# ZihanLiao/pytorch-kaldi-resnet

Hardware: AMD Instinct MI355X
Metric: utterances/sec (300-frame x 80 fbank, bs256/GPU), ResNet-34 + AAM-softmax training step (higher is better)
Workload: dtype f32 (operands as 2 fp16 terms of value x 2^k, 3 cross products, f32 accumulate); 1 GPU; BASELINE configs[1]: ResNet-34 + AAM-softmax (m 0.2, s 30), 1211 speakers, 300-frame x 80 fbank, per-GPU batch 256, fwd+CE+bwd+SGD(0.9, wd 5e-4); global_batch=256, frames=300, feat_dim=80, parallelism=dp1, launch=hipGraph replay (1 graph), mfma=f16x3

## Files before the change

### include/spkhip.h

```cpp
#ifndef SPKHIP_H
#define SPKHIP_H
#include <stddef.h>
#ifdef __cplusplus
extern "C" {
#endif

int spk_version(void);
const char* spk_last_error(void);
int spk_build_flags(void);

#define SPK_IN_AFFINE_RELU 1
#define SPK_EPI_AFFINE 2
#define SPK_EPI_ADD 4
#define SPK_EPI_RELU 8
#define SPK_EPI_STATS 16
#define SPK_IN_BNBWD 64
#define SPK_EPI_BNBWD 32

#define SPK_CONV_WS 128
#define SPK_CONV_PIPE 1024

#define SPK_CONV_M16 (1 << 17)

#define SPK_WGRAD_GROUPS 2048

#define SPK_WGRAD_NOSHIFT (1 << 18)
#define SPK_WGRAD_M16 (1 << 19)
#define SPK_IN_PRESPLIT (1 << 14)
#define SPK_SIDE_PRESPLIT (1 << 15)
#define SPK_DY_PRESPLIT (1 << 16)
#define SPK_CONV_CK32 (1 << 23)
#define SPK_EPI_WMASK (1 << 24)


int spk_pack_conv_weight(const float* w, float* wpk, int Cout, int Cin, int KH, int KW, int transpose, void* stream);
int spk_pack_conv_weight_split(const float* w, void* wpk, int Cout, int Cin, int KH, int KW, int transpose, int split,
                               void* stream);
int spk_pack_job_bytes(void);
int spk_pack_conv_weights_batched(const void* jobs, int njobs, int total_blocks, int has_f16 , void* stream);

int spk_conv_mfma(const float* in, const float* wpk, float* out, const float* in_scale, const float* in_shift,
                  const float* epi_scale, const float* epi_shift, const float* epi_add, const float* in_raw,
                  const float* in_act, const float* in_bn4, const float* in_coef, const unsigned* in_mask , const unsigned* bn_mask , const unsigned* add_mask ,
                  float* side_draw, float* side_dz,
                  const float* bn_raw, const float* bn_act, const float* bn4, float* stats, int B, int IH,
                  int IW, int Cin, int OH, int OW, int OHf, int OWf, int Cout, int IS, int OS, int ooy, int oox,
                  int ntaps, const int* tap_dy , const int* tap_dx , const int* tap_w , int TH,
                  int TW, int MT, int NT, int kc, int ips, int flags, int split, const unsigned* in_amax, unsigned* out_amax,
                  unsigned* side_amax, void* stream);
int spk_conv_mfma_len(const float* in, const float* wpk, float* out, const float* in_scale, const float* in_shift,
                      const float* epi_scale, const float* epi_shift, const float* epi_add, const float* in_raw,
                      const float* in_act, const float* in_bn4, const float* in_coef, const unsigned* in_mask,
                      const unsigned* bn_mask, const unsigned* add_mask, float* side_draw, float* side_dz,
                      const float* bn_raw, const float* bn_act, const float* bn4, float* stats, int B, int IH,
                      int IW, int Cin, int OH, int OW, int OHf, int OWf, int Cout, int IS, int OS, int ooy, int oox,
                      int ntaps, const int* tap_dy , const int* tap_dx , const int* tap_w , int TH,
                      int TW, int MT, int NT, int kc, int ips, int flags, int split, const unsigned* in_amax, unsigned* out_amax,
                      unsigned* side_amax, const int* wlen , void* stream);

int spk_conv_wgrad_limits(int WN, int* max_halo_pix , int* max_tile_pix );
size_t spk_conv_wgrad_workspace(int nsplit, int ksize, int Cin, int Cout);
int spk_conv3x3_c32_stream(const float* in, const float* wpk, float* out, const float* in_scale, const float* in_shift, float* stats,
                           int B, int H, int W, int flags, const unsigned* in_amax, unsigned* out_amax, int nblocks, void* stream);
int spk_conv1x1_stream(const float* in, const float* wpk, float* out, const float* in_scale, const float* in_shift,
                       const float* epi_add, const unsigned* add_mask, const float* bn_raw, const unsigned* bn_mask,
                       const float* bn4, float* stats, long long P, int C, int flags, const unsigned* in_amax, unsigned* out_amax,
                       int nblocks, void* stream);
int spk_conv1x1_stream_rows(int nblocks, int C);
int spk_wgrad_reduce(const float* partial, float* dw, int nslab, int ksize, int Cin, int Cout, int accumulate, void* stream);
int spk_conv_wgrad(const float* x, const float* dy, float* dw, float* partial, const float* in_scale,
                   const float* in_shift, int B, int IH, int IW, int Cin, int OH, int OW, int Cout, int ksize, int stride,
                   int TH, int TW, int WN, int nsplit, int flags, int accumulate, int split , const unsigned* dy_amax , const unsigned* x_amax , void* stream);

#define SPK_PTR_ADD_MASK 1
#define SPK_PTR_BN_MASK 2
#define SPK_PTR_IN_MASK 4
#define SPK_PTR_IN_ACT 8
#define SPK_PTR_BN_ACT 16
#define SPK_PTR_SIDE_DZ 32
int spk_conv_variant_of(int MT, int NT, int split, int flags, int ptrs);
int spk_wgrad_variant_of(int ksize, int stride, int TH, int TW, int WN, int split, int flags);

int spk_stem_fwd_blocks(int B, int F, int T);
int spk_stem_conv_fwd(const float* x, const float* w, float* out, float* stats, const float* epi_scale,
                      const float* epi_shift, int B, int F, int T, int flags,
                      unsigned* amax_out , void* stream);
int spk_stem_conv_fwd_len(const float* x, const float* w, float* out, float* stats, const float* epi_scale,
                          const float* epi_shift, int B, int F, int T, int flags, unsigned* amax_out, const int* len ,
                          void* stream);
int spk_stem_wgrad_blocks(int B, int F, int T);
int spk_stem_conv_wgrad(const float* x, const float* draw, float* dw, float* partial, int B, int F, int T,
                        int accumulate, void* stream);
int spk_stem_stats(const float* x, const float* w, float* stats, int B, int F, int T, void* stream);
int spk_stem_fwd_apply(const float* x, const float* w, const float* scale, const float* shift, float* raw_out, float* act_out,
                       unsigned* mask_out, unsigned* amax_out, int B, int F, int T, void* stream);
int spk_stem_bwd_wgrad(const float* x, const float* d, const float* raw, const float* mean, const float* invstd,
                       const float* scale, const float* shift, const float* coef, float* dw, float* partial, int B, int F, int T,
                       int accumulate, void* stream);

int spk_bn_stats_blocks(long long N, int C);
int spk_bn_stats_partial(const float* x, float* partial , long long N, int C, void* stream);
size_t spk_bn_finalize_workspace(int nblk, int C);
int spk_bn_finalize(const float* partial, int nblk, int C, double count, const float* gamma, const float* beta,
                    float* running_mean, float* running_var, long long* num_batches_tracked, float* mean, float* invstd,
                    float* scale, float* shift, float momentum, float eps, double* ws,
                    const unsigned* amax_in, unsigned* est_out ,
                    void* stream);
int spk_bn_eval_coeffs(const float* gamma, const float* beta, const float* running_mean, const float* running_var,
                       float* scale, float* shift, int C, float eps, void* stream);
int spk_bn_apply(const float* raw, const float* scale, const float* shift, const float* res, const float* res_scale,
                 const float* res_shift, float* out, unsigned* mask_out, long long N, int C, int relu,
                 unsigned* amax_out , void* stream);
int spk_bn_bwd_reduce(const float* dy, const float* raw, const float* act, const float* mean, const float* invstd,
                      const float* scale, const float* shift, float* partial, long long N, int C, int mask_mode,
                      unsigned* chan_amax , void* stream);
int spk_bn_bwd_finalize(const float* partial, int nblk, int C, double count, const float* gamma, const float* invstd,
                        float* dgamma, float* dbeta, float* coef , int accumulate, double* ws,
                        const unsigned* amax_in, const unsigned* raw_amax, const float* mean, unsigned* est_out ,
                        const unsigned* chan_amax ,
                        void* stream);
int spk_bn_bwd_apply(const float* dy, const float* raw, const float* act, const float* mean, const float* invstd,
                     const float* scale, const float* shift, const float* coef, float* draw, float* dz_out, long long N,
                     int C, int mask_mode, unsigned* amax_out ,
                     const unsigned* pair_scale , void* stream);
int spk_absmax(const float* x, unsigned* slot, long long n, void* stream);
int spk_bnbwd_estimate(const float* coef, const float* mean, const float* invstd, int C, const unsigned* amax_in,
                       const unsigned* raw_amax, unsigned* est, void* stream);
int spk_f16_window_count(const float* x, const float* scale, const float* shift, long long n, int C, const unsigned* slot,
                         int pairs, unsigned long long* counts , void* stream);
int spk_affine_estimate(const float* scale, const float* shift, int C, const unsigned* amax_in, unsigned* est, void* stream);

int spk_se_chunks(long long HW);
int spk_se_squeeze(const float* x, float* partial, double* sums , int B, int H, int W, int C, const int* wlen,
                   void* stream);
int spk_se_excite(const double* sums, const float* scale, const float* shift, const float* W1, const float* W2, float* q,
                  float* u, float* g, int B, int C, int Cr, int H, int W, const int* wlen, void* stream);
int spk_se_apply(const float* raw, const float* scale, const float* shift, const float* gate, const float* res,
                 const float* res_scale, const float* res_shift, float* out, unsigned* mask_out, int B, int H, int W, int C,
                 int relu, unsigned* amax_out, const int* wlen, void* stream);
int spk_se_bwd_reduce(const float* dout, const float* raw, const float* act, float* partial, double* S , int B,
                      long long HW, int C, int mask_mode, unsigned* chan_amax, void* stream);
int spk_se_bwd_gate(const double* S, const double* sums, const float* q, const float* u, const float* g, const float* W1,
                    const float* W2, const float* mean, const float* invstd, const float* scale, const float* shift,
                    const float* gamma, float* da, float* du, float* dq, float* dW1, float* dW2, float* dgamma, float* dbeta,
                    float* coef, int accumulate, int B, int C, int Cr, long long HW, const unsigned* amax_in,
                    const unsigned* raw_amax, const unsigned* chan_amax, unsigned* est_out, void* stream);
int spk_se_bwd_apply(const float* dout, const float* raw, const float* act, const float* gate, const float* dqs ,
                     const float* mean, const float* invstd, const float* coef, float* draw, float* e_out, int B, long long HW,
                     int C, int mask_mode, unsigned* amax_out, const unsigned* pair_scale, void* stream);

int spk_stats_pool_fwd(const float* x , float* out , int B, int H, int W, int C,
                       int mode, void* stream);
int spk_stats_pool_fwd_len(const float* x, float* out, const int* wlen, int B, int H, int W, int C, int mode, void* stream);
int spk_stats_pool_bwd(const float* x, const float* gout, float* dx, int B, int H, int W, int C, int mode,
                       unsigned* amax_out , void* stream);
int spk_stats_pool_row_form(int on);
int spk_stats_pool_row_cap(void);

int spk_gemm_splitk(int M, int N, int K);
size_t spk_gemm_workspace(int M, int N, int K);
int spk_gemm_f32(const float* A, const float* B, float* C, const float* bias, int M, int N, int K, long long sam,
                 long long sak, long long sbk, long long sbn, long long ldc, float alpha, int accumulate, float* workspace,
                 void* stream);
int spk_colsum(const float* dy, float* db, int M, int N, int accumulate, void* stream);

int spk_l2norm_fwd(const float* x, float* y, float* inv_norm, int R, int D, float eps, void* stream);
int spk_l2norm_bwd(const float* y, const float* inv_norm, const float* dy, float* dx, int R, int D, float eps,
                   int accumulate, void* stream);
int spk_aam_margin_fwd(const float* cosv, const long long* label, float* logits, int B, int S, float m, float s,
                       void* stream);
int spk_aam_margin_bwd(const float* cosv, const long long* label, const float* dlogits, float* dcos, int B, int S,
                       float m, float s, void* stream);
int spk_softmax_ce(const float* logits, const long long* label, float* loss_row, float* dlogits, int* rank, int B, int S,
                   float grad_scale, void* stream);
int spk_mean(const float* v, float* out, int n, void* stream);
int spk_relu_bwd(const float* y, const float* dy, float* dx, long long n, void* stream);

int spk_sgd_step(float* p, const float* g, float* buf, long long n, float lr, float momentum, float weight_decay,
                 float grad_scale, int first_step, void* stream);

int spk_center_normalize(const float* emb , const float* mean , float* out, int N, int D, float eps,
                         void* stream);
int spk_trial_cosine(const float* en , const float* te , const int* ia, const int* ib, float* out,
                     int T, int D, int n_en, int n_te, void* stream);
int spk_topk_mean_std(const float* scores, float* mean_out, float* std_out, int N, int M, int k, long long ld, void* stream);

int spk_eval_tile(int which);
int spk_segment_mean(const double* emb , const int* rows , const int* seg_off , float* out ,
                     int N, int S, int D, void* stream);
int spk_trial_snorm(const void* score, int score_f64, const int* ia, const int* ib, const double* e_mean, const double* e_std,
                    const double* t_mean, const double* t_std, double* out, int T, void* stream);
size_t spk_sort_trials_workspace(int T);
int spk_sort_trials(const double* score, unsigned* order, void* ws, int T, void* stream);
size_t spk_error_sweep_workspace(int T, int P);
int spk_error_sweep(const double* score, const unsigned char* label, const unsigned* order, const double* costs, int P,
                    double* out_d , long long* out_i , void* ws, int T, void* stream);

int spk_fbank_tile_frames(int L, int S, int P, int F);
int spk_fbank_fwd(const float* wave, const int* nsamp, const long long* utt_ids, int B, long long Nmax, const float* window,
                  const float* twiddle, const float* mel_w, const int* mel_lo, const int* mel_off, int L, int S, int P, int F,
                  int snip_edges, float dither, float preemph, int remove_dc, float energy_floor, unsigned long long seed,
                  float* feats, float* log_energy, int* T_out, int Tcap, void* stream);
int spk_mfcc_tile_frames(int L, int S, int P, int F, int C);
int spk_mfcc_fwd(const float* wave, const int* nsamp, const long long* utt_ids, int B, long long Nmax, const float* window,
                 const float* twiddle, const float* mel_w, const int* mel_lo, const int* mel_off, const float* dct,
                 const float* lifter, int L, int S, int P, int F, int C, int snip_edges, float dither, float preemph, int remove_dc,
                 float energy_floor, int use_energy, int htk_compat, unsigned long long seed, float* feats, float* log_energy,
                 int* T_out, int Tcap, void* stream);
int spk_fbank_span_fwd(const float* wave, const int* nsamp, const long long* first, const long long* total, const int* frame0,
                       const int* nframes, const long long* utt_ids, int B, long long Nmax, const float* window, const float* twiddle,
                       const float* mel_w, const int* mel_lo, const int* mel_off, int L, int S, int P, int F, int snip_edges,
                       float dither, float preemph, int remove_dc, float energy_floor, unsigned long long seed, float* feats,
                       float* log_energy, int* T_out, int Tcap, void* stream);
int spk_mfcc_span_fwd(const float* wave, const int* nsamp, const long long* first, const long long* total, const int* frame0,
                      const int* nframes, const long long* utt_ids, int B, long long Nmax, const float* window, const float* twiddle,
                      const float* mel_w, const int* mel_lo, const int* mel_off, const float* dct, const float* lifter, int L, int S,
                      int P, int F, int C, int snip_edges, float dither, float preemph, int remove_dc, float energy_floor,
                      int use_energy, int htk_compat, unsigned long long seed, float* feats, float* log_energy, int* T_out, int Tcap,
                      void* stream);
int spk_pcm16_to_f32(const short* pcm , const int* count , int B, long long Nmax, float* out ,
                     void* stream);
int spk_fbank_dither_noise(float* out , long long utt_id, unsigned long long seed, int frame0, int nframes, int L,
                           void* stream);
int spk_vad_count(const float* log_energy, const int* T, int B, int Tcap, double energy_threshold, double mean_scale,
                  int frames_context, double proportion, int* vad , int* idx , int* count ,
                  void* stream);
int spk_cmn_select(const float* x, const int* T, const int* idx, const int* count, double* prefix, float* out, int B, int F,
                   int Tcap, int Tout, int cmn_window, void* stream);

int spk_resample_tile(int iu, int ou, int K);
int spk_resample_fwd(const float* wave_in, const int* nsamp_in, int B, long long Nmax_in, const int* first, const float* wq,
                     int fi, int fo, int K, float* wave_out, int* nsamp_out, long long Nmax_out, void* stream);

int spk_augment_max_rir(void);
int spk_augment_max_early(void);
int spk_augment_workspace(int B, long long Nmax, int Rmax, int Emax, long long Fmax, int nd, long long* sizes );
int spk_augment_fwd(const float* wave, const int* nsamp, int B, long long Nmax, const float* rir_pool, long long rir_pool_len,
                    const long long* rir_off, const int* rir_row, int Rmax, int Emax, const float* noise_pool,
                    long long noise_pool_len, const int* desc_ptr, const long long* desc_off, const int* desc_len,
                    const double* desc_snr, int nd, long long Fmax, const float* twiddle, float* spectra, float* y, double* work,
                    int quantize, float* out, unsigned long long* clipped, void* stream);

int spk_cm_decode(const unsigned char* codes, const float* colhdr, const int* lengths, int B, int F, int T, float* out, void* stream);
int spk_cm_compress(const float* x, const int* T, int B, int F, int Tcap, float* ws, float* minrange, int* hdr, unsigned char* codes,
                    void* stream);

int spk_scatter_slab_rows(long long N);
size_t spk_scatter_f64_workspace(long long N, int D);
int spk_scatter_f64(const void* X, int x_f64, long long ld, const double* mu, const double* w, double* C, void* ws, long long N, int D,
                    void* stream);
int spk_segment_sum_f64(const void* X, int x_f64, long long ld, const int* rows, const int* seg_off , double* out ,
                        int* count , int mean, int K, int D, void* stream);
int spk_affine_lennorm(const void* X, int x_f64, long long ldx, const double* A, const double* b, const double* q, int scale, void* Y,
                       int y_f64, long long N, int Di, int Do, void* stream);
int spk_plda_posterior_rows(const double* mt , const int* count, const double* psi, double* w_out, double* r_out, int K,
                            int D, void* stream);
int spk_plda_llr(const double* en , const double* te , const int* ia, const int* ib, const double* psi,
                 const int* count , const int* tab_count , const double* tab_log , int U, float* out,
                 int T, int D, int n_en, int n_te, void* stream);

#ifdef __cplusplus
}
#endif
#endif
```

### pytorch-kaldi-resnet_amd/csrc/bn.hip

```cpp
#include "spk_common.h"

enum { MASK_NONE = 0, MASK_ACT = 1, MASK_RAW = 2, MASK_BITS = 3 };

__global__ __launch_bounds__(256) void bn_stats_partial_kernel(const float* __restrict__ x, float* __restrict__ partial,
                                                               long long N, int C, int rows_per_block) {
    __shared__ float red[256][8];
    const int tid = threadIdx.x;
    const int qpr = C >> 2;
    const int quad = tid % qpr, prow = tid / qpr, rstep = 256 / qpr;
    const long long r0 = (long long)blockIdx.x * rows_per_block;
    long long r1 = r0 + rows_per_block;
    if (r1 > N) r1 = N;
    f32x4 s = {0.f, 0.f, 0.f, 0.f}, ss = {0.f, 0.f, 0.f, 0.f};
    for (long long r = r0 + prow; r < r1; r += rstep) {
        const f32x4 v = *(const f32x4*)(x + r * C + quad * 4);
        s += v;
        ss += v * v;
    }
#pragma unroll
    for (int k = 0; k < 4; ++k) {
        red[tid][k] = s[k];
        red[tid][4 + k] = ss[k];
    }
    __syncthreads();
    if (tid < qpr) {
        float a[8];
#pragma unroll
        for (int k = 0; k < 8; ++k) a[k] = 0.f;
        for (int p = 0; p < rstep; ++p)
#pragma unroll
            for (int k = 0; k < 8; ++k) a[k] += red[p * qpr + tid][k];
        float* dst = partial + ((size_t)blockIdx.x * C + tid * 4) * 2;
#pragma unroll
        for (int k = 0; k < 4; ++k) {
            dst[k * 2 + 0] = a[k];
            dst[k * 2 + 1] = a[4 + k];
        }
    }
}

static bool bn_c_ok(int C) { return C >= 4 && C <= 1024 && (C & (C - 1)) == 0; }

#ifndef BN_STATS_BLOCKS
#define BN_STATS_BLOCKS 4096
#endif
extern "C" int spk_bn_stats_blocks(long long N, int C) {
    (void)C;
    long long nb = (N + 255) / 256;
    if (nb > BN_STATS_BLOCKS) nb = BN_STATS_BLOCKS;
    return (int)(nb < 1 ? 1 : nb);
}

extern "C" int spk_bn_stats_partial(const float* x, float* partial, long long N, int C, void* stream) {
    SPK_REQUIRE(x && partial, "spk_bn_stats_partial: null pointer");
    SPK_REQUIRE(N > 0 && bn_c_ok(C), "spk_bn_stats_partial: N=%lld C=%d (C must be a power of two in [4,1024])", N, C);
    const int nb = spk_bn_stats_blocks(N, C);
    const int rpb = (int)((N + nb - 1) / nb);
    hipLaunchKernelGGL(bn_stats_partial_kernel, dim3(nb), dim3(256), 0, (hipStream_t)stream, x, partial, N, C, rpb);
    SPK_LAUNCH_CHECK("spk_bn_stats_partial");
    return 0;
}

#define BN_STAGE_ROWS 256
__global__ __launch_bounds__(256) void bn_fold_partials_kernel(const float* __restrict__ partial, double* __restrict__ ws,
                                                               int nblk, int C) {
    __shared__ double red[8][32][2];
    const int tid = threadIdx.x, c = tid & 31, row = tid >> 5;
    const int ch = blockIdx.x * 32 + c;
    const int per = (nblk + BN_STAGE_ROWS - 1) / BN_STAGE_ROWS;
    const int k0 = blockIdx.y * per;
    int k1 = k0 + per;
    if (k1 > nblk) k1 = nblk;
    double s = 0.0, ss = 0.0;
    if (ch < C) {
        const size_t pitch = (size_t)8 * C * 2;
        const float* q = partial + ((size_t)(k0 + row) * C + ch) * 2;
        int k = k0 + row;
        for (; k + 24 < k1; k += 32, q += 4 * pitch) {
            const float2 a = *(const float2*)q, b = *(const float2*)(q + pitch);
            const float2 c2 = *(const float2*)(q + 2 * pitch), d = *(const float2*)(q + 3 * pitch);
            s += (double)a.x; ss += (double)a.y;
            s += (double)b.x; ss += (double)b.y;
            s += (double)c2.x; ss += (double)c2.y;
            s += (double)d.x; ss += (double)d.y;
        }
        for (; k < k1; k += 8, q += pitch) {
            const float2 p = *(const float2*)q;
            s += (double)p.x;
            ss += (double)p.y;
        }
    }
    red[row][c][0] = s;
    red[row][c][1] = ss;
    __syncthreads();
    if (row == 0 && ch < C) {
        for (int k = 1; k < 8; ++k) {
            s += red[k][c][0];
            ss += red[k][c][1];
        }
        ws[((size_t)blockIdx.y * C + ch) * 2 + 0] = s;
        ws[((size_t)blockIdx.y * C + ch) * 2 + 1] = ss;
    }
}

template <typename T>
__device__ inline void bn_sum_rows(const T* __restrict__ partial, int nrows, int C, int ch, int row, double& s, double& ss) {
    const size_t pitch = (size_t)8 * C * 2;
    const T* p = partial + ((size_t)row * C + ch) * 2;
    int k = row;
    for (; k + 24 < nrows; k += 32, p += 4 * pitch) {
        const T a0 = p[0], a1 = p[1], b0 = p[pitch], b1 = p[pitch + 1];
        const T c0 = p[2 * pitch], c1 = p[2 * pitch + 1], d0 = p[3 * pitch], d1 = p[3 * pitch + 1];
        s += (double)a0; ss += (double)a1;
        s += (double)b0; ss += (double)b1;
        s += (double)c0; ss += (double)c1;
        s += (double)d0; ss += (double)d1;
    }
    for (; k < nrows; k += 8, p += pitch) {
        s += (double)p[0];
        ss += (double)p[1];
    }
}

template <typename T>
__global__ __launch_bounds__(256) void bn_finalize_kernel(const T* __restrict__ partial, int nblk, int C, double count,
                                                          const float* __restrict__ gamma, const float* __restrict__ beta,
                                                          float* __restrict__ running_mean, float* __restrict__ running_var,
                                                          long long* __restrict__ nbt, float* __restrict__ mean_out,
                                                          float* __restrict__ invstd_out, float* __restrict__ scale,
                                                          float* __restrict__ shift, float momentum, float eps,
                                                          const unsigned* __restrict__ amax_in, unsigned* __restrict__ est_out) {
    __shared__ double red[8][32][2];
    const int tid = threadIdx.x, c = tid & 31, row = tid >> 5;
    const int ch = blockIdx.x * 32 + c;
    double s = 0.0, ss = 0.0;
    if (ch < C) bn_sum_rows<T>(partial, nblk, C, ch, row, s, ss);
    red[row][c][0] = s;
    red[row][c][1] = ss;
    __syncthreads();
    if (row == 0 && ch < C) {
        for (int k = 1; k < 8; ++k) {
            s += red[k][c][0];
            ss += red[k][c][1];
        }
        const double mean = s / count;
        double var = ss / count - mean * mean;
        if (var < 0.0 || count <= 1.0) var = 0.0;
        const float invstd = (float)(1.0 / sqrt(var + (double)eps));
        const float g = gamma[ch], b = beta[ch];
        const float sc = g * invstd;
        mean_out[ch] = (float)mean;
        invstd_out[ch] = invstd;
        const float shv = b - (float)mean * sc;
        scale[ch] = sc;
        shift[ch] = shv;
        if (est_out) {
            const float e = fabsf(sc) * __uint_as_float(*amax_in) + fabsf(shv);
            const unsigned bits = __float_as_uint(e);
            if (bits > __hip_atomic_load(est_out, __ATOMIC_RELAXED, __HIP_MEMORY_SCOPE_AGENT)) atomicMax(est_out, bits);
        }
        if (running_mean) {
            const double unbiased = count > 1.0 ? var * (count / (count - 1.0)) : var;
            running_mean[ch] = (1.f - momentum) * running_mean[ch] + momentum * (float)mean;
            running_var[ch] = (1.f - momentum) * running_var[ch] + momentum * (float)unbiased;
        }
    }
    if (nbt && blockIdx.x == 0 && tid == 0) *nbt += 1;
}

extern "C" size_t spk_bn_finalize_workspace(int nblk, int C) {
    return nblk > BN_STAGE_ROWS ? (size_t)BN_STAGE_ROWS * C * 2 * sizeof(double) : 0;
}

extern "C" int spk_bn_finalize(const float* partial, int nblk, int C, double count, const float* gamma, const float* beta,
                               float* running_mean, float* running_var, long long* num_batches_tracked, float* mean,
                               float* invstd, float* scale, float* shift, float momentum, float eps, double* ws,
                               const unsigned* amax_in, unsigned* est_out, void* stream) {
    SPK_REQUIRE(partial && gamma && beta && mean && invstd && scale && shift, "spk_bn_finalize: null pointer");
    SPK_REQUIRE(nblk > 0 && C > 0 && count > 0, "spk_bn_finalize: bad sizes");
    SPK_REQUIRE((running_mean == nullptr) == (running_var == nullptr), "spk_bn_finalize: running stats must come in pairs");
    SPK_REQUIRE(!est_out || amax_in, "spk_bn_finalize: est_out needs amax_in");
    hipStream_t st = (hipStream_t)stream;
    if (spk_bn_finalize_workspace(nblk, C)) {
        SPK_REQUIRE(ws, "spk_bn_finalize: %d partial rows need the fp64 workspace", nblk);
        hipLaunchKernelGGL(bn_fold_partials_kernel, dim3(spk_ceil_div(C, 32), BN_STAGE_ROWS), dim3(256), 0, st, partial, ws, nblk, C);
        SPK_LAUNCH_CHECK("spk_bn_finalize(fold)");
        hipLaunchKernelGGL(bn_finalize_kernel<double>, dim3(spk_ceil_div(C, 32)), dim3(256), 0, st, ws, BN_STAGE_ROWS, C, count,
                           gamma, beta, running_mean, running_var, num_batches_tracked, mean, invstd, scale, shift, momentum, eps,
                           amax_in, est_out);
    } else {
        hipLaunchKernelGGL(bn_finalize_kernel<float>, dim3(spk_ceil_div(C, 32)), dim3(256), 0, st, partial, nblk, C, count, gamma,
                           beta, running_mean, running_var, num_batches_tracked, mean, invstd, scale, shift, momentum, eps, amax_in,
                           est_out);
    }
    SPK_LAUNCH_CHECK("spk_bn_finalize");
    return 0;
}

__global__ void bn_eval_coeffs_kernel(const float* gamma, const float* beta, const float* rm, const float* rv,
                                      float* scale, float* shift, int C, float eps) {
    const int c = blockIdx.x * blockDim.x + threadIdx.x;
    if (c >= C) return;
    const float invstd = 1.f / sqrtf(rv[c] + eps);
    const float sc = gamma[c] * invstd;
    scale[c] = sc;
    shift[c] = beta[c] - rm[c] * sc;
}

extern "C" int spk_bn_eval_coeffs(const float* gamma, const float* beta, const float* running_mean,
                                  const float* running_var, float* scale, float* shift, int C, float eps, void* stream) {
    SPK_REQUIRE(gamma && beta && running_mean && running_var && scale && shift, "spk_bn_eval_coeffs: null pointer");
    hipLaunchKernelGGL(bn_eval_coeffs_kernel, dim3(spk_ceil_div(C, 256)), dim3(256), 0, (hipStream_t)stream, gamma, beta,
                       running_mean, running_var, scale, shift, C, eps);
    SPK_LAUNCH_CHECK("spk_bn_eval_coeffs");
    return 0;
}

#ifndef BN_APPLY_U
#define BN_APPLY_U 4
#endif
#ifndef BN_APPLY_CAP
#define BN_APPLY_CAP 0
#endif
#ifndef BN_BWD_APPLY_U
#define BN_BWD_APPLY_U 1
#endif
#ifndef BN_BWD_APPLY_CAP
#define BN_BWD_APPLY_CAP 2048
#endif
static int stream_grid(long long nquads, int per_thread = 1, int cap = 8192) {
    long long nb = (nquads + 256LL * per_thread - 1) / (256LL * per_thread);
    if (cap > 0 && nb > cap) nb = cap;
    if (nb > 2147483647LL) nb = 2147483647LL;
    return (int)(nb < 1 ? 1 : nb);
}
#ifndef BN_NT
#define BN_NT 1
#endif
static __device__ __forceinline__ f32x4 ld_stream(const float* p) {
#if BN_NT
    return __builtin_nontemporal_load((const f32x4*)p);
#else
    return *(const f32x4*)p;
#endif
}
static __device__ __forceinline__ void st_stream(float* p, f32x4 v) {
#if BN_NT
    __builtin_nontemporal_store(v, (f32x4*)p);
#else
    *(f32x4*)p = v;
#endif
}
__global__ __launch_bounds__(256) void bn_apply_kernel(const float* __restrict__ raw, const float* __restrict__ scale,
                                                       const float* __restrict__ shift, const float* __restrict__ res,
                                                       const float* __restrict__ rscale, const float* __restrict__ rshift,
                                                       float* __restrict__ out, unsigned* __restrict__ mask_out, long long nquads,
                                                       int C, int relu, unsigned* __restrict__ amax_out) {
    const int cmask = C - 1;
    float mx = 0.f;
    constexpr int U = BN_APPLY_U;
    const long long stride = (long long)gridDim.x * 256;
    const bool fixed_c = C <= 1024;
    const int c0 = (threadIdx.x * 4) & cmask;
    f32x4 psc = *(const f32x4*)(scale + c0), psh = *(const f32x4*)(shift + c0), prs = psc, prh = psh;
    if (rscale) {
        prs = *(const f32x4*)(rscale + c0);
        prh = *(const f32x4*)(rshift + c0);
    }
    for (long long i0 = (long long)blockIdx.x * 256 + threadIdx.x; i0 < nquads; i0 += stride * U) {
        f32x4 rv[U], sv[U];
        long long idx[U];
#pragma unroll
        for (int u = 0; u < U; ++u) {
            const long long i = i0 + stride * u;
            idx[u] = i < nquads ? i : i0;
            rv[u] = ld_stream(raw + idx[u] * 4);
            if (res) sv[u] = ld_stream(res + idx[u] * 4);
        }
#pragma unroll
        for (int u = 0; u < U; ++u) {
            const long long i = i0 + stride * u;
            if (i >= nquads) continue;
            if (!fixed_c) {
                const int c = (int)((i * 4) & cmask);
                psc = *(const f32x4*)(scale + c);
                psh = *(const f32x4*)(shift + c);
                if (rscale) {
                    prs = *(const f32x4*)(rscale + c);
                    prh = *(const f32x4*)(rshift + c);
                }
            }
            f32x4 v = rv[u] * psc + psh;
            if (res) {
                f32x4 r = sv[u];
                if (rscale) r = r * prs + prh;
                v += r;
            }
            if (relu) {
                v[0] = fmaxf(v[0], 0.f);
                v[1] = fmaxf(v[1], 0.f);
                v[2] = fmaxf(v[2], 0.f);
                v[3] = fmaxf(v[3], 0.f);
            }
            st_stream(out + i * 4, v);
            mx = fmaxf(fmaxf(mx, fmaxf(fabsf(v[0]), fabsf(v[1]))), fmaxf(fabsf(v[2]), fabsf(v[3])));
            if (mask_out) {
                unsigned bits = (v[0] > 0.f ? 1u : 0u) | (v[1] > 0.f ? 2u : 0u) | (v[2] > 0.f ? 4u : 0u) | (v[3] > 0.f ? 8u : 0u);
                bits <<= 4 * (threadIdx.x & 7);
                bits |= __shfl_xor(bits, 1, 64);
                bits |= __shfl_xor(bits, 2, 64);
                bits |= __shfl_xor(bits, 4, 64);
                if ((threadIdx.x & 7) == 0) mask_out[i >> 3] = bits;
            }
        }
    }
    if (amax_out) spk_wave_amax_commit(mx, amax_out);
}

extern "C" int spk_bn_apply(const float* raw, const float* scale, const float* shift, const float* res,
                            const float* res_scale, const float* res_shift, float* out, unsigned* mask_out, long long N, int C,
                            int relu, unsigned* amax_out, void* stream) {
    SPK_REQUIRE(raw && scale && shift && out, "spk_bn_apply: null pointer");
    SPK_REQUIRE(N > 0 && bn_c_ok(C), "spk_bn_apply: N=%lld C=%d", N, C);
    SPK_REQUIRE((res_scale == nullptr) == (res_shift == nullptr), "spk_bn_apply: residual affine must come in pairs");
    SPK_REQUIRE(!res_scale || res, "spk_bn_apply: residual affine without residual");
    SPK_REQUIRE(!mask_out || C % 32 == 0, "spk_bn_apply: the sign mask needs C %% 32 == 0 (C=%d)", C);
    const long long nquads = N * C / 4;
    hipLaunchKernelGGL(bn_apply_kernel, dim3(stream_grid(nquads, BN_APPLY_U, BN_APPLY_CAP)), dim3(256), 0, (hipStream_t)stream, raw, scale, shift, res,
                       res_scale, res_shift, out, mask_out, nquads, C, relu, amax_out);
    SPK_LAUNCH_CHECK("spk_bn_apply");
    return 0;
}

__device__ inline f32x4 bn_mask(f32x4 dy, int mode, const float* act, const float* raw_p, f32x4 rawv, f32x4 sc, f32x4 sh,
                                long long off, int C = 0) {
    if (mode == MASK_BITS) {
        const int lg = 31 - __builtin_clz((unsigned)C);
        const long long pix = off >> lg;
        const int c = (int)(off & (C - 1));
        const unsigned bits = ((const unsigned*)act)[pix * (C >> 5) + (c >> 5)] >> (c & 31);
#pragma unroll
        for (int k = 0; k < 4; ++k) dy[k] = ((bits >> k) & 1u) ? dy[k] : 0.f;
    } else if (mode == MASK_ACT) {
        const f32x4 a = *(const f32x4*)(act + off);
#pragma unroll
        for (int k = 0; k < 4; ++k) dy[k] = a[k] > 0.f ? dy[k] : 0.f;
    } else if (mode == MASK_RAW) {
        const f32x4 z = rawv * sc + sh;
#pragma unroll
        for (int k = 0; k < 4; ++k) dy[k] = z[k] > 0.f ? dy[k] : 0.f;
    }
    (void)raw_p;
    return dy;
}

__global__ __launch_bounds__(256) void bn_bwd_reduce_kernel(const float* __restrict__ dy, const float* __restrict__ raw,
                                                            const float* __restrict__ act, const float* __restrict__ mean,
                                                            const float* __restrict__ invstd, const float* __restrict__ scale,
                                                            const float* __restrict__ shift, float* __restrict__ partial,
                                                            long long N, int C, int rows_per_block, int mode,
                                                            unsigned* __restrict__ chan_amax) {
    __shared__ float red[256][8];
    const int tid = threadIdx.x;
    const int qpr = C >> 2;
    const int quad = tid % qpr, prow = tid / qpr, rstep = 256 / qpr;
    const long long r0 = (long long)blockIdx.x * rows_per_block;
    long long r1 = r0 + rows_per_block;
    if (r1 > N) r1 = N;
    const f32x4 mu = *(const f32x4*)(mean + quad * 4), is = *(const f32x4*)(invstd + quad * 4);
    const f32x4 sc = *(const f32x4*)(scale + quad * 4), sh = *(const f32x4*)(shift + quad * 4);
    f32x4 s = {0.f, 0.f, 0.f, 0.f}, ss = {0.f, 0.f, 0.f, 0.f}, mx = {0.f, 0.f, 0.f, 0.f};
    for (long long r = r0 + prow; r < r1; r += rstep) {
        const long long off = r * C + quad * 4;
        const f32x4 rv = ld_stream(raw + off);
        f32x4 d = ld_stream(dy + off);
        d = bn_mask(d, mode, act, raw, rv, sc, sh, off, C);
        const f32x4 xh = (rv - mu) * is;
        s += d;
        ss += d * xh;
#pragma unroll
        for (int k = 0; k < 4; ++k) mx[k] = fmaxf(mx[k], spk_finite_abs(d[k]));
    }
#pragma unroll
    for (int k = 0; k < 4; ++k) {
        red[tid][k] = s[k];
        red[tid][4 + k] = ss[k];
    }
    __syncthreads();
    if (tid < qpr) {
        float a[8];
#pragma unroll
        for (int k = 0; k < 8; ++k) a[k] = 0.f;
        for (int p = 0; p < rstep; ++p)
#pragma unroll
            for (int k = 0; k < 8; ++k) a[k] += red[p * qpr + tid][k];
        float* dst = partial + ((size_t)blockIdx.x * C + tid * 4) * 2;
#pragma unroll
        for (int k = 0; k < 4; ++k) {
            dst[k * 2 + 0] = a[k];
            dst[k * 2 + 1] = a[4 + k];
        }
    }
    if (chan_amax) {
        __syncthreads();
#pragma unroll
        for (int k = 0; k < 4; ++k) red[tid][k] = mx[k];
        __syncthreads();
        if (tid < qpr) {
#pragma unroll
            for (int k = 0; k < 4; ++k) {
                float m = 0.f;
                for (int p = 0; p < rstep; ++p) m = fmaxf(m, red[p * qpr + tid][k]);
                const unsigned bits = __float_as_uint(m);
                unsigned* slot = chan_amax + tid * 4 + k;
                if (bits > __hip_atomic_load(slot, __ATOMIC_RELAXED, __HIP_MEMORY_SCOPE_AGENT)) atomicMax(slot, bits);
            }
        }
    }
}

extern "C" int spk_bn_bwd_reduce(const float* dy, const float* raw, const float* act, const float* mean, const float* invstd,
                                 const float* scale, const float* shift, float* partial, long long N, int C, int mask_mode,
                                 unsigned* chan_amax, void* stream) {
    SPK_REQUIRE(dy && raw && mean && invstd && scale && shift && partial, "spk_bn_bwd_reduce: null pointer");
    SPK_REQUIRE(N > 0 && bn_c_ok(C), "spk_bn_bwd_reduce: N=%lld C=%d", N, C);
    SPK_REQUIRE(mask_mode >= 0 && mask_mode <= 3, "spk_bn_bwd_reduce: mask_mode=%d", mask_mode);
    SPK_REQUIRE((mask_mode != MASK_ACT && mask_mode != MASK_BITS) || act, "spk_bn_bwd_reduce: MASK_ACT / MASK_BITS need the activated tensor / its sign bits");
    const int nb = spk_bn_stats_blocks(N, C);
    const int rpb = (int)((N + nb - 1) / nb);
    hipLaunchKernelGGL(bn_bwd_reduce_kernel, dim3(nb), dim3(256), 0, (hipStream_t)stream, dy, raw, act, mean, invstd, scale,
                       shift, partial, N, C, rpb, mask_mode, chan_amax);
    SPK_LAUNCH_CHECK("spk_bn_bwd_reduce");
    return 0;
}

__device__ inline float bnbwd_bound(float k1, float m1, float m2, float mean, float invstd, float A, float R) {
    const float xh = (R + fabsf(mean)) * fabsf(invstd);
    return fabsf(k1) * (A + fabsf(m1) + xh * fabsf(m2)) * (1.f + 1.52587890625e-05f);
}

template <typename T>
__global__ __launch_bounds__(256) void bn_bwd_finalize_kernel(const T* __restrict__ partial, int nblk, int C, double count,
                                                              const float* __restrict__ gamma, const float* __restrict__ invstd,
                                                              float* __restrict__ dgamma, float* __restrict__ dbeta,
                                                              float* __restrict__ coef, int accumulate,
                                                              const unsigned* __restrict__ amax_in, const unsigned* __restrict__ raw_amax,
                                                              const float* __restrict__ mean, unsigned* __restrict__ est_out,
                                                              const unsigned* __restrict__ chan_amax) {
    __shared__ double red[8][32][2];
    const int tid = threadIdx.x, c = tid & 31, row = tid >> 5;
    const int ch = blockIdx.x * 32 + c;
    double s = 0.0, ss = 0.0;
    if (ch < C) bn_sum_rows<T>(partial, nblk, C, ch, row, s, ss);
    red[row][c][0] = s;
    red[row][c][1] = ss;
    __syncthreads();
    if (row == 0 && ch < C) {
        for (int k = 1; k < 8; ++k) {
            s += red[k][c][0];
            ss += red[k][c][1];
        }
        dbeta[ch] = accumulate ? dbeta[ch] + (float)s : (float)s;
        dgamma[ch] = accumulate ? dgamma[ch] + (float)ss : (float)ss;
        const float k1 = gamma[ch] * invstd[ch], m1 = (float)(s / count), m2 = (float)(ss / count);
        coef[ch] = k1;
        coef[C + ch] = m1;
        coef[2 * C + ch] = m2;
        if (est_out) {
            const float A = chan_amax ? __uint_as_float(chan_amax[ch]) : __uint_as_float(*amax_in);
            const float e = bnbwd_bound(k1, m1, m2, mean[ch], invstd[ch], A, __uint_as_float(*raw_amax));
            const unsigned bits = __float_as_uint(e);
            if (bits > __hip_atomic_load(est_out, __ATOMIC_RELAXED, __HIP_MEMORY_SCOPE_AGENT)) atomicMax(est_out, bits);
        }
    }
}

extern "C" int spk_bn_bwd_finalize(const float* partial, int nblk, int C, double count, const float* gamma,
                                   const float* invstd, float* dgamma, float* dbeta, float* coef, int accumulate,
                                   double* ws, const unsigned* amax_in, const unsigned* raw_amax, const float* mean,
                                   unsigned* est_out, const unsigned* chan_amax, void* stream) {
    SPK_REQUIRE(partial && gamma && invstd && dgamma && dbeta && coef, "spk_bn_bwd_finalize: null pointer");
    SPK_REQUIRE(nblk > 0 && C > 0 && count > 0, "spk_bn_bwd_finalize: bad sizes");
    SPK_REQUIRE(!est_out || ((amax_in || chan_amax) && raw_amax && mean),
                "spk_bn_bwd_finalize: est_out needs amax_in (or chan_amax), raw_amax and mean");
    hipStream_t st = (hipStream_t)stream;
    if (spk_bn_finalize_workspace(nblk, C)) {
        SPK_REQUIRE(ws, "spk_bn_bwd_finalize: %d partial rows need the fp64 workspace", nblk);
        hipLaunchKernelGGL(bn_fold_partials_kernel, dim3(spk_ceil_div(C, 32), BN_STAGE_ROWS), dim3(256), 0, st, partial, ws, nblk, C);
        SPK_LAUNCH_CHECK("spk_bn_bwd_finalize(fold)");
        hipLaunchKernelGGL(bn_bwd_finalize_kernel<double>, dim3(spk_ceil_div(C, 32)), dim3(256), 0, st, ws, BN_STAGE_ROWS, C, count,
                           gamma, invstd, dgamma, dbeta, coef, accumulate, amax_in, raw_amax, mean, est_out, chan_amax);
    } else {
        hipLaunchKernelGGL(bn_bwd_finalize_kernel<float>, dim3(spk_ceil_div(C, 32)), dim3(256), 0, st, partial, nblk, C, count, gamma,
                           invstd, dgamma, dbeta, coef, accumulate, amax_in, raw_amax, mean, est_out, chan_amax);
    }
    SPK_LAUNCH_CHECK("spk_bn_bwd_finalize");
    return 0;
}

__global__ __launch_bounds__(256) void bn_bwd_apply_kernel(const float* __restrict__ dy, const float* __restrict__ raw,
                                                           const float* __restrict__ act, const float* __restrict__ mean,
                                                           const float* __restrict__ invstd, const float* __restrict__ scale,
                                                           const float* __restrict__ shift, const float* __restrict__ coef,
                                                           float* __restrict__ draw, float* __restrict__ dz_out,
                                                           unsigned nquads, int C, int mode, unsigned* __restrict__ amax_out,
                                                           const unsigned* __restrict__ pair_scale) {
    const int cmask = C - 1;
    float mx = 0.f;
    const float sig = pair_scale ? spk_sigma_from_amax_bits(*pair_scale) : 1.f;
    constexpr int U = BN_BWD_APPLY_U;
    const unsigned stride = gridDim.x * 256u;
    const int lgq = 29 - __builtin_clz((unsigned)C);
    const unsigned cw = (unsigned)C >> 5;
    const bool fixed_c = C <= 1024;
    const int c0 = (threadIdx.x * 4) & cmask;
    f32x4 pmu = *(const f32x4*)(mean + c0), pis = *(const f32x4*)(invstd + c0), pk1 = *(const f32x4*)(coef + c0);
    f32x4 pm1 = *(const f32x4*)(coef + C + c0), pm2 = *(const f32x4*)(coef + 2 * C + c0), psc = pmu, psh = pmu;
    if (mode == MASK_RAW) {
        psc = *(const f32x4*)(scale + c0);
        psh = *(const f32x4*)(shift + c0);
    }
    for (unsigned i0 = blockIdx.x * 256u + threadIdx.x; i0 < nquads; i0 += stride * U) {
        f32x4 rvv[U], dv[U], av[U];
        unsigned mw[U];
#pragma unroll
        for (int u = 0; u < U; ++u) {
            const unsigned i = i0 + stride * u;
            const unsigned ii = i < nquads && i >= i0 ? i : i0;
            const size_t off = (size_t)ii * 4;
            rvv[u] = ld_stream(raw + off);
            dv[u] = ld_stream(dy + off);
            if (mode == MASK_BITS) mw[u] = ((const unsigned*)act)[(size_t)(ii >> lgq) * cw + (((ii * 4u) & (unsigned)cmask) >> 5)];
            else if (mode == MASK_ACT) av[u] = *(const f32x4*)(act + off);
        }
#pragma unroll
        for (int u = 0; u < U; ++u) {
            const unsigned i = i0 + stride * u;
            if (i >= nquads || i < i0) continue;
            const int c = fixed_c ? c0 : (int)((i * 4u) & (unsigned)cmask);
            if (!fixed_c) {
                pmu = *(const f32x4*)(mean + c);
                pis = *(const f32x4*)(invstd + c);
                pk1 = *(const f32x4*)(coef + c);
                pm1 = *(const f32x4*)(coef + C + c);
                pm2 = *(const f32x4*)(coef + 2 * C + c);
                if (mode == MASK_RAW) {
                    psc = *(const f32x4*)(scale + c);
                    psh = *(const f32x4*)(shift + c);
                }
            }
            const size_t off = (size_t)i * 4;
            const f32x4 rv = rvv[u];
            f32x4 d = dv[u];
            if (mode == MASK_BITS) {
                const unsigned bits = mw[u] >> (c & 31);
#pragma unroll
                for (int k = 0; k < 4; ++k) d[k] = ((bits >> k) & 1u) ? d[k] : 0.f;
            } else if (mode == MASK_ACT) {
#pragma unroll
                for (int k = 0; k < 4; ++k) d[k] = av[u][k] > 0.f ? d[k] : 0.f;
            } else if (mode == MASK_RAW) {
                const f32x4 z = rv * psc + psh;
#pragma unroll
                for (int k = 0; k < 4; ++k) d[k] = z[k] > 0.f ? d[k] : 0.f;
            }
            const f32x4 xh = (rv - pmu) * pis;
            const f32x4 o = pk1 * (d - pm1 - xh * pm2);
            if (dz_out) st_stream(dz_out + off, d);
            if (pair_scale) {
                uint2 t0, t1;
                split2h(o, sig, t0, t1);
                st_stream(draw + off, spk_pair_pack(t0, t1));
            } else
                st_stream(draw + off, o);
            mx = fmaxf(fmaxf(mx, fmaxf(fabsf(o[0]), fabsf(o[1]))), fmaxf(fabsf(o[2]), fabsf(o[3])));
        }
    }
    if (amax_out) spk_wave_amax_commit(mx, amax_out);
}

extern "C" int spk_bn_bwd_apply(const float* dy, const float* raw, const float* act, const float* mean, const float* invstd,
                                const float* scale, const float* shift, const float* coef, float* draw, float* dz_out,
                                long long N, int C, int mask_mode, unsigned* amax_out, const unsigned* pair_scale, void* stream) {
    SPK_REQUIRE(dy && raw && mean && invstd && scale && shift && coef && draw, "spk_bn_bwd_apply: null pointer");
    SPK_REQUIRE(N > 0 && bn_c_ok(C), "spk_bn_bwd_apply: N=%lld C=%d", N, C);
    SPK_REQUIRE(mask_mode >= 0 && mask_mode <= 3, "spk_bn_bwd_apply: mask_mode=%d", mask_mode);
    SPK_REQUIRE((mask_mode != MASK_ACT && mask_mode != MASK_BITS) || act, "spk_bn_bwd_apply: MASK_ACT / MASK_BITS need the activated tensor / its sign bits");
    const long long nquads = N * C / 4;
    SPK_REQUIRE(nquads < 2147483647LL / 8, "spk_bn_bwd_apply: %lld values exceed the 32-bit group index of the kernel", N * C);
    hipLaunchKernelGGL(bn_bwd_apply_kernel, dim3(stream_grid(nquads, BN_BWD_APPLY_U, BN_BWD_APPLY_CAP)), dim3(256), 0, (hipStream_t)stream, dy, raw, act, mean,
                       invstd, scale, shift, coef, draw, dz_out, (unsigned)nquads, C, mask_mode, amax_out, pair_scale);
    SPK_LAUNCH_CHECK("spk_bn_bwd_apply");
    return 0;
}

__global__ __launch_bounds__(256) void absmax_kernel(const float* __restrict__ x, long long n, unsigned* __restrict__ slot) {
    float mx = 0.f;
    const long long nq = n >> 2;
    for (long long i = (long long)blockIdx.x * 256 + threadIdx.x; i < nq; i += (long long)gridDim.x * 256) {
        const f32x4 v = *(const f32x4*)(x + i * 4);
        mx = fmaxf(fmaxf(mx, fmaxf(spk_finite_abs(v[0]), spk_finite_abs(v[1]))), fmaxf(spk_finite_abs(v[2]), spk_finite_abs(v[3])));
    }
    if (blockIdx.x == 0 && threadIdx.x < (n & 3)) mx = fmaxf(mx, spk_finite_abs(x[nq * 4 + threadIdx.x]));
    spk_wave_amax_commit(mx, slot);
}

extern "C" int spk_absmax(const float* x, unsigned* slot, long long n, void* stream) {
    SPK_REQUIRE(x && slot && n > 0, "spk_absmax: bad arguments");
    SPK_REQUIRE((((size_t)x) & 15) == 0, "spk_absmax: x must be 16-byte aligned");
    hipLaunchKernelGGL(absmax_kernel, dim3(stream_grid(n / 4 + 1)), dim3(256), 0, (hipStream_t)stream, x, n, slot);
    SPK_LAUNCH_CHECK("spk_absmax");
    return 0;
}

__global__ __launch_bounds__(256) void bnbwd_estimate_kernel(const float* __restrict__ coef, const float* __restrict__ mean,
                                                             const float* __restrict__ invstd, int C,
                                                             const unsigned* __restrict__ amax_in, const unsigned* __restrict__ raw_amax,
                                                             unsigned* __restrict__ est) {
    __shared__ float red[4];
    const float A = __uint_as_float(*amax_in), R = __uint_as_float(*raw_amax);
    float mx = 0.f;
    for (int c = threadIdx.x; c < C; c += 256)
        mx = fmaxf(mx, bnbwd_bound(coef[c], coef[C + c], coef[2 * C + c], mean[c], invstd[c], A, R));
#pragma unroll
    for (int off = 32; off >= 1; off >>= 1) mx = fmaxf(mx, __shfl_xor(mx, off, 64));
    if ((threadIdx.x & 63) == 0) red[threadIdx.x >> 6] = mx;
    __syncthreads();
    if (threadIdx.x == 0) *est = __float_as_uint(fmaxf(fmaxf(red[0], red[1]), fmaxf(red[2], red[3])));
}

__global__ __launch_bounds__(256) void affine_estimate_kernel(const float* __restrict__ scale, const float* __restrict__ shift, int C,
                                                              const unsigned* __restrict__ amax_in, unsigned* __restrict__ est) {
    __shared__ float red[2][4];
    float ms = 0.f, mh = 0.f;
    for (int c = threadIdx.x; c < C; c += 256) {
        ms = fmaxf(ms, fabsf(scale[c]));
        mh = fmaxf(mh, fabsf(shift[c]));
    }
#pragma unroll
    for (int off = 32; off >= 1; off >>= 1) {
        ms = fmaxf(ms, __shfl_xor(ms, off, 64));
        mh = fmaxf(mh, __shfl_xor(mh, off, 64));
    }
    if ((threadIdx.x & 63) == 0) {
        red[0][threadIdx.x >> 6] = ms;
        red[1][threadIdx.x >> 6] = mh;
    }
    __syncthreads();
    if (threadIdx.x == 0) {
        ms = fmaxf(fmaxf(red[0][0], red[0][1]), fmaxf(red[0][2], red[0][3]));
        mh = fmaxf(fmaxf(red[1][0], red[1][1]), fmaxf(red[1][2], red[1][3]));
        *est = __float_as_uint(ms * __uint_as_float(*amax_in) + mh);
    }
}

extern "C" int spk_affine_estimate(const float* scale, const float* shift, int C, const unsigned* amax_in, unsigned* est,
                                   void* stream) {
    SPK_REQUIRE(scale && shift && amax_in && est && C > 0, "spk_affine_estimate: bad arguments");
    hipLaunchKernelGGL(affine_estimate_kernel, dim3(1), dim3(256), 0, (hipStream_t)stream, scale, shift, C, amax_in, est);
    SPK_LAUNCH_CHECK("spk_affine_estimate");
    return 0;
}

extern "C" int spk_bnbwd_estimate(const float* coef, const float* mean, const float* invstd, int C, const unsigned* amax_in,
                                  const unsigned* raw_amax, unsigned* est, void* stream) {
    SPK_REQUIRE(coef && mean && invstd && amax_in && raw_amax && est && C > 0, "spk_bnbwd_estimate: bad arguments");
    hipLaunchKernelGGL(bnbwd_estimate_kernel, dim3(1), dim3(256), 0, (hipStream_t)stream, coef, mean, invstd, C, amax_in, raw_amax, est);
    SPK_LAUNCH_CHECK("spk_bnbwd_estimate");
    return 0;
}

__global__ __launch_bounds__(256) void f16_window_count_kernel(const float* __restrict__ x, const float* __restrict__ scale,
                                                               const float* __restrict__ shift, long long nquads, int C,
                                                               const unsigned* __restrict__ slot, int pairs,
                                                               unsigned long long* __restrict__ counts) {
    const float sig = spk_sigma_from_amax_bits(*slot);
    const int cmask = C - 1;
    unsigned n = 0, sat = 0, lo_lost = 0, hi_sub = 0;
    for (long long i = (long long)blockIdx.x * 256 + threadIdx.x; i < nquads; i += (long long)gridDim.x * 256) {
        f32x4 v = *(const f32x4*)(x + i * 4);
        float hi[4], lo[4];
        if (pairs) {
            const uint4 u = __builtin_bit_cast(uint4, v);
            const f16x4 a = __builtin_bit_cast(f16x4, (uint2){u.x, u.y}), b = __builtin_bit_cast(f16x4, (uint2){u.z, u.w});
#pragma unroll
            for (int k = 0; k < 4; ++k) {
                hi[k] = (float)a[k];
                lo[k] = (float)b[k];
                sat += fabsf(hi[k]) >= 65504.f;
            }
        } else {
            if (scale) {
                const int c = (int)((i * 4) & cmask);
                v = v * *(const f32x4*)(scale + c) + *(const f32x4*)(shift + c);
#pragma unroll
                for (int k = 0; k < 4; ++k) v[k] = fmaxf(v[k], 0.f);
            }
#pragma unroll
            for (int k = 0; k < 4; ++k) {
                const float u = v[k] * sig;
                sat += fabsf(u) > 65504.f;
                const float uc = __builtin_amdgcn_fmed3f(u, -65504.f, 65504.f);
                const _Float16 a = (_Float16)uc;
                hi[k] = (float)a;
                lo[k] = (float)(_Float16)(uc - (float)a);
            }
        }
#pragma unroll
        for (int k = 0; k < 4; ++k) {
            n += 1;
            lo_lost += lo[k] != 0.f && fabsf(lo[k]) < 6.103515625e-05f;
            hi_sub += hi[k] != 0.f && fabsf(hi[k]) < 6.103515625e-05f;
        }
    }
    unsigned vals[4] = {n, sat, lo_lost, hi_sub};
#pragma unroll
    for (int j = 0; j < 4; ++j) {
        unsigned v = vals[j];
#pragma unroll
        for (int off = 32; off >= 1; off >>= 1) v += __shfl_xor(v, off, 64);
        if ((threadIdx.x & 63) == 0 && v) atomicAdd(counts + j, (unsigned long long)v);
    }
}

extern "C" int spk_f16_window_count(const float* x, const float* scale, const float* shift, long long n, int C,
                                    const unsigned* slot, int pairs, unsigned long long* counts, void* stream) {
    SPK_REQUIRE(x && slot && counts && n > 0 && n % 4 == 0, "spk_f16_window_count: bad arguments (n must be a multiple of 4)");
    SPK_REQUIRE((scale == nullptr) == (shift == nullptr), "spk_f16_window_count: scale / shift come in pairs");
    SPK_REQUIRE(!scale || (bn_c_ok(C) && !pairs), "spk_f16_window_count: the affine form needs a power-of-two C and an fp32 tensor");
    hipLaunchKernelGGL(f16_window_count_kernel, dim3(stream_grid(n / 4)), dim3(256), 0, (hipStream_t)stream, x, scale, shift, n / 4,
                       scale ? C : 4, slot, pairs, counts);
    SPK_LAUNCH_CHECK("spk_f16_window_count");
    return 0;
}
```

### pytorch-kaldi-resnet_amd/engine.py

```python
import torch

from . import ops
from .hip import MASK_ACT, MASK_BITS, MASK_NONE, MASK_RAW


class _Conv:
    def __init__(self, holder):
        self.h = holder
        self.cin, self.cout, self.k, self.stride = holder.cin, holder.cout, holder.k, holder.stride
        self.wpk = None
        self.wpk_t = None

    def repack(self, need_t):
        w = self.h.weight.data
        if self.cin == 1:
            return
        self.wpk = ops.pack_conv_weight(w, False, self.wpk)
        if need_t:
            self.wpk_t = ops.pack_conv_weight(w, True, self.wpk_t)

    def pack_jobs(self, need_t):
        w = self.h.weight.data
        if self.cin == 1:
            return []
        n = ops.packed_numel(w)
        if self.wpk is None or self.wpk.numel() != n:
            self.wpk = torch.empty(n, device=w.device, dtype=torch.float32)
        jobs = [(w, self.wpk, False)]
        if need_t:
            nt = ops.packed_numel(w, bwd=True)
            if self.wpk_t is None or self.wpk_t.numel() != nt:
                self.wpk_t = torch.empty(nt, device=w.device, dtype=torch.float32)
            jobs.append((w, self.wpk_t, True))
        return jobs


class _BN:
    def __init__(self, holder):
        self.h = holder
        self.c = holder.c
        self.t4 = None
        self.s4 = None
        self.e2 = None

    def finalize(self, partial, count, amax_in=None, est_out=None, keep=True):
        name = "t4" if keep else "s4"
        if getattr(self, name) is None:
            setattr(self, name, torch.empty(4, self.c, device=partial.device, dtype=torch.float32))
        t4 = getattr(self, name)
        h = self.h
        ops.bn_finalize(partial, count, h.weight.data, h.bias.data, h.running_mean, h.running_var, h.num_batches_tracked,
                        t4, amax_in=amax_in, est_out=est_out)
        return t4

    def eval_coeffs(self):
        h = self.h
        if self.e2 is None:
            self.e2 = torch.empty(2, self.c, device=h.weight.device, dtype=torch.float32)
        ops.bn_eval_coeffs(h.weight.data, h.bias.data, h.running_mean, h.running_var, self.e2)
        return self.e2


class _Block:
    def __init__(self, bp):
        self.kind = bp.kind
        self.convs = [_Conv(bp.conv1), _Conv(bp.conv2)] + ([_Conv(bp.conv3)] if bp.kind == "bottleneck" else [])
        self.bns = [_BN(bp.bn1), _BN(bp.bn2)] + ([_BN(bp.bn3)] if bp.kind == "bottleneck" else [])
        self.ds = None
        if bp.downsample is not None:
            self.ds = (_Conv(bp.downsample[0]), _BN(bp.downsample[1]))
        self.se = bp.se if bp.kind == "se_basic" else None


class _LogitsFn(torch.autograd.Function):

    @staticmethod
    def forward(ctx, eng, x, y, anchor):
        logits, saved = eng.forward_train(x, y)
        ctx.eng = eng
        ctx.saved = saved
        return logits

    @staticmethod
    def backward(ctx, dlogits):
        ctx.eng.backward(ctx.saved, dlogits.contiguous())
        ctx.saved = None
        return None, None, None, None


class Engine:
    def __init__(self, model):
        self.m = model
        r = model.res
        self.stem_conv = _Conv(r.conv1)
        self.stem_bn = _BN(r.bn1)
        self.blocks = []
        for li in range(1, 5):
            for bp in getattr(r, "layer%d" % li):
                self.blocks.append(_Block(bp))
        self.head_bn = _BN(model.bn1) if hasattr(model, "bn1") else None
        self.pool_mode = 1 if model.pooling == "mean+std" else 0
        self.dirty = True
        self._packed_for_bwd = False
        self._pack_tables = {}
        self._amax_pool = None
        self._amax_fwd = None
        self._amax_eval = None
        self._fwd_gen = 0
        self.wgrad_stream = None
        self.use_side_stream = True
        self.fuse_bn_reduce = True
        self.fuse_bn_apply = True
        import os
        self.use_sign_masks = os.environ.get("SPK_SIGN_MASKS", "1") == "1"
        self.fuse_apply_min_c = int(os.environ.get("SPK_FUSE_APPLY_MINC", "0"))
        self._fuse_apply_max_c = int(os.environ["SPK_FUSE_APPLY_MAXC"]) if "SPK_FUSE_APPLY_MAXC" in os.environ else None
        self.fuse_apply_1x1 = os.environ.get("SPK_FUSE_APPLY_1X1", "0") == "1"
        self.pair_draw = os.environ.get("SPK_PAIR_DRAW", "1") == "1"
        stem_fused = os.environ.get("SPK_STEM_FUSED", "1")
        self.stem_fused_fwd = stem_fused in ("1", "fwd")
        self.stem_fused_bwd = stem_fused in ("1", "bwd")
        self.chan_amax = os.environ.get("SPK_CHAN_AMAX", "1") == "1"
        self.window_counts = None
        self.bound_log = None

    @property
    def fuse_apply_max_c(self):
        if self._fuse_apply_max_c is not None:
            return self._fuse_apply_max_c
        return 32 if (self.pair_draw and ops.split_for(3, True) == 3) else 1000000

    @fuse_apply_max_c.setter
    def fuse_apply_max_c(self, v):
        self._fuse_apply_max_c = v

    def _all_convs(self):
        for b in self.blocks:
            for c in b.convs:
                yield c
            if b.ds is not None:
                yield b.ds[0]

    def _repack(self, need_t):
        if not self.dirty and (self._packed_for_bwd or not need_t):
            return
        jobs = [j for c in self._all_convs() for j in c.pack_jobs(need_t)]
        key = [(w.data_ptr(), p.data_ptr(), t, ops.split_for(w.shape[2], t)) for w, p, t in jobs]
        tab = self._pack_tables.get(need_t)
        if tab is None or tab.key != key:
            assert not torch.cuda.is_current_stream_capturing() or tab is None, "pack table changed during graph capture"
            tab = self._pack_tables[need_t] = ops.PackTable(jobs, jobs[0][0].device)
        tab.run()
        self.dirty = False
        self._packed_for_bwd = need_t

    def _check_input(self, x):
        if not x.is_cuda:
            raise RuntimeError("pytorch_kaldi_resnet_amd runs on MI355X only: input must be a device tensor "
                               "(there is no CPU fallback)")
        if x.dim() != 3 or x.size(1) != self.m.feat_dim:
            raise RuntimeError("expected input [B, %d, T], got %s" % (self.m.feat_dim, tuple(x.shape)))
        if x.dtype != torch.float32:
            raise RuntimeError("expected float32 input")
        return x.contiguous()

    def _fwd_pool(self, device, train=False):
        if ops.split_for(3) != 3 and ops.split_for(3, True) != 3:
            return None
        name = "_amax_fwd" if train else "_amax_eval"
        if getattr(self, name) is None:
            setattr(self, name, ops.AmaxPool(device))
        pool = getattr(self, name)
        pool.reset()
        return pool

    def _count(self, x, slot, affine=None, pairs=False):
        if self.window_counts is not None and slot is not None:
            ops.f16_window_count(x, slot, self.window_counts, affine=affine, pairs=pairs)

    def trunk_eval(self, x, wl=None):
        self._repack(False)
        pool = self._fwd_pool(x.device)
        take = (lambda: pool.take()) if pool is not None else (lambda: None)
        f16 = ops.split_for(3) == 3
        e = self.stem_bn.eval_coeffs()
        a_amax = take()
        a, _ = ops.stem_fwd(x, self.stem_conv.h.weight.data, epi_affine=(e[0], e[1]), relu=True, amax_out=a_amax,
                            wlen=None if wl is None else wl[0])
        stage = 0
        for b in self.blocks:
            evs = [bn.eval_coeffs() for bn in b.bns]
            if b.ds is not None:
                ed = b.ds[1].eval_coeffs()
                res, _ = ops.conv_fwd(a, b.ds[0].wpk, b.ds[0].cout, 1, b.ds[0].stride, epi_affine=(ed[0], ed[1]),
                                      in_amax=a_amax if ops.split_for(1) == 3 else None)
            else:
                res = a
            h, h_amax = a, a_amax
            n = len(b.convs)
            for i, (c, ev) in enumerate(zip(b.convs, evs)):
                last = i == n - 1
                o_amax = take()
                if c.stride == 2:
                    stage += 1
                if last and b.se is not None:
                    wls = None if wl is None else wl[stage]
                    z, _ = ops.conv_fwd(h, c.wpk, c.cout, c.k, c.stride, epi_affine=(ev[0], ev[1]),
                                        in_amax=h_amax if ops.split_for(c.k) == 3 else None)
                    _, gate = self._se_gate(b, z, None, wls)
                    h = ops.se_apply(z, None, gate, res=res, relu=True, amax_out=o_amax, wlen=wls)
                    h_amax = o_amax
                    continue
                h, _ = ops.conv_fwd(h, c.wpk, c.cout, c.k, c.stride, epi_affine=(ev[0], ev[1]),
                                    epi_add=res if last else None, relu=True,
                                    in_amax=h_amax if ops.split_for(c.k) == 3 else None, out_amax=o_amax,
                                    wlen=None if wl is None else wl[stage])
                h_amax = o_amax
            a, a_amax = h, h_amax
        return a

    @staticmethod
    def _se_gate(b, t, affine, wlen=None):
        sums = ops.se_squeeze(t, wlen)
        q, u, g = ops.se_excite(sums, affine, b.se.w1.data, b.se.w2.data, t.shape[1], t.shape[2], wlen)
        return (sums, q, u, g), g

    def embed_eval(self, x, wl=None):
        feat = self.trunk_eval(x, wl)
        pooled = ops.stats_pool_fwd(feat, self.pool_mode, wlen=None if wl is None else wl[3])
        return ops.linear_fwd(pooled, self.m.fc1.weight.data, self.m.fc1.bias.data)

    @staticmethod
    def stage_widths(lengths, B, T, device):
        if isinstance(lengths, torch.Tensor):
            if lengths.dtype.is_floating_point or lengths.dtype.is_complex or lengths.dtype == torch.bool:
                raise TypeError("lengths must be integers, got a %s tensor" % lengths.dtype)
            L = lengths.detach().to("cpu", torch.int64).reshape(-1)
            if lengths.dim() != 1:
                raise ValueError("lengths must be one-dimensional [B], got shape %s" % (tuple(lengths.shape),))
        else:
            vals = list(lengths)
            if not all(isinstance(v, int) or (hasattr(v, "__index__") and not isinstance(v, (bool, float))) for v in vals) \
                    or any(isinstance(v, bool) for v in vals):
                raise TypeError("lengths must be integers")
            L = torch.tensor([int(v) for v in vals], dtype=torch.int64)
        if L.numel() != B:
            raise ValueError("lengths has %d entries for a batch of %d utterances" % (L.numel(), B))
        if B and (int(L.min()) < 1 or int(L.max()) > T):
            raise ValueError("lengths must lie in [1, T=%d], got min %d max %d" % (T, int(L.min()), int(L.max())))
        w = [L]
        for _ in range(3):
            w.append((w[-1] + 1) // 2)
        return torch.stack(w).to(torch.int32).to(device)

    def predict(self, x, lengths=None):
        x = self._check_input(x)
        with torch.no_grad():
            if lengths is not None:
                if self.m.training:
                    raise RuntimeError("predict(lengths=...) needs eval mode: with BatchNorm batch statistics a padded batch has "
                                       "no per-utterance meaning (call model.eval() first)")
                return self.embed_eval(x, self.stage_widths(lengths, x.shape[0], x.shape[2], x.device))
            if self.m.training:
                emb, _ = self._embed_train(x, save=False)
                return emb
            return self.embed_eval(x)

    def _head_fwd(self, emb, y, train, save):
        m = self.m
        sv = {}
        h = emb
        if m.loss in ("softmax", "AAM-v1"):
            bn = self.head_bn
            if train:
                part = ops.bn_stats_partial(emb)
                t4 = bn.finalize(part, emb.shape[0], keep=save)
                h = ops.bn_apply(emb, t4[2], t4[3], relu=True)
            else:
                e2 = bn.eval_coeffs()
                h = ops.bn_apply(emb, e2[0], e2[1], relu=True)
            sv["h"] = h
        if m.loss == "softmax":
            logits = ops.linear_fwd(h, m.last.weight.data, m.last.bias.data)
        else:
            if y is None:
                raise RuntimeError("AAM heads need labels (scripts/model.py:483: label=None fails in the reference too)")
            y = y.contiguous()
            hn, hinv = ops.l2norm_fwd(h)
            wn, winv = ops.l2norm_fwd(m.last.weight.data)
            B, S, D = h.shape[0], wn.shape[0], wn.shape[1]
            cosv = ops.gemm(hn, wn, B, S, D, D, 1, 1, D)
            logits = ops.aam_margin_fwd(cosv, y, m.m, m.s)
            if save:
                sv.update(hn=hn, hinv=hinv, wn=wn, winv=winv, cosv=cosv, y=y)
        return logits, sv

    def _head_bwd(self, emb, sv, dlogits, acc):
        m = self.m
        if m.loss == "softmax":
            dh = ops.linear_bwd(sv["h"], m.last.weight.data, dlogits, m.last.weight.grad, m.last.bias.grad, accumulate=acc)
        else:
            dcos = ops.aam_margin_bwd(sv["cosv"], sv["y"], dlogits, m.m, m.s)
            B, S = dcos.shape
            D = sv["wn"].shape[1]
            dhn = ops.gemm(dcos, sv["wn"], B, D, S, S, 1, D, 1)
            dwn = ops.gemm(dcos, sv["hn"], S, D, B, 1, S, D, 1)
            dh = ops.l2norm_bwd(sv["hn"], sv["hinv"], dhn)
            ops.l2norm_bwd(sv["wn"], sv["winv"], dwn, out=m.last.weight.grad, accumulate=acc)
        if m.loss in ("softmax", "AAM-v1"):
            bn = self.head_bn
            dh = ops.bn_backward(dh, emb, sv["h"], bn.t4, bn.h.weight.data, bn.h.weight.grad, bn.h.bias.grad, MASK_ACT,
                                 accumulate=acc)
        return dh

    def _trunk_train(self, x, save):
        saved = {"x": x, "blocks": []}
        pool = self._fwd_pool(x.device, train=save)
        if save:
            self._fwd_gen += 1
        saved["gen"] = self._fwd_gen
        take = (lambda: pool.take()) if pool is not None else (lambda: None)
        f16 = ops.split_for(3) == 3
        B, F, T = x.shape
        use_masks = save and self.use_sign_masks
        w0 = self.stem_conv.h.weight.data
        if self.stem_fused_fwd:
            t4 = self.stem_bn.finalize(ops.stem_stats(x, w0), B * F * T, keep=save)
            a_amax = take()
            raw0, a, amask = ops.stem_fwd_apply(x, w0, t4[2], t4[3], mask=use_masks, amax_out=a_amax)
        else:
            raw0, st = ops.stem_fwd(x, w0, stats=True)
            t4 = self.stem_bn.finalize(st, B * F * T, keep=save)
            a_amax = take()
            a = ops.bn_apply(raw0, t4[2], t4[3], relu=True, mask=use_masks, amax_out=a_amax)
            a, amask = a if use_masks else (a, None)
        saved["raw0"] = raw0
        for b in self.blocks:
            rec = {"x": a, "xmask": amask, "in_amax": [], "raw_amax": []}
            raws = []
            h, aff, h_amax = a, None, a_amax
            for c, bn in zip(b.convs, b.bns):
                rec["in_amax"].append(h_amax)
                raw_amax = take()
                rec["raw_amax"].append(raw_amax)
                if ops.split_for(c.k) == 3:
                    self._count(h, h_amax, affine=aff)
                raw, st = ops.conv_fwd(h, c.wpk, c.cout, c.k, c.stride, in_affine=aff, stats=True,
                                       in_amax=h_amax if ops.split_for(c.k) == 3 else None, out_amax=raw_amax)
                est = take()
                t4 = bn.finalize(st, raw.shape[0] * raw.shape[1] * raw.shape[2], amax_in=raw_amax, est_out=est, keep=save)
                raws.append(raw)
                h, aff, h_amax = raw, (t4[2], t4[3]), est
            out_amax = take()
            gate = None
            if b.se is not None:
                rec["se"], gate = self._se_gate(b, h, aff)
            if b.ds is not None:
                rawd, st = ops.conv_fwd(a, b.ds[0].wpk, b.ds[0].cout, 1, b.ds[0].stride, stats=True,
                                        in_amax=a_amax if ops.split_for(1) == 3 else None)
                td = b.ds[1].finalize(st, rawd.shape[0] * rawd.shape[1] * rawd.shape[2], keep=save)
                if gate is not None:
                    out = ops.se_apply(h, aff, gate, res=rawd, res_affine=(td[2], td[3]), relu=True, mask=use_masks,
                                       amax_out=out_amax)
                else:
                    out = ops.bn_apply(h, aff[0], aff[1], res=rawd, res_affine=(td[2], td[3]), relu=True, mask=use_masks,
                                       amax_out=out_amax)
                rec["rawd"] = rawd
            elif gate is not None:
                out = ops.se_apply(h, aff, gate, res=a, relu=True, mask=use_masks, amax_out=out_amax)
            else:
                out = ops.bn_apply(h, aff[0], aff[1], res=a, relu=True, mask=use_masks, amax_out=out_amax)
            out, amask = out if use_masks else (out, None)
            rec["raws"] = raws
            rec["out"] = out
            rec["mask"] = amask
            if save:
                saved["blocks"].append(rec)
            a, a_amax = out, out_amax
        return a, saved

    def _embed_train(self, x, save):
        self._repack(save)
        feat, saved = self._trunk_train(x, save)
        pooled = ops.stats_pool_fwd(feat, self.pool_mode)
        emb = ops.linear_fwd(pooled, self.m.fc1.weight.data, self.m.fc1.bias.data)
        saved["feat"], saved["pooled"], saved["emb"] = feat, pooled, emb
        return emb, saved

    def forward_train(self, x, y):
        emb, saved = self._embed_train(x, True)
        logits, sv = self._head_fwd(emb, y, True, True)
        saved["head"] = sv
        return logits, saved

    def forward_logits(self, x, y=None):
        x = self._check_input(x)
        m = self.m
        if m.training and torch.is_grad_enabled():
            anchor = m.fc1.bias
            return _LogitsFn.apply(self, x, y, anchor)
        with torch.no_grad():
            if m.training:
                emb, _ = self._embed_train(x, save=False)
                logits, _ = self._head_fwd(emb, y, True, False)
            else:
                emb = self.embed_eval(x)
                logits, _ = self._head_fwd(emb, y, False, False)
            return logits

    def _wgrad(self, x, dy, dw, k, stride, in_affine=None, accumulate=False, dy_amax=None, x_amax=None, dy_presplit=False):
        if not self.use_side_stream:
            return ops.conv_wgrad(x, dy, dw, k, stride, in_affine=in_affine, accumulate=accumulate, dy_amax=dy_amax,
                                  x_amax=x_amax, dy_presplit=dy_presplit)
        if self.wgrad_stream is None:
            self.wgrad_stream = torch.cuda.Stream()
        main = torch.cuda.current_stream()
        side = self.wgrad_stream
        side.wait_stream(main)
        for t in (x, dy):
            t.record_stream(side)
        with torch.cuda.stream(side):
            ops.conv_wgrad(x, dy, dw, k, stride, in_affine=in_affine, accumulate=accumulate, dy_amax=dy_amax, x_amax=x_amax,
                           dy_presplit=dy_presplit)

    def _join_wgrad(self):
        if self.use_side_stream and self.wgrad_stream is not None:
            torch.cuda.current_stream().wait_stream(self.wgrad_stream)

    def backward(self, saved, dlogits, on_stage_done=None):
        m = self.m
        acc = not m.attach_grads()
        if saved.get("gen") != self._fwd_gen:
            raise RuntimeError("backward of a training forward whose BatchNorm statistics rows and operand-scale slots were reused "
                               "by a later training forward (the engine keeps one set per model: run backward before the next "
                               "forward that requires grad)")
        with torch.no_grad():
            demb = self._head_bwd(saved["emb"], saved["head"], dlogits, acc)
            dpooled = ops.linear_bwd(saved["pooled"], m.fc1.weight.data, demb, m.fc1.weight.grad, m.fc1.bias.grad,
                                     accumulate=acc)
            amx = None
            if ops.split_for(3, True) == 3:
                if self._amax_pool is None:
                    self._amax_pool = ops.AmaxPool(dpooled.device)
                amx = self._amax_pool
                amx.reset()
            d_amax = amx.take() if amx else None
            d = ops.stats_pool_bwd(saved["feat"], dpooled, self.pool_mode, amax_out=d_amax)
            if on_stage_done:
                on_stage_done("head")
            nblk = len(self.blocks)
            stage_of = []
            for li in range(1, 5):
                stage_of += [li] * len(getattr(m.res, "layer%d" % li))
            part = None
            last_stage = stage_of[-1]
            for bi in range(nblk - 1, -1, -1):
                if bi > 0:
                    prev = (saved["blocks"][bi - 1]["raws"][-1], self.blocks[bi - 1].bns[-1].t4)
                else:
                    prev = (saved["raw0"], self.stem_bn.t4)
                chan = self.chan_amax and amx is not None and stage_of[bi] == last_stage
                if chan and bi > 0 and stage_of[bi - 1] == last_stage:
                    prev = None
                if bi > 0 and self.blocks[bi - 1].se is not None:
                    prev = None
                d, part, d_amax = self._block_bwd(self.blocks[bi], saved["blocks"][bi], d, acc, part, prev, d_amax, amx, chan)
                saved["blocks"][bi] = None
                if on_stage_done and (bi == 0 or stage_of[bi - 1] != stage_of[bi]):
                    self._join_wgrad()
                    on_stage_done("layer%d" % stage_of[bi])
            bn = self.stem_bn
            if self.stem_fused_bwd:
                raw0 = saved["raw0"]
                if part is None:
                    part = ops.bn_bwd_partial(d, raw0, None, bn.t4, MASK_RAW)
                coef = ops.bn_bwd_coef(part, raw0.numel() // raw0.shape[-1], bn.h.weight.data, bn.t4, bn.h.weight.grad,
                                       bn.h.bias.grad, accumulate=acc)
                ops.stem_bwd_wgrad(saved["x"], d, raw0, bn.t4, coef, self.stem_conv.h.weight.grad, accumulate=acc)
            else:
                draw0 = ops.bn_backward(d, saved["raw0"], None, bn.t4, bn.h.weight.data, bn.h.weight.grad, bn.h.bias.grad,
                                        MASK_RAW, draw_out=d, accumulate=acc, partial=part)
                ops.stem_wgrad(saved["x"], draw0, self.stem_conv.h.weight.grad, accumulate=acc)
            self._join_wgrad()
            if on_stage_done:
                on_stage_done("stem")

    def _block_bwd(self, b, rec, dout, acc, dout_partial=None, prev=None, dout_amax=None, amx=None, chan=False):
        x, raws, out = rec["x"], rec["raws"], rec["out"]
        n = len(b.convs)
        g, g_part, g_amax, dz = dout, dout_partial, dout_amax, None
        take = (lambda: amx.take()) if amx is not None else (lambda: None)
        for i in range(n - 1, -1, -1):
            c, bn, raw = b.convs[i], b.bns[i], raws[i]
            last = i == n - 1
            inp = x if i == 0 else raws[i - 1]
            in_aff = None if i == 0 else (b.bns[i - 1].t4[2], b.bns[i - 1].t4[3])
            hw = (inp.shape[1], inp.shape[2])
            act = out if last else None
            f16 = amx is not None and ops.split_for(c.k, True) == 3
            add_dz, bnb = False, None
            if i > 0:
                if c.stride == 1 and self.fuse_bn_reduce:
                    bnb = (raws[i - 1], None, b.bns[i - 1].t4)
            elif b.ds is None:
                add_dz = True
                if c.stride == 1 and self.fuse_bn_reduce and prev is not None:
                    bnb = (prev[0], x, prev[1])
                    if rec.get("xmask") is not None:
                        bnb = bnb + (rec["xmask"],)
            res_amax, draw_amax = take(), take()
            pairs = f16 and self.pair_draw
            raw_amax = rec["raw_amax"][i] if f16 else None
            se_last = last and b.se is not None
            if not se_last and self.fuse_bn_apply and c.stride == 1 and (self.fuse_apply_min_c <= c.cout <= self.fuse_apply_max_c
                                                                         or (c.k == 1 and self.fuse_apply_1x1)):
                ca = None
                if g_part is None:
                    ca = amx.take_n(c.cout) if (chan and last and f16) else None
                    g_part = ops.bn_bwd_partial(g, raw, act, bn.t4, MASK_ACT if last else MASK_RAW, chan_amax=ca)
                est = take() if f16 else None
                coef = ops.bn_bwd_coef(g_part, raw.numel() // raw.shape[-1], bn.h.weight.data, bn.t4, bn.h.weight.grad,
                                       bn.h.bias.grad, acc, amax_in=g_amax, raw_amax=raw_amax, est_out=est, chan_amax=ca)
                draw = torch.empty_like(raw)
                lazy_dz = b.ds is None and rec.get("mask") is not None and n > 1
                dzb = torch.empty_like(raw) if (last and not lazy_dz) else None
                inb = (raw, act, bn.t4, coef)
                if last and rec.get("mask") is not None:
                    inb = inb + (rec["mask"],)
                if add_dz and lazy_dz:
                    res = ops.conv_dgrad(g, c.wpk_t, c.cin, c.k, 1, hw, add=dout, add_mask=rec["mask"], bn_bwd=bnb,
                                         in_bnbwd=inb, side=(draw, dzb), in_amax=est, out_amax=res_amax, side_amax=draw_amax,
                                         side_presplit=pairs)
                else:
                    res = ops.conv_dgrad(g, c.wpk_t, c.cin, c.k, 1, hw, add=dz if add_dz else None, bn_bwd=bnb,
                                         in_bnbwd=inb, side=(draw, dzb), in_amax=est, out_amax=res_amax, side_amax=draw_amax,
                                         side_presplit=pairs)
                if last:
                    dz = dzb
                draw_slot = est if pairs else draw_amax
                self._count(draw, draw_slot, pairs=pairs)
                if self.bound_log is not None and est is not None:
                    self.bound_log.append((c.cout, c.k, est, draw_amax))
            else:
                lazy_dz = False
                est = take() if pairs else None
                pair = (g_amax, raw_amax, est) if pairs else None
                if se_last:
                    bits = rec.get("mask")
                    lazy_dz = b.ds is None and bits is not None and n > 1
                    ca = amx.take_n(c.cout) if (chan and pairs) else None
                    mode, actm = (MASK_BITS, bits) if bits is not None else (MASK_ACT, out)
                    sums, q, u, gate = rec["se"]
                    S = ops.se_bwd_reduce(g, raw, actm, mode, chan_amax=ca)
                    w1, w2 = b.se.w1, b.se.w2
                    coef, dq, _, _ = ops.se_bwd_gate(S, sums, q, u, gate, w1.data, w2.data, bn.t4, bn.h.weight.data, w1.grad,
                                                     w2.grad, bn.h.weight.grad, bn.h.bias.grad, raw.shape[1] * raw.shape[2],
                                                     accumulate=acc, pair=pair, chan_amax=ca)
                    draw = ops.se_bwd_apply(g, raw, actm, mode, gate, dq[1], bn.t4, coef, e_out=None if lazy_dz else g,
                                            amax_out=draw_amax, pair_scale=est)
                    dz = None if lazy_dz else g
                elif last:
                    bits = rec.get("mask")
                    lazy_dz = b.ds is None and bits is not None and n > 1
                    ca = amx.take_n(c.cout) if (chan and pairs and g_part is None) else None
                    draw = ops.bn_backward(g, raw, bits if bits is not None else out, bn.t4, bn.h.weight.data, bn.h.weight.grad,
                                           bn.h.bias.grad, MASK_BITS if bits is not None else MASK_ACT,
                                           dz_out=None if lazy_dz else g, accumulate=acc, partial=g_part, amax_out=draw_amax,
                                           pair=pair, chan_amax=ca)
                    dz = None if lazy_dz else g
                else:
                    draw = ops.bn_backward(g, raw, None, bn.t4, bn.h.weight.data, bn.h.weight.grad, bn.h.bias.grad, MASK_RAW,
                                           draw_out=g, accumulate=acc, partial=g_part, amax_out=draw_amax, pair=pair)
                draw_slot = est if pairs else draw_amax
                self._count(draw, draw_slot, pairs=pairs)
                if self.bound_log is not None and est is not None:
                    self.bound_log.append((c.cout, c.k, est, draw_amax))
                if add_dz and dz is None and rec.get("mask") is not None:
                    res = ops.conv_dgrad(draw, c.wpk_t, c.cin, c.k, c.stride, hw, add=dout, add_mask=rec["mask"], bn_bwd=bnb,
                                         in_amax=draw_slot if f16 else None, out_amax=res_amax, in_presplit=pairs)
                else:
                    res = ops.conv_dgrad(draw, c.wpk_t, c.cin, c.k, c.stride, hw, add=dz if add_dz else None, bn_bwd=bnb,
                                         in_amax=draw_slot if f16 else None, out_amax=res_amax, in_presplit=pairs)
            g, g_part = res if bnb is not None else (res, None)
            g_amax = res_amax
            self._wgrad(inp, draw, c.h.weight.grad, c.k, c.stride, in_affine=in_aff, accumulate=acc,
                        dy_amax=draw_slot if f16 else None, x_amax=rec["in_amax"][i] if f16 else None, dy_presplit=pairs)
        dx, part, dx_amax = g, g_part, g_amax
        if b.ds is not None:
            cd, bnd = b.ds
            f16d = amx is not None and ops.split_for(1, True) == 3
            drawd_amax = take() if f16d else None
            drawd = ops.bn_backward(dz, rec["rawd"], None, bnd.t4, bnd.h.weight.data, bnd.h.weight.grad, bnd.h.bias.grad,
                                    MASK_NONE, draw_out=dz, accumulate=acc, amax_out=drawd_amax)
            self._count(drawd, drawd_amax)
            self._wgrad(x, drawd, cd.h.weight.grad, 1, cd.stride, accumulate=acc, dy_amax=drawd_amax,
                        x_amax=rec["in_amax"][0] if f16d else None)
            ops.conv_dgrad(drawd, cd.wpk_t, cd.cin, 1, cd.stride, (x.shape[1], x.shape[2]), out=dx, accumulate=True,
                           in_amax=drawd_amax, out_amax=dx_amax)
            part = None
        return dx, part, dx_amax

    def loss_and_grad(self, x, y, on_stage_done=None):
        x = self._check_input(x)
        y = y.contiguous()
        with torch.no_grad():
            logits, saved = self.forward_train(x, y)
            loss_row, dl, rank = ops.softmax_ce(logits, y, grad_scale=1.0 / logits.shape[0])
            loss = ops.mean(loss_row)
        self.backward(saved, dl, on_stage_done)
        return loss, logits, rank


STAGE_ORDER = ["head", "layer4", "layer3", "layer2", "layer1", "stem"]


class GraphedTrainStep:

    def __init__(self, engine, batch, frames, warmup=2, side_stream=None, segmented=False, pool=None):
        import os
        if side_stream is None:
            side_stream = os.environ.get("SPK_GRAPH_SIDE", "0") == "1"
        m = engine.m
        dev = m.flat_parameters().device
        self.eng = engine
        side, engine.use_side_stream = engine.use_side_stream, bool(side_stream)
        self.x = torch.zeros(batch, m.feat_dim, frames, device=dev)
        self.y = torch.zeros(batch, dtype=torch.long, device=dev)
        self.shape = (batch, m.feat_dim, frames)
        saved_buffers = [b.clone() for b in m.buffers()]
        s = torch.cuda.Stream()
        s.wait_stream(torch.cuda.current_stream())
        with torch.cuda.stream(s):
            for _ in range(warmup):
                for p in m.parameters():
                    p.grad = None
                engine.loss_and_grad(self.x, self.y)
        torch.cuda.current_stream().wait_stream(s)
        torch.cuda.synchronize()
        for b, sb in zip(m.buffers(), saved_buffers):
            b.copy_(sb)
        for p in m.parameters():
            p.grad = None
        engine.dirty = True
        self.segments = []
        cap = {"g": None, "ctx": None}

        def begin():
            g = torch.cuda.CUDAGraph()
            kw = {"pool": self.segments[0][0].pool()} if self.segments else ({"pool": pool} if pool is not None else {})
            ctx = torch.cuda.graph(g, capture_error_mode="thread_local", **kw)
            ctx.__enter__()
            cap["g"], cap["ctx"] = g, ctx

        def end(name):
            cap["ctx"].__exit__(None, None, None)
            self.segments.append((cap["g"], name))
            cap["g"] = cap["ctx"] = None

        def cut(name):
            end(name)
            if name != STAGE_ORDER[-1]:
                begin()

        begin()
        try:
            self.loss, self.logits, self.rank = engine.loss_and_grad(self.x, self.y, cut if segmented else None)
            if cap["ctx"] is not None:
                end(None)
        except BaseException:
            if cap["ctx"] is not None:
                cap["ctx"].__exit__(None, None, None)
            raise
        self.graph = self.segments[0][0]
        assert [n for _, n in self.segments] == (STAGE_ORDER if segmented else [None])
        self.pack_table = engine._pack_tables.get(True)
        assert self.pack_table is not None and self.pack_table.launches_captured >= 1, \
            "the captured training step does not contain the conv-weight re-pack"
        engine.dirty = True
        engine.use_side_stream = side

    def matches(self, x):
        return tuple(x.shape) == self.shape

    def pool(self):
        return self.segments[0][0].pool()

    def __call__(self, x, y, on_stage_done=None):
        self.x.copy_(x, non_blocking=True)
        self.y.copy_(y, non_blocking=True)
        for g, name in self.segments:
            g.replay()
            if name is not None and on_stage_done is not None:
                on_stage_done(name)
        self.eng.dirty, self.eng._packed_for_bwd = False, True
        self.eng.m.attach_grads()
        return self.loss, self.logits, self.rank


class GraphedStepCache:

    def __init__(self, engine, segmented=False, max_graphs=64, warmup=2):
        self.eng, self.segmented, self.max_graphs, self.warmup = engine, segmented, max_graphs, warmup
        self.steps = {}
        self._pool_owner = None
        self.captures = 0

    def get(self, batch, frames):
        key = (int(batch), int(frames))
        st = self.steps.pop(key, None)
        if st is None:
            pool = self._pool_owner.pool() if self._pool_owner is not None else None
            st = GraphedTrainStep(self.eng, key[0], key[1], warmup=self.warmup, segmented=self.segmented, pool=pool)
            if self._pool_owner is None:
                self._pool_owner = st
            self.captures += 1
            while len(self.steps) >= self.max_graphs:
                old = next(iter(self.steps))
                if self.steps[old] is self._pool_owner:
                    self.steps[old] = self.steps.pop(old)
                    if len(self.steps) == 1:
                        break
                    continue
                del self.steps[old]
        self.steps[key] = st
        return st

    def __call__(self, x, y, on_stage_done=None):
        return self.get(x.shape[0], x.shape[2])(x, y, on_stage_done)

    def __len__(self):
        return len(self.steps)
```

### pytorch-kaldi-resnet_amd/hip.py

```python
import ctypes
import os

import torch

_HERE = os.path.dirname(os.path.abspath(__file__))
LIB_PATH = os.environ.get("SPK_LIB", os.path.join(_HERE, "libspkhip.so"))

IN_AFFINE_RELU, EPI_AFFINE, EPI_ADD, EPI_RELU, EPI_STATS, EPI_BNBWD, IN_BNBWD, CONV_WS = 1, 2, 4, 8, 16, 32, 64, 128
CONV_PIPE = 1024
WGRAD_GROUPS = 2048
IN_PRESPLIT, SIDE_PRESPLIT, DY_PRESPLIT = 1 << 14, 1 << 15, 1 << 16
CONV_M16 = 1 << 17
CONV_CK32 = 1 << 23
WGRAD_NOSHIFT = 1 << 18
WGRAD_M16 = 1 << 19
EPI_WMASK = 1 << 24
PTR_ADD_MASK, PTR_BN_MASK, PTR_IN_MASK, PTR_IN_ACT, PTR_BN_ACT, PTR_SIDE_DZ = 1, 2, 4, 8, 16, 32
MASK_NONE, MASK_ACT, MASK_RAW, MASK_BITS = 0, 1, 2, 3

_P = ctypes.c_void_p
_I = ctypes.c_int
_L = ctypes.c_longlong
_F = ctypes.c_float
_D = ctypes.c_double
_IP = ctypes.POINTER(ctypes.c_int)

_SIGS = {
    "spk_pack_conv_weight": [_P, _P, _I, _I, _I, _I, _I, _P],
    "spk_pack_conv_weight_split": [_P, _P, _I, _I, _I, _I, _I, _I, _P],
    "spk_pack_job_bytes": [],
    "spk_build_flags": [],
    "spk_pack_conv_weights_batched": [_P, _I, _I, _I, _P],
    "spk_conv_mfma": [_P] * 21 + [_I] * 14 + [_IP, _IP, _IP] + [_I] * 8 + [_P, _P, _P, _P],
    "spk_conv_mfma_len": [_P] * 21 + [_I] * 14 + [_IP, _IP, _IP] + [_I] * 8 + [_P, _P, _P, _P, _P],
    "spk_conv3x3_c32_stream": [_P] * 6 + [_I] * 4 + [_P, _P, _I, _P],
    "spk_conv1x1_stream": [_P] * 11 + [_L, _I, _I, _P, _P, _I, _P],
    "spk_conv1x1_stream_rows": [_I, _I],
    "spk_conv_wgrad": [_P] * 6 + [_I] * 16 + [_P, _P, _P],
    "spk_conv_wgrad_limits": [_I, _IP, _IP],
    "spk_wgrad_reduce": [_P, _P, _I, _I, _I, _I, _I, _P],
    "spk_conv_variant_of": [_I, _I, _I, _I, _I],
    "spk_wgrad_variant_of": [_I, _I, _I, _I, _I, _I, _I],
    "spk_stem_fwd_blocks": [_I, _I, _I],
    "spk_stem_conv_fwd": [_P] * 6 + [_I] * 4 + [_P, _P],
    "spk_stem_conv_fwd_len": [_P] * 6 + [_I] * 4 + [_P, _P, _P],
    "spk_stem_wgrad_blocks": [_I, _I, _I],
    "spk_stem_conv_wgrad": [_P] * 4 + [_I] * 4 + [_P],
    "spk_stem_stats": [_P] * 3 + [_I] * 3 + [_P],
    "spk_stem_fwd_apply": [_P] * 8 + [_I] * 3 + [_P],
    "spk_stem_bwd_wgrad": [_P] * 10 + [_I] * 4 + [_P],
    "spk_bn_stats_blocks": [_L, _I],
    "spk_bn_stats_partial": [_P, _P, _L, _I, _P],
    "spk_bn_finalize": [_P, _I, _I, _D] + [_P] * 9 + [_F, _F, _P, _P, _P, _P],
    "spk_bn_eval_coeffs": [_P] * 6 + [_I, _F, _P],
    "spk_bn_apply": [_P] * 8 + [_L, _I, _I, _P, _P],
    "spk_bn_bwd_reduce": [_P] * 8 + [_L, _I, _I, _P, _P],
    "spk_bn_bwd_finalize": [_P, _I, _I, _D] + [_P] * 5 + [_I, _P, _P, _P, _P, _P, _P, _P],
    "spk_bn_bwd_apply": [_P] * 10 + [_L, _I, _I, _P, _P, _P],
    "spk_absmax": [_P, _P, _L, _P],
    "spk_bnbwd_estimate": [_P, _P, _P, _I, _P, _P, _P, _P],
    "spk_f16_window_count": [_P, _P, _P, _L, _I, _P, _I, _P, _P],
    "spk_affine_estimate": [_P, _P, _I, _P, _P, _P],
    "spk_se_chunks": [_L],
    "spk_se_squeeze": [_P, _P, _P, _I, _I, _I, _I, _P, _P],
    "spk_se_excite": [_P] * 8 + [_I] * 5 + [_P, _P],
    "spk_se_apply": [_P] * 9 + [_I] * 5 + [_P, _P, _P],
    "spk_se_bwd_reduce": [_P] * 5 + [_I, _L, _I, _I, _P, _P],
    "spk_se_bwd_gate": [_P] * 20 + [_I] * 4 + [_L] + [_P] * 5,
    "spk_se_bwd_apply": [_P] * 10 + [_I, _L, _I, _I, _P, _P, _P],
    "spk_stats_pool_fwd": [_P, _P, _I, _I, _I, _I, _I, _P],
    "spk_stats_pool_fwd_len": [_P, _P, _P, _I, _I, _I, _I, _I, _P],
    "spk_stats_pool_bwd": [_P, _P, _P, _I, _I, _I, _I, _I, _P, _P],
    "spk_stats_pool_row_form": [_I],
    "spk_stats_pool_row_cap": [],
    "spk_gemm_f32": [_P] * 4 + [_I] * 3 + [_L] * 5 + [_F, _I, _P, _P],
    "spk_gemm_splitk": [_I, _I, _I],
    "spk_colsum": [_P, _P, _I, _I, _I, _P],
    "spk_l2norm_fwd": [_P, _P, _P, _I, _I, _F, _P],
    "spk_l2norm_bwd": [_P, _P, _P, _P, _I, _I, _F, _I, _P],
    "spk_aam_margin_fwd": [_P, _P, _P, _I, _I, _F, _F, _P],
    "spk_aam_margin_bwd": [_P, _P, _P, _P, _I, _I, _F, _F, _P],
    "spk_softmax_ce": [_P] * 5 + [_I, _I, _F, _P],
    "spk_mean": [_P, _P, _I, _P],
    "spk_relu_bwd": [_P, _P, _P, _L, _P],
    "spk_sgd_step": [_P, _P, _P, _L, _F, _F, _F, _F, _I, _P],
    "spk_center_normalize": [_P, _P, _P, _I, _I, _F, _P],
    "spk_trial_cosine": [_P, _P, _P, _P, _P, _I, _I, _I, _I, _P],
    "spk_topk_mean_std": [_P, _P, _P, _I, _I, _I, _L, _P],
    "spk_fbank_tile_frames": [_I, _I, _I, _I],
    "spk_fbank_fwd": [_P, _P, _P, _I, _L] + [_P] * 5 + [_I] * 5 + [_F, _F, _I, _F, ctypes.c_ulonglong, _P, _P, _P, _I, _P],
    "spk_mfcc_tile_frames": [_I, _I, _I, _I, _I],
    "spk_mfcc_fwd": [_P, _P, _P, _I, _L] + [_P] * 7 + [_I] * 6 + [_F, _F, _I, _F, _I, _I, ctypes.c_ulonglong, _P, _P, _P, _I, _P],
    "spk_fbank_span_fwd": [_P] * 7 + [_I, _L] + [_P] * 5 + [_I] * 5 + [_F, _F, _I, _F, ctypes.c_ulonglong, _P, _P, _P, _I, _P],
    "spk_mfcc_span_fwd": [_P] * 7 + [_I, _L] + [_P] * 7 + [_I] * 6 + [_F, _F, _I, _F, _I, _I, ctypes.c_ulonglong, _P, _P, _P, _I, _P],
    "spk_pcm16_to_f32": [_P, _P, _I, _L, _P, _P],
    "spk_fbank_dither_noise":[_P, _L, ctypes.c_ulonglong, _I, _I, _I, _P],
    "spk_vad_count": [_P, _P, _I, _I, _D, _D, _I, _D, _P, _P, _P, _P],
    "spk_cmn_select": [_P] * 6 + [_I] * 5 + [_P],
    "spk_resample_tile": [_I, _I, _I],
    "spk_resample_fwd": [_P, _P, _I, _L, _P, _P, _I, _I, _I, _P, _P, _L, _P],
    "spk_augment_max_rir": [],
    "spk_augment_max_early": [],
    "spk_augment_workspace": [_I, _L, _I, _I, _L, _I, ctypes.POINTER(_L)],
    "spk_cm_decode": [_P, _P, _P, _I, _I, _I, _P, _P],
    "spk_cm_compress": [_P, _P, _I, _I, _I, _P, _P, _P, _P, _P],
    "spk_eval_tile": [_I],
    "spk_segment_mean": [_P, _P, _P, _P, _I, _I, _I, _P],
    "spk_trial_snorm": [_P, _I] + [_P] * 7 + [_I, _P],
    "spk_sort_trials": [_P, _P, _P, _I, _P],
    "spk_error_sweep": [_P, _P, _P, _P, _I, _P, _P, _P, _I, _P],
    "spk_scatter_slab_rows": [_L],
    "spk_scatter_f64": [_P, _I, _L, _P, _P, _P, _P, _L, _I, _P],
    "spk_segment_sum_f64": [_P, _I, _L, _P, _P, _P, _P, _I, _I, _I, _P],
    "spk_affine_lennorm": [_P, _I, _L, _P, _P, _P, _I, _P, _I, _L, _I, _I, _P],
    "spk_plda_posterior_rows": [_P] * 5 + [_I, _I, _P],
    "spk_plda_llr": [_P] * 8 + [_I, _P, _I, _I, _I, _I, _P],
    "spk_augment_fwd": [_P, _P, _I, _L, _P, _L, _P, _P, _I, _I, _P, _L, _P, _P, _P, _P, _I, _L, _P, _P, _P, _P, _I, _P, _P, _P],
}

_lib = None


def lib():
    global _lib
    if _lib is None:
        if not os.path.exists(LIB_PATH) and "SPK_LIB" not in os.environ:
            try:
                import importlib.util
                spec = importlib.util.spec_from_file_location("spk_build", os.path.join(_HERE, "build.py"))
                mod = importlib.util.module_from_spec(spec)
                spec.loader.exec_module(mod)
                mod.build(force=True, verbose=False)
            except Exception as e:
                raise RuntimeError("libspkhip.so is missing at %s and building it failed (%s). Run `python "
                                   "__graft_entry__.py build` (hipcc --offload-arch=gfx950). There is no fallback path."
                                   % (LIB_PATH, e))
        if not os.path.exists(LIB_PATH):
            raise RuntimeError(
                "libspkhip.so is missing at %s: run `python __graft_entry__.py build` "
                "(hipcc --offload-arch=gfx950). There is no fallback path." % LIB_PATH)
        l = ctypes.CDLL(LIB_PATH)
        l.spk_last_error.restype = ctypes.c_char_p
        l.spk_version.restype = ctypes.c_int
        l.spk_conv_wgrad_workspace.restype = ctypes.c_size_t
        l.spk_conv_wgrad_workspace.argtypes = [_I, _I, _I, _I]
        l.spk_bn_finalize_workspace.restype = ctypes.c_size_t
        l.spk_bn_finalize_workspace.argtypes = [_I, _I]
        l.spk_gemm_workspace.restype = ctypes.c_size_t
        l.spk_gemm_workspace.argtypes = [_I, _I, _I]
        l.spk_sort_trials_workspace.restype = ctypes.c_size_t
        l.spk_sort_trials_workspace.argtypes = [_I]
        l.spk_error_sweep_workspace.restype = ctypes.c_size_t
        l.spk_error_sweep_workspace.argtypes = [_I, _I]
        l.spk_scatter_f64_workspace.restype = ctypes.c_size_t
        l.spk_scatter_f64_workspace.argtypes = [_L, _I]
        for name, sig in _SIGS.items():
            fn = getattr(l, name)
            fn.argtypes = sig
            fn.restype = ctypes.c_int
        if os.environ.get("SPK_POOL_ROWS", "1") == "0":
            l.spk_stats_pool_row_form(0)
        _lib = l
    return _lib


def has_experimental():
    return bool(lib().spk_build_flags() & 1)


def exported_symbols():
    return ["spk_version", "spk_last_error", "spk_conv_wgrad_workspace", "spk_bn_finalize_workspace", "spk_gemm_workspace",
            "spk_sort_trials_workspace", "spk_error_sweep_workspace", "spk_scatter_f64_workspace"] + list(_SIGS)


def ptr(t):
    if t is None:
        return None
    assert t.is_cuda, "libspkhip takes device tensors only"
    assert t.is_contiguous(), "libspkhip takes contiguous tensors only"
    return t.data_ptr()


def stream():
    return torch.cuda.current_stream().cuda_stream


def check(rc, name):
    if rc != 0:
        msg = lib().spk_last_error().decode()
        raise RuntimeError("%s failed (rc=%d): %s" % (name, rc, msg))


def call(name, *args):
    rc = getattr(lib(), name)(*args)
    check(rc, name)
```

### pytorch-kaldi-resnet_amd/ops.py

```python
import collections
import ctypes
import os

import torch

from . import hip, tiling
from .hip import (CONV_CK32, CONV_M16, CONV_PIPE, CONV_WS, DY_PRESPLIT, IN_PRESPLIT, SIDE_PRESPLIT, WGRAD_GROUPS, EPI_ADD, EPI_AFFINE, EPI_BNBWD, EPI_RELU,
                  EPI_STATS, EPI_WMASK, IN_AFFINE_RELU, IN_BNBWD, MASK_ACT, MASK_NONE, MASK_RAW,
                  call, ptr, stream)

BN_EPS = 1e-5
BN_MOMENTUM = 0.1

PROFILE = None
_raw_call = call


def call(name, *args, label=None, flops=0.0, nbytes=0.0):
    if PROFILE is None:
        return _raw_call(name, *args)
    e0 = torch.cuda.Event(enable_timing=True)
    e1 = torch.cuda.Event(enable_timing=True)
    e0.record()
    _raw_call(name, *args)
    e1.record()
    PROFILE.append((label or name, flops, e0, e1, nbytes))


def _iarr(v):
    return (ctypes.c_int * len(v))(*v)


class AmaxPool:

    def __init__(self, device, n=4096):
        self.table = torch.zeros(n, device=device, dtype=torch.int32)
        self.next = 0

    def take_n(self, n):
        i = self.next
        assert i + n <= self.table.numel(), "AmaxPool exhausted"
        self.next = i + n
        return self.table[i:i + n]

    def reset(self):
        self.table.zero_()
        self.next = 0

    def take(self):
        i = self.next
        assert i < self.table.numel(), "AmaxPool exhausted"
        self.next = i + 1
        return self.table[i:i + 1]


def absmax_into(t, slot):
    call("spk_absmax", ptr(t), ptr(slot), t.numel(), stream())
    return slot


def affine_estimate(scale, shift, amax_in, est):
    call("spk_affine_estimate", ptr(scale), ptr(shift), scale.numel(), ptr(amax_in), ptr(est), stream())
    return est


def _amax_fwd_fallback(x, in_affine):
    slot = absmax_into(x, torch.zeros(1, device=x.device, dtype=torch.int32))
    if in_affine is None:
        return slot
    return affine_estimate(in_affine[0], in_affine[1], slot, torch.zeros(1, device=x.device, dtype=torch.int32))


def bnbwd_estimate(coef, bn4, amax_in, raw_amax, est=None):
    if est is None:
        est = torch.zeros(1, device=coef.device, dtype=torch.int32)
    call("spk_bnbwd_estimate", ptr(coef), ptr(bn4[0]), ptr(bn4[1]), coef.shape[1], ptr(amax_in), ptr(raw_amax), ptr(est), stream())
    return est


def _amax_fallback(dy, in_bnbwd):
    slot = torch.zeros(1, device=dy.device, dtype=torch.int32)
    absmax_into(dy, slot)
    if in_bnbwd is None:
        return slot
    raw_slot = absmax_into(in_bnbwd[0], torch.zeros(1, device=dy.device, dtype=torch.int32))
    return bnbwd_estimate(in_bnbwd[3], in_bnbwd[2], slot, raw_slot)


def f16_window_count(x, slot, counts, affine=None, pairs=False):
    C = x.shape[-1]
    call("spk_f16_window_count", ptr(x), ptr(affine[0]) if affine else None, ptr(affine[1]) if affine else None, x.numel(), C,
         ptr(slot), 1 if pairs else 0, ptr(counts), stream())
    return counts


def conv_out_hw(h, w, ksize, stride):
    pad = 1 if ksize == 3 else 0
    return (h + 2 * pad - ksize) // stride + 1, (w + 2 * pad - ksize) // stride + 1


MFMA_MODES = {"f32": 0, "bf16x6": 6, "bf16x9": 9, "f16x3": 3}
SPLIT = MFMA_MODES[os.environ.get("SPK_MFMA", "f16x3")]
SPLIT_BWD = MFMA_MODES[os.environ["SPK_MFMA_BWD"]] if os.environ.get("SPK_MFMA_BWD") else None


WS_CONV = os.environ.get("SPK_CONV_WS", "auto")
assert WS_CONV in ("0", "1", "auto"), "SPK_CONV_WS must be 0, 1 or auto"
WS_AUTO_MIN_COUT = 128
PIPE_CONV = os.environ.get("SPK_CONV_PIPE", "1") == "1"
PIPE_M16 = os.environ.get("SPK_PIPE_M16", "1") == "1"
PIPE_WGRAD = os.environ.get("SPK_WGRAD_PIPE", "0") == "1"
PIPE_BNBWD = os.environ.get("SPK_PIPE_BNBWD", "0") == "1"
GROUPED_1X1 = os.environ.get("SPK_WGRAD_1X1_GROUPS", "1") == "1"
WM16 = os.environ.get("SPK_WM16", "1") == "1"
C32M16 = os.environ.get("SPK_C32M16", "1") == "1"
WM_SHIFT = os.environ.get("SPK_WM_SHIFT", "1") == "1"
GROUPED_3X3 = os.environ.get("SPK_WGRAD_3X3_GROUPS", "1") == "1"
GROUPED_1X1_BLOCKS = int(os.environ.get("SPK_WGRAD_1X1_BLOCKS", "512"))
C32_PLANE = int(os.environ.get("SPK_C32_PLANE", "32"))
assert C32_PLANE in (16, 32), "SPK_C32_PLANE: 16 or 32"
C32_PLANE_TILES = ((2, 1), (1, 1))
PIPE_MIN_CIN = int(os.environ.get("SPK_PIPE_MIN_CIN", "64"))
PIPE_MAX_LDS = int(os.environ.get("SPK_PIPE_MAX_LDS", str(80 * 1024)))
PIPE_TILES = ((2, 1), (3, 1), (1, 2), (2, 2), (3, 2), (1, 4))
WS_WGRAD = os.environ.get("SPK_WGRAD_WS", "0") == "1"
WS_WGRAD_BLOCKS = int(os.environ.get("SPK_WGRAD_WS_BLOCKS", "256"))
WS_MIN_TAPS = int(os.environ.get("SPK_WS_MIN_TAPS", "9"))
LABEL_SHAPES = os.environ.get("SPK_LABEL_SHAPES", "0") == "1"
WS_FORCE = None


def _experimental():
    return hip.has_experimental()


SPLIT_1X1 = os.environ.get("SPK_SPLIT_1X1", "1") == "1"
KC_CANDIDATES = tuple(int(v) for v in os.environ.get("SPK_KC", "4,2").split(","))


def split_for(ksize, bwd=False):
    mode = SPLIT_BWD if (bwd and SPLIT_BWD is not None) else SPLIT
    if ksize == 3:
        return mode
    return 3 if (mode == 3 and SPLIT_1X1 and ksize == 1) else 0


def pack_conv_weight(w, transpose=False, out=None):
    Cout, Cin, KH, KW = w.shape
    split = split_for(KH, bwd=transpose)
    n = packed_numel(w, bwd=transpose)
    if out is None or out.numel() != n:
        out = torch.empty(n, device=w.device, dtype=torch.float32)
    if split:
        call("spk_pack_conv_weight_split", ptr(w), ptr(out), Cout, Cin, KH, KW, 1 if transpose else 0, split, stream(),
             label="spk_pack_conv_weight")
    else:
        call("spk_pack_conv_weight", ptr(w), ptr(out), Cout, Cin, KH, KW, 1 if transpose else 0, stream(),
             label="spk_pack_conv_weight")
    return out


def packed_numel(w, bwd=False):
    sp = split_for(w.shape[2], bwd)
    return w.numel() * 3 // 2 if sp in (6, 9) else (w.numel() + 4 if sp == 3 else w.numel())


class PackTable:

    def __init__(self, jobs, device):
        import struct
        assert hip.lib().spk_pack_job_bytes() == 48
        blob, block0 = b"", 0
        self.key = []
        for w, wpk, transpose in jobs:
            Cout, Cin, KH, KW = w.shape
            split = split_for(KH, bwd=transpose)
            assert wpk.numel() == packed_numel(w, bwd=transpose) and w.is_contiguous()
            blob += struct.pack("<QQ8i", w.data_ptr(), wpk.data_ptr(), Cout, Cin, KH * KW, 1 if transpose else 0, split,
                                w.numel(), block0, 0)
            block0 += (w.numel() + 255) // 256
            self.key.append((w.data_ptr(), wpk.data_ptr(), transpose, split))
        self.njobs, self.blocks = len(jobs), block0
        self.has_f16 = any(k[3] == 3 for k in self.key)
        self.table = torch.frombuffer(bytearray(blob), dtype=torch.uint8).to(device)
        self.launches = 0
        self.launches_captured = 0

    def run(self):
        self.launches += 1
        if torch.cuda.is_current_stream_capturing():
            self.launches_captured += 1
        call("spk_pack_conv_weights_batched", ptr(self.table), self.njobs, self.blocks, 1 if self.has_f16 else 0, stream(),
             label="spk_pack_conv_weight")


STREAM_1X1 = os.environ.get("SPK_STREAM_1X1", "1") == "1"
STREAM_1X1_BLOCKS = int(os.environ.get("SPK_STREAM_1X1_BLOCKS", "512"))
STREAM_C32 = os.environ.get("SPK_STREAM_C32", "1") == "1"
STREAM_C32_BLOCKS = int(os.environ.get("SPK_STREAM_C32_BLOCKS", "512"))
FWD_TAPS = tuple((kh - 1, kw - 1, kh * 3 + kw) for kh in range(3) for kw in range(3))

ConvPlan = collections.namedtuple("ConvPlan", "entry flags label nblocks stats_rows key TH TW MT NT WC kc ips IS",
                                  defaults=(None,) * 9 + (1, 1))
WgradPlan = collections.namedtuple("WgradPlan", "TH TW WN family cg nsplit flags label")


def _mask_form(t, n):
    return None if t is None else "sign" if len(t) > n else "raw" if t[1] is None else "act"


def _plan_conv(B, IH, IW, Cin, OH, OW, OHf, OWf, Cout, taps, IS, OS, ooy, oox, split, experimental, in_affine=False,
               epi_affine=False, epi_add=False, relu=False, want_stats=False, bn_bwd=None, in_bnbwd=None, side=False,
               add_mask=False, in_presplit=False, side_presplit=False, wlen=False, out_is_x=False):
    ntaps = len(taps)
    dys, dxs = [t[0] for t in taps], [t[1] for t in taps]
    want_stats = want_stats or bn_bwd is not None
    flags = ((IN_AFFINE_RELU if in_affine else 0) | (IN_PRESPLIT if in_presplit else 0) | (SIDE_PRESPLIT if side_presplit else 0)
             | (EPI_AFFINE if epi_affine else 0) | (EPI_ADD if epi_add else 0) | (EPI_RELU if relu else 0)
             | (IN_BNBWD if in_bnbwd is not None else 0) | (EPI_BNBWD if bn_bwd is not None else 0) | (EPI_WMASK if wlen else 0)
             | (EPI_STATS if want_stats else 0))
    shape = " C%d %dx%d" % (Cout, OH, OW) if LABEL_SHAPES else ""
    same_map = (not wlen and split == 3 and IS == 1 and OS == 1 and ooy == 0 and oox == 0 and (IH, IW) == (OH, OW) == (OHf, OWf)
                and in_bnbwd is None and not side and not epi_affine and not relu and not side_presplit)
    stream_c32 = (STREAM_C32 and same_map and Cin == 32 and Cout == 32 and want_stats and bn_bwd is None and not epi_add
                  and not in_presplit and not add_mask and tuple(taps) == FWD_TAPS and B * OH * OW * 32 < 2 ** 31 - 65536)
    if stream_c32:
        nblocks = max(1, min(STREAM_C32_BLOCKS, B * (-(-IH // 8)) * (-(-IW // 16))))
        return ConvPlan("spk_conv3x3_c32_stream", flags, "conv3x3_c32_stream_kernel" + shape, nblocks, 4 * nblocks)
    stream_1x1 = (STREAM_1X1 and same_map and ntaps == 1 and dys[0] == 0 and dxs[0] == 0 and Cin == Cout and Cin in (32, 64, 128)
                  and not out_is_x and bn_bwd != "act" and B * OH * OW * Cin < 2 ** 31)
    if stream_1x1:
        tp = 64 * (1 if Cin >= 128 else (2 if Cin == 64 else 4))
        nblocks = max(1, min(STREAM_1X1_BLOCKS, -(-(B * IH * IW) // tp)))
        return ConvPlan("spk_conv1x1_stream", flags, "conv1x1_stream_kernel<%d>" % Cin + shape, nblocks)
    ips = 1
    if ntaps == 1 and IS > 1 and dys[0] == 0 and dxs[0] == 0:
        ips, IS = IS, 1
    key = (OH, OW, IS, max(dys) - min(dys) + 1, max(dxs) - min(dxs) + 1, ntaps, Cout)
    c32 = C32_PLANE == 32 and split == 3 and Cin == 32 and in_bnbwd is not None and ntaps == 9
    TH, TW, MT, NT = tiling.conv_tile(*key, mode=(2 if c32 else 1) if in_bnbwd is not None else 0, split=split)
    pipe_fused = (PIPE_CONV and PIPE_BNBWD and split == 3 and in_bnbwd == "sign" and MT * NT <= 4 and Cout <= 128
                  and WS_FORCE is None and WS_CONV != "1" and not side_presplit)
    ws_on = (WS_CONV == "1" or WS_FORCE is not None or (
        WS_CONV == "auto" and experimental and split == 3 and in_bnbwd is not None and Cout >= WS_AUTO_MIN_COUT and not pipe_fused))
    ws, WC = None, 1
    if split and ws_on and not side_presplit and not in_presplit and ntaps >= WS_MIN_TAPS and ips == 1:
        ws = WS_FORCE or tiling.ws_tile(*key)
    if ws is not None:
        TH, TW, MT, NT, WC = ws
        flags |= CONV_WS | ({1: 0, 2: 1, 4: 2}[WC] << 8)
    kc = 1
    if ntaps == 1:
        halo = ((TH - 1) * IS + 1) * ((TW - 1) * IS + 1)
        kc = next((c for c in KC_CANDIDATES if Cin % (32 * c) == 0 and c * halo * tiling.LDS_PIX_BYTES <= tiling.LDS_HARD), 1)
    halo9 = ((TH - 1) * IS + key[3]) * ((TW - 1) * IS + key[4])
    pipe = (PIPE_CONV and ws is None and split == 3 and ntaps == 9 and kc == 1 and (in_bnbwd is None or pipe_fused) and halo9 <= 576
            and (2 * halo9 + 1) * 80 <= PIPE_MAX_LDS and Cin >= PIPE_MIN_CIN and (MT, NT) in PIPE_TILES)
    m16 = pipe and PIPE_M16 and in_bnbwd is None and (MT, NT) == (3, 2) and halo9 <= 512 and IS == 1
    c32 = c32 and ws is None and not pipe and kc == 1 and (MT, NT) in C32_PLANE_TILES
    flags |= (CONV_PIPE if pipe else 0) | (CONV_M16 if m16 else 0) | (CONV_CK32 if c32 else 0)
    fused = "true" if in_bnbwd is not None else "false"
    if ws is not None:
        label = "conv_ws_kernel<%d,%d,%d,%s,%d>" % (MT, NT, WC, fused, split)
    elif pipe and in_bnbwd is not None:
        label = "conv_pipe_kernel<%d,%d,true,true>" % (MT, NT)
    elif pipe:
        pair = ",true" if in_presplit else (",false" if m16 else "")
        label = "conv_pipe_kernel<%d,%d,false,false%s%s>" % (MT, NT, pair, ",true" if m16 else "")
    else:
        label = "conv_mfma_kernel<%d,%d,%s,%d>" % (MT, NT, fused, split)
    if LABEL_SHAPES and c32:
        shape += " plane32"
    rows = (4 // WC) * B * (-(-OH // TH)) * (-(-OW // TW))
    return ConvPlan("spk_conv_mfma_len" if wlen else "spk_conv_mfma", flags, label + shape, None, rows, key,
                    TH, TW, MT, NT, WC, kc, ips, IS)


def _conv_launch(x, wpk, out, Cout, taps, IS, OS, ooy, oox, OH, OW, in_affine, epi_affine, epi_add, relu, want_stats,
                 bn_bwd=None, in_bnbwd=None, side=None, split=0, add_mask=None, in_amax=None, out_amax=None, side_amax=None,
                 in_presplit=False, side_presplit=False, wlen=None):
    B, IH, IW, Cin = x.shape
    OHf, OWf = out.shape[1], out.shape[2]
    pa = (B, IH, IW, Cin, OH, OW, OHf, OWf, Cout, taps, IS, OS, ooy, oox, split, _experimental(), in_affine is not None,
          epi_affine is not None, epi_add is not None, relu, want_stats, _mask_form(bn_bwd, 3), _mask_form(in_bnbwd, 4),
          side is not None, add_mask is not None, in_presplit, side_presplit, wlen is not None, out is x)
    if tiling.AUTOTUNE and PROFILE is None and not torch.cuda.is_current_stream_capturing():
        p = _plan_conv(*pa)
        if p.key is not None and p.key not in (tiling.FORCE_CONV_SPLIT if split else tiling.FORCE_CONV):
            _autotune_conv(p.key, x, wpk, out, Cout, taps, p.IS, OS, ooy, oox, OH, OW, in_affine, epi_affine, epi_add, relu, split,
                           in_amax=in_amax, in_presplit=in_presplit)
    p = _plan_conv(*pa)
    if wlen is not None:
        _check_wlen(wlen, B)
    assert not in_presplit or (split == 3 and in_affine is None and in_bnbwd is None), "f16 pair input: f16x3 mode, plain input"
    assert not side_presplit or (split == 3 and in_bnbwd is not None), "f16 pair side output: fused BatchNorm-backward data gradient in the f16x3 mode"
    assert epi_add is None or epi_add.shape == out.shape
    in_mask = in_bnbwd[4] if (in_bnbwd is not None and len(in_bnbwd) > 4) else None
    bn_mask = bn_bwd[3] if (bn_bwd is not None and len(bn_bwd) > 3) else None
    for mk, ref in ((in_mask, x), (bn_mask, out), (add_mask, out)):
        if mk is not None:
            assert mk.dtype == torch.int32 and mk.numel() == ref.numel() // 32, "sign mask shape"
    if in_bnbwd is not None:
        assert in_affine is None and side is not None and side[0].shape == x.shape
        assert in_bnbwd[0].shape == x.shape and (in_bnbwd[1] is None or in_bnbwd[1].shape == x.shape)
    if bn_bwd is not None:
        assert bn_bwd[0].shape == out.shape and (bn_bwd[1] is None or bn_bwd[1].shape == out.shape)
    stats = None
    if p.flags & EPI_STATS:
        rows = p.stats_rows if p.stats_rows is not None else hip.lib().spk_conv1x1_stream_rows(p.nblocks, Cin)
        stats = torch.empty(rows, Cout, 2, device=x.device, dtype=torch.float32)
    in_aff = (ptr(in_affine[0]), ptr(in_affine[1])) if in_affine else (None, None)
    bn_raw, bn4 = (ptr(bn_bwd[0]), ptr(bn_bwd[2])) if bn_bwd else (None, None)
    if p.entry == "spk_conv3x3_c32_stream":
        args = (*in_aff, ptr(stats), B, IH, IW, p.flags, ptr(in_amax), ptr(out_amax), p.nblocks)
    elif p.entry == "spk_conv1x1_stream":
        args = (*in_aff, ptr(epi_add), ptr(add_mask), bn_raw, ptr(bn_mask), bn4, ptr(stats), B * IH * IW, Cin, p.flags,
                ptr(in_amax), ptr(out_amax), p.nblocks)
    else:
        args = (*in_aff, ptr(epi_affine[0]) if epi_affine else None, ptr(epi_affine[1]) if epi_affine else None, ptr(epi_add),
                ptr(in_bnbwd[0]) if in_bnbwd else None, ptr(in_bnbwd[1]) if (in_bnbwd and in_mask is None) else None,
                ptr(in_bnbwd[2]) if in_bnbwd else None, ptr(in_bnbwd[3]) if in_bnbwd else None,
                ptr(in_mask), ptr(bn_mask), ptr(add_mask), ptr(side[0]) if side else None, ptr(side[1]) if side else None,
                bn_raw, ptr(bn_bwd[1]) if (bn_bwd and bn_mask is None) else None, bn4, ptr(stats),
                B, IH, IW, Cin, OH, OW, OHf, OWf, Cout, p.IS, OS, ooy, oox, len(taps),
                _iarr([t[0] for t in taps]), _iarr([t[1] for t in taps]), _iarr([t[2] for t in taps]),
                p.TH, p.TW, p.MT, p.NT, p.kc, p.ips, p.flags, split, ptr(in_amax), ptr(out_amax), ptr(side_amax),
                *(() if wlen is None else (ptr(wlen),)))
    ips, eff_is = p.ips, p.IS
    call(p.entry, ptr(x), ptr(wpk), ptr(out), *args, stream(), label=p.label,
         flops=2.0 * B * OH * OW * Cout * Cin * len(taps),
         nbytes=4.0 * (B * (IH // ips) * (IW // ips) * Cin * (min(1.0, len(taps) * OH * OW / max(1, (IH // ips) * (IW // ips))) if eff_is == 1 and OS > 1 else 1.0)
                       + B * OH * OW * Cout * (1 + (1 if epi_add is not None else 0) + (1 if bn_bwd is not None else 0))
                       + (2 * x.numel() if in_bnbwd is not None else 0)
                       + (x.numel() / 32 if in_mask is not None else 0) + (B * OH * OW * Cout / 32) * ((bn_mask is not None) + (add_mask is not None))
                       + wpk.numel()))
    return stats


def _check_wlen(wlen, B):
    if not (wlen.is_cuda and wlen.dtype == torch.int32 and wlen.dim() == 1 and wlen.numel() == B and wlen.is_contiguous()):
        raise RuntimeError("wlen must be a contiguous int32 device tensor [%d], got %s %s %s" % (B, wlen.dtype, tuple(wlen.shape), wlen.device))


def _time_launch(fn, reps=2):
    fn()
    e0, e1 = torch.cuda.Event(enable_timing=True), torch.cuda.Event(enable_timing=True)
    e0.record()
    for _ in range(reps):
        fn()
    e1.record()
    e1.synchronize()
    return e0.elapsed_time(e1) / reps


def _autotune_conv(key, x, wpk, out, Cout, taps, IS, OS, ooy, oox, OH, OW, in_affine, epi_affine, epi_add, relu, split=0,
                   in_amax=None, in_presplit=False):
    scratch = torch.empty_like(out)
    if split == 3 and in_amax is None:
        in_amax = _amax_fwd_fallback(x, in_affine)
    add = epi_add if (epi_add is None or epi_add.data_ptr() != out.data_ptr()) else scratch
    best = None
    table = tiling.FORCE_CONV_SPLIT if split else tiling.FORCE_CONV
    for cand in tiling.conv_candidates(*key, split=split):
        table[key] = cand
        try:
            ms = _time_launch(lambda: _conv_launch(x, wpk, scratch, Cout, taps, IS, OS, ooy, oox, OH, OW, in_affine,
                                                   epi_affine, add, relu, True, split=split, in_amax=in_amax,
                                                   in_presplit=in_presplit))
        except RuntimeError:
            continue
        if best is None or ms < best[0]:
            best = (ms, cand)
    if best is None:
        del table[key]
    else:
        table[key] = best[1]


def _autotune_wgrad(key, x, dy, ksize, stride, in_affine, dy_amax=None, x_amax=None, dy_presplit=False):
    scratch = torch.empty(dy.shape[3], x.shape[3], ksize, ksize, device=x.device, dtype=torch.float32)
    best = None
    for cand in tiling.wgrad_candidates(*key):
        tiling.FORCE_WGRAD[key] = cand
        try:
            ms = _time_launch(lambda: conv_wgrad(x, dy, scratch, ksize, stride, in_affine=in_affine, dy_amax=dy_amax,
                                                 x_amax=x_amax, dy_presplit=dy_presplit))
        except RuntimeError:
            continue
        if best is None or ms < best[0]:
            best = (ms, cand)
    if best is None:
        del tiling.FORCE_WGRAD[key]
    else:
        tiling.FORCE_WGRAD[key] = best[1]


def conv_fwd(x, wpk, Cout, ksize, stride, in_affine=None, epi_affine=None, epi_add=None, relu=False, stats=False,
             out=None, in_amax=None, out_amax=None, wlen=None):
    B, IH, IW, Cin = x.shape
    if split_for(ksize) == 3 and in_amax is None:
        in_amax = _amax_fwd_fallback(x, in_affine)
    OH, OW = conv_out_hw(IH, IW, ksize, stride)
    if out is None:
        out = torch.empty(B, OH, OW, Cout, device=x.device, dtype=torch.float32)
    taps = FWD_TAPS if ksize == 3 else [(0, 0, 0)]
    st = _conv_launch(x, wpk, out, Cout, taps, stride, 1, 0, 0, OH, OW, in_affine, epi_affine, epi_add, relu, stats,
                      split=split_for(ksize), in_amax=in_amax, out_amax=out_amax, wlen=wlen)
    return out, st


def conv_dgrad(dy, wpk_t, Cin, ksize, stride, in_hw, add=None, out=None, accumulate=False, bn_bwd=None, in_bnbwd=None,
               side=None, add_mask=None, in_amax=None, out_amax=None, side_amax=None, in_presplit=False, side_presplit=False):
    B, OH, OW, Cout = dy.shape
    assert not in_presplit or in_amax is not None, "an f16 pair tensor comes with its scale slot"
    if split_for(ksize, True) == 3 and in_amax is None:
        in_amax = _amax_fallback(dy, in_bnbwd)
    IH, IW = in_hw
    if out is None:
        assert not accumulate
        out = torch.empty(B, IH, IW, Cin, device=dy.device, dtype=torch.float32)
    if accumulate:
        assert add is None
        add = out
    if stride == 1:
        if ksize == 3:
            taps = [(1 - kh, 1 - kw, kh * 3 + kw) for kh in range(3) for kw in range(3)]
        else:
            taps = [(0, 0, 0)]
        st = _conv_launch(dy, wpk_t, out, Cin, taps, 1, 1, 0, 0, IH, IW, None, None, add, False, False, bn_bwd, in_bnbwd,
                          side, split=split_for(ksize, True), add_mask=add_mask, in_amax=in_amax, out_amax=out_amax,
                          side_amax=side_amax, in_presplit=in_presplit, side_presplit=side_presplit)
        return (out, st) if bn_bwd is not None else out
    assert stride == 2 and bn_bwd is None and in_bnbwd is None and add_mask is None
    if ksize == 1:
        if not accumulate:
            if add is not None:
                out.copy_(add)
            else:
                out.zero_()
        _conv_launch(dy, wpk_t, out, Cin, [(0, 0, 0)], 1, 2, 0, 0, (IH + 1) // 2, (IW + 1) // 2, None, None, out, False,
                     False, split=split_for(1, True), in_amax=in_amax, out_amax=out_amax, in_presplit=in_presplit)
        return out
    for cy in range(2):
        for cx in range(2):
            LH, LW = (IH - cy + 1) // 2, (IW - cx + 1) // 2
            if LH <= 0 or LW <= 0:
                continue
            taps = []
            for kh in range(3):
                if (cy + 1 - kh) % 2:
                    continue
                for kw in range(3):
                    if (cx + 1 - kw) % 2:
                        continue
                    taps.append(((cy + 1 - kh) // 2, (cx + 1 - kw) // 2, kh * 3 + kw))
            _conv_launch(dy, wpk_t, out, Cin, taps, 1, 2, cy, cx, LH, LW, None, None, add, False, False, split=split_for(3, True),
                         in_amax=in_amax, out_amax=out_amax, in_presplit=in_presplit)
    return out


_ws_cache = {}
_ws_retired = []


def _workspace(nbytes, device, name=None):
    key = (name, str(device), torch.cuda.current_stream().cuda_stream)
    w = _ws_cache.get(key)
    if w is None or w.numel() * 4 < nbytes:
        if w is not None:
            _ws_retired.append(w)
        w = torch.empty((nbytes + 3) // 4, device=device, dtype=torch.float32)
        _ws_cache[key] = w
    return w


def _plan_wgrad(B, Cin, OH, OW, Cout, ksize, stride, split, in_affine=False, dy_presplit=False):
    TH, TW, WN = tiling.wgrad_tile(OH, OW, Cin, Cout, ksize, stride, split=split)
    f16_3x3 = split == 3 and ksize == 3
    if C32M16 and f16_3x3 and WN == 1 and dy_presplit:
        TH, TW, WN = tiling.c32m16_tile(OH, OW, Cin, Cout, ksize, stride) or (TH, TW, WN)
    nreg = B * (-(-OH // TH)) * (-(-OW // TW))
    halo = ((TH - 1) * stride + ksize) * ((TW - 1) * stride + ksize)
    wv, hs = 4 // WN, 4 if halo <= 128 else 5
    nst = -(-(TH * TW) // 16)
    cg = 0
    if WS_WGRAD and f16_3x3 and not dy_presplit and 2 * (halo * 192 + nst * 16 * (WN * 192 + (64 if WN > 1 else 0))) <= 160 * 1024:
        family, label = "ws", "conv_wgrad_ws_kernel<%d,%d,%d,%d>" % (ksize * ksize, wv, WN, hs)
    elif (PIPE_WGRAD and f16_3x3 and not dy_presplit and nst % wv == 0 and nst // wv in (1, 2)
          and 2 * (2 * halo * 64 + 2 * WN * nst * 16 * 64) + 128 <= PIPE_MAX_LDS):
        family, label = "pipe", "conv_wgrad_pipe_kernel<%d,%d,%d,%d>" % (wv, WN, hs, nst // wv)
    elif (GROUPED_3X3 and f16_3x3 and WN == 2 and Cin % 64 == 0 and Cout % 64 == 0 and halo <= 112 and TH * TW <= 64
          and halo * 384 + nst * 16 * 448 <= 80 * 1024):
        m16 = WM16 and dy_presplit and halo * 416 + 2 * -(-(TH * TW) // 32) * 32 * 256 <= 80 * 1024
        family, label, cg = ("wm16", "conv_wgrad_wm16_kernel", 2) if m16 else ("wm", "conv_wgrad_wm_kernel", 2)
    elif (C32M16 and f16_3x3 and WN == 1 and dy_presplit and halo <= 192
          and halo * 192 + 2 * -(-(TH * TW) // 32) * 32 * 128 <= 80 * 1024):
        family, label = "c32m16", "conv_wgrad_c32m16_kernel"
    else:
        family = "split" if split else "f32"
        label = ("conv_wgrad_split_kernel<%d,%d,%d,%d,%d>" % (ksize * ksize, wv, WN, split, hs) if split
                 else "conv_wgrad_kernel<%d,%d,%d>" % (ksize * ksize, wv, WN))
    if GROUPED_1X1 and split == 3 and ksize == 1 and WN in (2, 4) and TH * TW <= 64:
        cg = 4 if Cin % 128 == 0 else (2 if Cin % 64 == 0 else 0)
        if cg and nst * 16 * (cg * 192 + WN * 192 + 64) > 80 * 1024:
            cg = 2 if cg == 4 else 0
        if cg:
            family, label = "1x1", "conv_wgrad_1x1_kernel<%d,%d,%d>" % (wv, WN, cg)
    nsplit = min(nreg, tiling.wgrad_nsplit(nreg, Cin, Cout, WN, WS_WGRAD_BLOCKS if family == "ws" else (GROUPED_1X1_BLOCKS if cg else None),
                                           cin_groups=cg or 1))
    flags = ((IN_AFFINE_RELU if in_affine else 0) | (CONV_WS if family == "ws" else 0) | (CONV_PIPE if family == "pipe" else 0)
             | (WGRAD_GROUPS | ({2: 1, 4: 2}[cg] << 12) if cg else 0) | (DY_PRESPLIT if dy_presplit else 0)
             | (hip.WGRAD_NOSHIFT if family in ("wm", "wm16") and not WM_SHIFT else 0)
             | (hip.WGRAD_M16 if family in ("wm16", "c32m16") else 0))
    return WgradPlan(TH, TW, WN, family, cg, nsplit, flags, label + (" C%d %dx%d" % (Cout, OH, OW) if LABEL_SHAPES else ""))


def conv_wgrad(x, dy, dw, ksize, stride, in_affine=None, accumulate=False, dy_amax=None, x_amax=None, dy_presplit=False):
    B, IH, IW, Cin = x.shape
    _, OH, OW, Cout = dy.shape
    split = split_for(ksize, True)
    assert not dy_presplit or (split == 3 and dy_amax is not None), "an f16 pair tensor comes with its scale slot (f16x3 mode)"
    if split == 3 and dy_amax is None:
        dy_amax = absmax_into(dy, torch.zeros(1, device=dy.device, dtype=torch.int32))
    if split == 3 and x_amax is None:
        x_amax = _amax_fwd_fallback(x, in_affine)
    wkey = (OH, OW, Cin, Cout, ksize, stride)
    if tiling.AUTOTUNE and wkey not in tiling.FORCE_WGRAD and PROFILE is None and not torch.cuda.is_current_stream_capturing():
        tiling.FORCE_WGRAD[wkey] = tiling._wgrad_tile(*wkey)
        _autotune_wgrad(wkey, x, dy, ksize, stride, in_affine, dy_amax, x_amax, dy_presplit)
    p = _plan_wgrad(B, Cin, OH, OW, Cout, ksize, stride, split, in_affine is not None, dy_presplit)
    nbytes = hip.lib().spk_conv_wgrad_workspace(p.nsplit, ksize, Cin, Cout)
    ws = _workspace(nbytes, x.device)
    call("spk_conv_wgrad", ptr(x), ptr(dy), ptr(dw), ptr(ws),
         ptr(in_affine[0]) if in_affine else None, ptr(in_affine[1]) if in_affine else None,
         B, IH, IW, Cin, OH, OW, Cout, ksize, stride, p.TH, p.TW, p.WN, p.nsplit, p.flags, 1 if accumulate else 0, split,
         ptr(dy_amax) if split == 3 else None, ptr(x_amax) if split == 3 else None, stream(), label=p.label,
         flops=2.0 * B * OH * OW * Cout * Cin * ksize * ksize, nbytes=4.0 * (x.numel() + dy.numel() + nbytes / 4))
    call("spk_wgrad_reduce", ptr(ws), ptr(dw), p.nsplit, ksize, Cin, Cout, 1 if accumulate else 0, stream())
    return dw


def stem_fwd(x, w, epi_affine=None, relu=False, stats=False, amax_out=None, wlen=None):
    B, F, T = x.shape
    out = torch.empty(B, F, T, 32, device=x.device, dtype=torch.float32)
    flags = (EPI_AFFINE if epi_affine is not None else 0) | (EPI_RELU if relu else 0) | (EPI_STATS if stats else 0)
    st = None
    if stats:
        st = torch.empty(hip.lib().spk_stem_fwd_blocks(B, F, T), 32, 2, device=x.device, dtype=torch.float32)
    args = (ptr(x), ptr(w), ptr(out), ptr(st), ptr(epi_affine[0]) if epi_affine else None,
            ptr(epi_affine[1]) if epi_affine else None, B, F, T)
    if wlen is None:
        call("spk_stem_conv_fwd", *args, flags, ptr(amax_out), stream())
    else:
        _check_wlen(wlen, B)
        call("spk_stem_conv_fwd_len", *args, flags | EPI_WMASK, ptr(amax_out), ptr(wlen), stream())
    return out, st


def stem_wgrad(x, draw, dw, accumulate=False):
    B, F, T = x.shape
    nblk = hip.lib().spk_stem_wgrad_blocks(B, F, T)
    ws = _workspace(nblk * 288 * 4, x.device)
    call("spk_stem_conv_wgrad", ptr(x), ptr(draw), ptr(dw), ptr(ws), B, F, T, 1 if accumulate else 0, stream())
    return dw


def stem_stats(x, w):
    B, F, T = x.shape
    st = torch.empty(hip.lib().spk_stem_fwd_blocks(B, F, T), 32, 2, device=x.device, dtype=torch.float32)
    call("spk_stem_stats", ptr(x), ptr(w), ptr(st), B, F, T, stream(), nbytes=4.0 * x.numel())
    return st


def stem_fwd_apply(x, w, scale, shift, mask=False, amax_out=None):
    B, F, T = x.shape
    raw = torch.empty(B, F, T, 32, device=x.device, dtype=torch.float32)
    act = torch.empty_like(raw)
    mk = torch.empty(B * F * T, device=x.device, dtype=torch.int32) if mask else None
    call("spk_stem_fwd_apply", ptr(x), ptr(w), ptr(scale), ptr(shift), ptr(raw), ptr(act), ptr(mk), ptr(amax_out), B, F, T,
         stream(), nbytes=4.0 * (x.numel() + 2 * raw.numel()) + (raw.numel() / 8 if mask else 0))
    return raw, act, mk


def stem_bwd_wgrad(x, d, raw, bn4, coef, dw, accumulate=False):
    B, F, T = x.shape
    nblk = hip.lib().spk_stem_wgrad_blocks(B, F, T)
    ws = _workspace(nblk * 288 * 4, x.device)
    call("spk_stem_bwd_wgrad", ptr(x), ptr(d), ptr(raw), ptr(bn4[0]), ptr(bn4[1]), ptr(bn4[2]), ptr(bn4[3]), ptr(coef), ptr(dw),
         ptr(ws), B, F, T, 1 if accumulate else 0, stream(), nbytes=4.0 * (x.numel() + 2 * raw.numel()))
    return dw


def bn_stats_partial(x2d):
    N, C = x2d.shape
    nblk = hip.lib().spk_bn_stats_blocks(N, C)
    part = torch.empty(nblk, C, 2, device=x2d.device, dtype=torch.float32)
    call("spk_bn_stats_partial", ptr(x2d), ptr(part), N, C, stream())
    return part


_ws64_cache = {}


def _ws64(device):
    w = _ws64_cache.get(str(device))
    if w is None:
        w = torch.zeros(256 * 2048 * 2 + 64, device=device, dtype=torch.float64)
        _ws64_cache[str(device)] = w
    return w


def bn_finalize(partial, count, gamma, beta, running_mean, running_var, nbt, out4, amax_in=None, est_out=None):
    C = gamma.numel()
    call("spk_bn_finalize", ptr(partial), partial.shape[0], C, float(count), ptr(gamma), ptr(beta), ptr(running_mean),
         ptr(running_var), ptr(nbt), ptr(out4[0]), ptr(out4[1]), ptr(out4[2]), ptr(out4[3]), BN_MOMENTUM, BN_EPS,
         ptr(_ws64(partial.device)), ptr(amax_in), ptr(est_out), stream())


def bn_eval_coeffs(gamma, beta, rm, rv, out2):
    C = gamma.numel()
    call("spk_bn_eval_coeffs", ptr(gamma), ptr(beta), ptr(rm), ptr(rv), ptr(out2[0]), ptr(out2[1]), C, BN_EPS, stream())


def bn_apply(raw, scale, shift, res=None, res_affine=None, relu=True, out=None, mask=False, amax_out=None):
    C = raw.shape[-1]
    N = raw.numel() // C
    if out is None:
        out = torch.empty_like(raw)
    mk = torch.empty(N * (C // 32), device=raw.device, dtype=torch.int32) if mask else None
    call("spk_bn_apply", ptr(raw), ptr(scale), ptr(shift), ptr(res),
         ptr(res_affine[0]) if res_affine else None, ptr(res_affine[1]) if res_affine else None, ptr(out), ptr(mk), N, C,
         1 if relu else 0, ptr(amax_out), stream(),
         nbytes=4.0 * raw.numel() * (2 + (1 if res is not None else 0)) + (raw.numel() / 8 if mask else 0))
    return (out, mk) if mask else out


def _bn_bwd_bytes(raw, mask_mode, passes):
    n = raw.numel()
    return 4.0 * n * passes + {MASK_NONE: 0.0, MASK_RAW: 0.0, MASK_ACT: 4.0 * n}.get(mask_mode, n / 8.0)


def bn_backward(dy, raw, act, bn4, gamma, dgamma, dbeta, mask_mode, draw_out=None, dz_out=None, accumulate=False,
                partial=None, amax_out=None, pair=None, chan_amax=None):
    C = raw.shape[-1]
    N = raw.numel() // C
    coef = torch.empty(3, C, device=raw.device, dtype=torch.float32)
    if partial is None:
        nblk = hip.lib().spk_bn_stats_blocks(N, C)
        part = torch.empty(nblk, C, 2, device=raw.device, dtype=torch.float32)
        call("spk_bn_bwd_reduce", ptr(dy), ptr(raw), ptr(act), ptr(bn4[0]), ptr(bn4[1]), ptr(bn4[2]), ptr(bn4[3]), ptr(part),
             N, C, mask_mode, ptr(chan_amax), stream(), nbytes=_bn_bwd_bytes(raw, mask_mode, 2))
    else:
        assert chan_amax is None, "chan_amax comes out of the reduction pass: partial must be None"
        part, nblk = partial, partial.shape[0]
    call("spk_bn_bwd_finalize", ptr(part), nblk, C, float(N), ptr(gamma), ptr(bn4[1]), ptr(dgamma), ptr(dbeta), ptr(coef),
         1 if accumulate else 0, ptr(_ws64(raw.device)), ptr(pair[0]) if pair else None, ptr(pair[1]) if pair else None,
         ptr(bn4[0]) if pair else None, ptr(pair[2]) if pair else None, ptr(chan_amax) if pair else None, stream())
    if draw_out is None:
        draw_out = torch.empty_like(raw)
    call("spk_bn_bwd_apply", ptr(dy), ptr(raw), ptr(act), ptr(bn4[0]), ptr(bn4[1]), ptr(bn4[2]), ptr(bn4[3]), ptr(coef),
         ptr(draw_out), ptr(dz_out), N, C, mask_mode, ptr(amax_out), ptr(pair[2]) if pair else None, stream(),
         nbytes=_bn_bwd_bytes(raw, mask_mode, 3 + (1 if dz_out is not None else 0)))
    return draw_out


def bn_bwd_coef(partial, count, gamma, bn4, dgamma, dbeta, accumulate=False, amax_in=None, raw_amax=None, est_out=None,
                chan_amax=None):
    C = gamma.numel()
    coef = torch.empty(3, C, device=gamma.device, dtype=torch.float32)
    assert est_out is None or (amax_in is not None and raw_amax is not None)
    call("spk_bn_bwd_finalize", ptr(partial), partial.shape[0], C, float(count), ptr(gamma), ptr(bn4[1]), ptr(dgamma),
         ptr(dbeta), ptr(coef), 1 if accumulate else 0, ptr(_ws64(gamma.device)), ptr(amax_in) if est_out is not None else None,
         ptr(raw_amax) if est_out is not None else None, ptr(bn4[0]) if est_out is not None else None, ptr(est_out),
         ptr(chan_amax) if est_out is not None else None, stream())
    return coef


def bn_bwd_partial(dy, raw, act, bn4, mask_mode, chan_amax=None):
    C = raw.shape[-1]
    N = raw.numel() // C
    nblk = hip.lib().spk_bn_stats_blocks(N, C)
    part = torch.empty(nblk, C, 2, device=raw.device, dtype=torch.float32)
    call("spk_bn_bwd_reduce", ptr(dy), ptr(raw), ptr(act), ptr(bn4[0]), ptr(bn4[1]), ptr(bn4[2]), ptr(bn4[3]), ptr(part),
         N, C, mask_mode, ptr(chan_amax), stream(), nbytes=_bn_bwd_bytes(raw, mask_mode, 2))
    return part


def se_squeeze(x, wlen=None):
    B, H, W, C = x.shape
    if wlen is not None:
        _check_wlen(wlen, B)
    part = torch.empty(B * hip.lib().spk_se_chunks(H * W) * C, device=x.device, dtype=torch.float32)
    sums = torch.empty(B, C, device=x.device, dtype=torch.float64)
    call("spk_se_squeeze", ptr(x), ptr(part), ptr(sums), B, H, W, C, ptr(wlen), stream(), nbytes=4.0 * x.numel())
    return sums


def se_excite(sums, affine, w1, w2, H, W, wlen=None):
    B, C = sums.shape
    Cr = w1.shape[0]
    assert tuple(w1.shape) == (Cr, C) and tuple(w2.shape) == (C, Cr)
    q = torch.empty(B, C, device=sums.device, dtype=torch.float32)
    u = torch.empty(B, Cr, device=sums.device, dtype=torch.float32)
    g = torch.empty(B, C, device=sums.device, dtype=torch.float32)
    call("spk_se_excite", ptr(sums), ptr(affine[0]) if affine else None, ptr(affine[1]) if affine else None, ptr(w1), ptr(w2),
         ptr(q), ptr(u), ptr(g), B, C, Cr, H, W, ptr(wlen), stream())
    return q, u, g


def se_apply(raw, affine, gate, res=None, res_affine=None, relu=True, mask=False, amax_out=None, wlen=None, out=None):
    B, H, W, C = raw.shape
    if wlen is not None:
        _check_wlen(wlen, B)
    if out is None:
        out = torch.empty_like(raw)
    mk = torch.empty(B * H * W * (C // 32), device=raw.device, dtype=torch.int32) if mask else None
    call("spk_se_apply", ptr(raw), ptr(affine[0]) if affine else None, ptr(affine[1]) if affine else None, ptr(gate), ptr(res),
         ptr(res_affine[0]) if res_affine else None, ptr(res_affine[1]) if res_affine else None, ptr(out), ptr(mk), B, H, W, C,
         1 if relu else 0, ptr(amax_out), ptr(wlen), stream(),
         nbytes=4.0 * raw.numel() * (2 + (1 if res is not None else 0)) + (raw.numel() / 8 if mask else 0))
    return (out, mk) if mask else out


def se_bwd_reduce(dout, raw, act, mask_mode, chan_amax=None):
    B, H, W, C = raw.shape
    part = torch.empty(B * hip.lib().spk_se_chunks(H * W) * 2 * C, device=raw.device, dtype=torch.float32)
    S = torch.empty(B, 2, C, device=raw.device, dtype=torch.float64)
    call("spk_se_bwd_reduce", ptr(dout), ptr(raw), ptr(act), ptr(part), ptr(S), B, H * W, C, mask_mode, ptr(chan_amax), stream(),
         nbytes=_bn_bwd_bytes(raw, mask_mode, 2))
    return S


def se_bwd_gate(S, sums, q, u, g, w1, w2, bn4, gamma, dw1, dw2, dgamma, dbeta, HW, accumulate=False, pair=None, chan_amax=None):
    B, C = q.shape
    Cr = u.shape[1]
    dev = q.device
    coef = torch.empty(3, C, device=dev, dtype=torch.float32)
    dq = torch.empty(2, B, C, device=dev, dtype=torch.float32)
    da = torch.empty(B, C, device=dev, dtype=torch.float32)
    du = torch.empty(B, Cr, device=dev, dtype=torch.float32)
    call("spk_se_bwd_gate", ptr(S), ptr(sums), ptr(q), ptr(u), ptr(g), ptr(w1), ptr(w2), ptr(bn4[0]), ptr(bn4[1]), ptr(bn4[2]),
         ptr(bn4[3]), ptr(gamma), ptr(da), ptr(du), ptr(dq), ptr(dw1), ptr(dw2), ptr(dgamma), ptr(dbeta), ptr(coef),
         1 if accumulate else 0, B, C, Cr, HW, ptr(pair[0]) if pair else None, ptr(pair[1]) if pair else None,
         ptr(chan_amax) if pair else None, ptr(pair[2]) if pair else None, stream())
    return coef, dq, da, du


def se_bwd_apply(dout, raw, act, mask_mode, g, dqs, bn4, coef, e_out=None, amax_out=None, pair_scale=None, draw_out=None):
    B, H, W, C = raw.shape
    if draw_out is None:
        draw_out = torch.empty_like(raw)
    call("spk_se_bwd_apply", ptr(dout), ptr(raw), ptr(act), ptr(g), ptr(dqs), ptr(bn4[0]), ptr(bn4[1]), ptr(coef), ptr(draw_out),
         ptr(e_out), B, H * W, C, mask_mode, ptr(amax_out), ptr(pair_scale), stream(),
         nbytes=_bn_bwd_bytes(raw, mask_mode, 3 + (1 if e_out is not None else 0)))
    return draw_out


def stats_pool_fwd(x, mode, wlen=None):
    B, H, W, C = x.shape
    out = torch.empty(B, C * H * (2 if mode else 1), device=x.device, dtype=torch.float32)
    if wlen is None:
        call("spk_stats_pool_fwd", ptr(x), ptr(out), B, H, W, C, mode, stream())
    else:
        _check_wlen(wlen, B)
        call("spk_stats_pool_fwd_len", ptr(x), ptr(out), ptr(wlen), B, H, W, C, mode, stream())
    return out


def stats_pool_bwd(x, gout, mode, amax_out=None):
    B, H, W, C = x.shape
    dx = torch.empty_like(x)
    call("spk_stats_pool_bwd", ptr(x), ptr(gout), ptr(dx), B, H, W, C, mode, ptr(amax_out), stream())
    return dx


def _ptr_rows(t):
    assert t.is_cuda and t.dim() == 2 and (t.stride(1) == 1 or t.shape[1] == 1) and t.stride(0) >= t.shape[1], \
        "libspkhip takes rows of unit stride only"
    return t.data_ptr()


def gemm(A, Bm, M, N, K, sam, sak, sbk, sbn, bias=None, out=None, alpha=1.0, accumulate=False):
    if out is None:
        out = torch.empty(M, N, device=A.device, dtype=torch.float32)
    ws = _workspace(hip.lib().spk_gemm_workspace(M, N, K), A.device, name="gemm")
    call("spk_gemm_f32", ptr(A), ptr(Bm), _ptr_rows(out), ptr(bias), M, N, K, sam, sak, sbk, sbn, out.stride(0), float(alpha),
         1 if accumulate else 0, ptr(ws), stream(), label="gemm_f32_kernel", flops=2.0 * M * N * K)
    return out


def linear_fwd(x, w, bias=None):
    M, K = x.shape
    N = w.shape[0]
    return gemm(x, w, M, N, K, K, 1, 1, K, bias=bias)


def linear_bwd(x, w, dy, dw, db=None, need_dx=True, accumulate=False):
    M, K = x.shape
    N = w.shape[0]
    dx = None
    if need_dx:
        dx = gemm(dy, w, M, K, N, N, 1, K, 1)
    gemm(dy, x, N, K, M, 1, N, K, 1, out=dw, accumulate=accumulate)
    if db is not None:
        call("spk_colsum", ptr(dy), ptr(db), M, N, 1 if accumulate else 0, stream())
    return dx


def l2norm_fwd(x):
    R, D = x.shape
    y = torch.empty_like(x)
    inv = torch.empty(R, device=x.device, dtype=torch.float32)
    call("spk_l2norm_fwd", ptr(x), ptr(y), ptr(inv), R, D, 1e-12, stream())
    return y, inv


def l2norm_bwd(y, inv, dy, out=None, accumulate=False):
    R, D = y.shape
    if out is None:
        out = torch.empty_like(y)
    call("spk_l2norm_bwd", ptr(y), ptr(inv), ptr(dy), ptr(out), R, D, 1e-12, 1 if accumulate else 0, stream())
    return out


def aam_margin_fwd(cosv, label, m, s):
    B, S = cosv.shape
    logits = torch.empty_like(cosv)
    call("spk_aam_margin_fwd", ptr(cosv), ptr(label), ptr(logits), B, S, float(m), float(s), stream())
    return logits


def aam_margin_bwd(cosv, label, dlogits, m, s):
    B, S = cosv.shape
    dcos = torch.empty_like(cosv)
    call("spk_aam_margin_bwd", ptr(cosv), ptr(label), ptr(dlogits), ptr(dcos), B, S, float(m), float(s), stream())
    return dcos


def softmax_ce(logits, label, grad_scale=None, want_rank=True):
    B, S = logits.shape
    loss_row = torch.empty(B, device=logits.device, dtype=torch.float32)
    dl = torch.empty_like(logits) if grad_scale is not None else None
    rank = torch.empty(B, device=logits.device, dtype=torch.int32) if want_rank else None
    call("spk_softmax_ce", ptr(logits), ptr(label), ptr(loss_row), ptr(dl), ptr(rank), B, S,
         float(grad_scale if grad_scale is not None else 0.0), stream())
    return loss_row, dl, rank


def mean(v):
    out = torch.empty(1, device=v.device, dtype=torch.float32)
    call("spk_mean", ptr(v), ptr(out), v.numel(), stream())
    return out


def relu_bwd(y, dy):
    dx = torch.empty_like(dy)
    call("spk_relu_bwd", ptr(y), ptr(dy), ptr(dx), y.numel(), stream())
    return dx


def sgd_step(p, g, buf, lr, momentum, weight_decay, grad_scale, first):
    call("spk_sgd_step", ptr(p), ptr(g), ptr(buf), p.numel(), float(lr), float(momentum), float(weight_decay),
         float(grad_scale), 1 if first else 0, stream())


def center_normalize(emb, mean=None, eps=1e-8):
    N, D = emb.shape
    out = torch.empty_like(emb)
    call("spk_center_normalize", ptr(emb), ptr(mean), ptr(out), N, D, float(eps), stream())
    return out


def trial_cosine(en, te, ia, ib):
    T = ia.numel()
    out = torch.empty(T, device=en.device, dtype=torch.float32)
    assert ia.dtype == torch.int32 and ib.dtype == torch.int32 and ib.numel() == T and en.shape[1] == te.shape[1]
    call("spk_trial_cosine", ptr(en), ptr(te), ptr(ia), ptr(ib), ptr(out), T, en.shape[1], en.shape[0], te.shape[0], stream())
    return out


def topk_mean_std(scores, k):
    N, M = scores.shape
    mean = torch.empty(N, device=scores.device, dtype=torch.float32)
    std = torch.empty_like(mean)
    call("spk_topk_mean_std", _ptr_rows(scores), ptr(mean), ptr(std), N, M, int(k), scores.stride(0), stream())
    return mean, std


def sort_tile():
    return hip.lib().spk_eval_tile(0)


def sweep_block():
    return hip.lib().spk_eval_tile(1)


def segment_mean(emb, rows, seg_off):
    N, D = emb.shape
    S = seg_off.numel() - 1
    assert emb.dtype == torch.float64 and rows.dtype == torch.int32 and seg_off.dtype == torch.int32 and rows.numel() == N
    out = torch.empty(S, D, device=emb.device, dtype=torch.float32)
    call("spk_segment_mean", ptr(emb), ptr(rows), ptr(seg_off), ptr(out), N, S, D, stream())
    return out


def trial_snorm(score, ia, ib, e_mean, e_std, t_mean, t_std):
    T = score.numel()
    assert score.dtype in (torch.float32, torch.float64) and ia.dtype == torch.int32 and ib.dtype == torch.int32
    assert ia.numel() == T and ib.numel() == T and all(t.dtype == torch.float64 for t in (e_mean, e_std, t_mean, t_std))
    out = torch.empty(T, device=score.device, dtype=torch.float64)
    call("spk_trial_snorm", ptr(score), 1 if score.dtype == torch.float64 else 0, ptr(ia), ptr(ib), ptr(e_mean), ptr(e_std),
         ptr(t_mean), ptr(t_std), ptr(out), T, stream())
    return out


def sort_trials(score):
    T = score.numel()
    assert score.dtype == torch.float64 and score.dim() == 1
    if T < 1 or T >= 1 << 31:
        raise ValueError("sort_trials: T=%d must lie in [1, 2^31)" % T)
    if bool(torch.isnan(score).any()):
        raise ValueError("sort_trials: a score is NaN")
    order = torch.empty(T, device=score.device, dtype=torch.int32)
    ws = torch.empty(hip.lib().spk_sort_trials_workspace(T), device=score.device, dtype=torch.uint8)
    call("spk_sort_trials", ptr(score), ptr(order), ptr(ws), T, stream())
    return order


def error_sweep(score, label, order, costs):
    T, P = score.numel(), len(costs)
    assert score.dtype == torch.float64 and label.dtype == torch.uint8 and order.dtype == torch.int32
    assert label.numel() == T and order.numel() == T and P <= 8
    cd = torch.tensor([[float(v) for v in c] for c in costs], dtype=torch.float64).reshape(P, 3).to(score.device)
    out_d = torch.empty(1 + 2 * P, device=score.device, dtype=torch.float64)
    out_i = torch.empty(3 + P, device=score.device, dtype=torch.int64)
    ws = torch.empty(hip.lib().spk_error_sweep_workspace(T, P), device=score.device, dtype=torch.uint8)
    call("spk_error_sweep", ptr(score), ptr(label), ptr(order), ptr(cd) if P else None, P, ptr(out_d), ptr(out_i), ptr(ws), T,
         stream())
    return out_d, out_i


def _f64_flag(t):
    assert t.dtype in (torch.float32, torch.float64), t.dtype
    return 1 if t.dtype == torch.float64 else 0


def _f64_or_none(t, n):
    assert t is None or (t.dtype == torch.float64 and t.numel() == n and t.is_contiguous()), "a double[%d] table or None" % n
    return ptr(t)


def _rows_ld(t):
    if t.shape[0] == 1:
        assert t.is_cuda and t.dim() == 2 and (t.stride(1) == 1 or t.shape[1] == 1), "libspkhip takes rows of unit stride only"
        return t.data_ptr(), t.shape[1]
    return _ptr_rows(t), t.stride(0)


def scatter_slab_rows(N):
    return hip.lib().spk_scatter_slab_rows(int(N))


def scatter_f64(X, mu=None, w=None):
    N, D = X.shape
    ws_bytes = hip.lib().spk_scatter_f64_workspace(N, D)
    if ws_bytes == 0:
        raise ValueError("scatter_f64: N=%d, D=%d out of range (1 <= D <= 512)" % (N, D))
    C = torch.empty(D, D, device=X.device, dtype=torch.float64)
    ws = torch.empty(ws_bytes // 8, device=X.device, dtype=torch.float64)
    call("spk_scatter_f64", _rows_ld(X)[0], _f64_flag(X), _rows_ld(X)[1], _f64_or_none(mu, D),
         _f64_or_none(w, N), ptr(C), ptr(ws), N, D, stream(), flops=2.0 * N * D * D, nbytes=float(N * D * X.element_size()))
    return C


def segment_sum_f64(X, seg_off, rows=None, mean=False):
    N, D = X.shape
    K = seg_off.numel() - 1
    assert seg_off.dtype == torch.int32 and (rows is None or rows.dtype == torch.int32)
    out = torch.empty(K, D, device=X.device, dtype=torch.float64)
    count = torch.empty(K, device=X.device, dtype=torch.int32)
    call("spk_segment_sum_f64", _rows_ld(X)[0], _f64_flag(X), _rows_ld(X)[1], ptr(rows), ptr(seg_off), ptr(out), ptr(count),
         1 if mean else 0, K, D, stream())
    return out, count


def affine_lennorm(X, A=None, b=None, q=None, scale=False, out_dtype=torch.float32, out=None):
    N, Di = X.shape
    Do = Di if A is None else A.shape[0]
    assert A is None or (A.dtype == torch.float64 and A.shape == (Do, Di))
    assert out_dtype in (torch.float32, torch.float64)
    Y = torch.empty(N, Do, device=X.device, dtype=out_dtype) if out is None else out
    assert Y.shape == (N, Do) and Y.dtype == out_dtype and Y.is_contiguous()
    call("spk_affine_lennorm", _rows_ld(X)[0], _f64_flag(X), _rows_ld(X)[1], ptr(A), _f64_or_none(b, Do), _f64_or_none(q, Do),
         1 if scale else 0, ptr(Y), 1 if out_dtype == torch.float64 else 0, N, Di, Do, stream(),
         flops=0.0 if A is None else 2.0 * N * Di * Do)
    return Y


def plda_posterior_rows(mt, count, psi):
    K, D = mt.shape
    assert mt.dtype == torch.float64 and count.dtype == torch.int32 and count.numel() == K and psi.dtype == torch.float64
    w, r = torch.empty_like(mt), torch.empty_like(mt)
    call("spk_plda_posterior_rows", ptr(mt), ptr(count), ptr(psi), ptr(w), ptr(r), K, D, stream())
    return w, r


def plda_llr(en, te, ia, ib, psi, count, tab_count, tab_log):
    T, D = ia.numel(), en.shape[1]
    assert en.dtype == torch.float64 and te.dtype == torch.float64 and psi.dtype == torch.float64 and te.shape[1] == D
    assert ia.dtype == torch.int32 and ib.dtype == torch.int32 and ib.numel() == T and psi.numel() == D
    assert count is None or (count.dtype == torch.int32 and count.numel() == en.shape[0])
    U = tab_count.numel()
    assert tab_count.dtype == torch.int32 and tab_log.dtype == torch.float64 and tab_log.numel() == 2 * U
    out = torch.empty(T, device=en.device, dtype=torch.float32)
    call("spk_plda_llr", ptr(en), ptr(te), ptr(ia), ptr(ib), ptr(psi), ptr(count), ptr(tab_count), ptr(tab_log), U, ptr(out), T, D,
         en.shape[0], te.shape[0], stream())
    return out
```

Measured before the change: 5659 utt/s.

## Fuse downsample BN backward with main branch; add single-launch BN finalize and reduce lookahead

Three changes to the BN paths. BN finalize now runs as a single-kernel fold for moderate partial-row counts instead of a fold launch followed by a finalize launch. The BN backward reduce loads several rows into registers before accumulating so more memory loads are in flight. In downsample residual blocks, the main-branch BN backward and the downsample BN backward share one apply kernel that reads dy and the mask bits once, with the downsample reduce computed directly from masked dy. This saves launches and memory passes in exchange for more kernels to maintain and extra register pressure.

```diff
diff --git a/include/spkhip.h b/include/spkhip.h
--- a/include/spkhip.h
+++ b/include/spkhip.h
@@ -123,6 +123,13 @@
                      const float* scale, const float* shift, const float* coef, float* draw, float* dz_out, long long N,
                      int C, int mask_mode, unsigned* amax_out ,
                      const unsigned* pair_scale , void* stream);
+int spk_bn_bwd_apply2(float* dy_drawd, const unsigned* bits, const float* raw2, const float* rawd, const float* mean2,
+                      const float* invstd2, const float* coef2, const float* meand, const float* invstdd, const float* coefd,
+                      float* draw2, long long N, int C, unsigned* draw2_amax, const unsigned* pair_scale, unsigned* drawd_amax,
+                      void* stream);
+int spk_bn_finalize_one_form(int on);
+int spk_bn_reduce_ahead_form(int on);
+int spk_ds_fused_bnbwd_form(int on);
 int spk_absmax(const float* x, unsigned* slot, long long n, void* stream);
 int spk_bnbwd_estimate(const float* coef, const float* mean, const float* invstd, int C, const unsigned* amax_in,
                        const unsigned* raw_amax, unsigned* est, void* stream);
diff --git a/pytorch-kaldi-resnet_amd/csrc/bn.hip b/pytorch-kaldi-resnet_amd/csrc/bn.hip
--- a/pytorch-kaldi-resnet_amd/csrc/bn.hip
+++ b/pytorch-kaldi-resnet_amd/csrc/bn.hip
@@ -122,7 +122,62 @@
     }
 }
 
-template <typename T>
+template <typename T, int DEPTH>
+__device__ inline void bn_sum_rows_ahead(const T* __restrict__ partial, int nrows, int C, int ch, int row, double& s, double& ss) {
+    const size_t pitch = (size_t)8 * C * 2;
+    const T* p = partial + ((size_t)row * C + ch) * 2;
+    int k = row;
+    for (; k + 8 * (DEPTH - 1) < nrows; k += 8 * DEPTH, p += DEPTH * pitch) {
+        T a[DEPTH][2];
+#pragma unroll
+        for (int j = 0; j < DEPTH; ++j) {
+            a[j][0] = p[j * pitch];
+            a[j][1] = p[j * pitch + 1];
+        }
+        __builtin_amdgcn_sched_barrier(0);
+#pragma unroll
+        for (int j = 0; j < DEPTH; ++j) {
+            s += (double)a[j][0];
+            ss += (double)a[j][1];
+        }
+    }
+    for (; k < nrows; k += 8, p += pitch) {
+        s += (double)p[0];
+        ss += (double)p[1];
+    }
+}
+#define BN_STAGE2_DEPTH (BN_STAGE_ROWS / 8)
+
+__device__ inline void bn_finalize_tail(int ch, double s, double ss, double count, const float* __restrict__ gamma,
+                                        const float* __restrict__ beta, float* __restrict__ running_mean,
+                                        float* __restrict__ running_var, float* __restrict__ mean_out,
+                                        float* __restrict__ invstd_out, float* __restrict__ scale, float* __restrict__ shift,
+                                        float momentum, float eps, const unsigned* __restrict__ amax_in,
+                                        unsigned* __restrict__ est_out) {
+    const double mean = s / count;
+    double var = ss / count - mean * mean;
+    if (var < 0.0 || count <= 1.0) var = 0.0;
+    const float invstd = (float)(1.0 / sqrt(var + (double)eps));
+    const float g = gamma[ch], b = beta[ch];
+    const float sc = g * invstd;
+    mean_out[ch] = (float)mean;
+    invstd_out[ch] = invstd;
+    const float shv = b - (float)mean * sc;
+    scale[ch] = sc;
+    shift[ch] = shv;
+    if (est_out) {
+        const float e = fabsf(sc) * __uint_as_float(*amax_in) + fabsf(shv);
+        const unsigned bits = __float_as_uint(e);
+        if (bits > __hip_atomic_load(est_out, __ATOMIC_RELAXED, __HIP_MEMORY_SCOPE_AGENT)) atomicMax(est_out, bits);
+    }
+    if (running_mean) {
+        const double unbiased = count > 1.0 ? var * (count / (count - 1.0)) : var;
+        running_mean[ch] = (1.f - momentum) * running_mean[ch] + momentum * (float)mean;
+        running_var[ch] = (1.f - momentum) * running_var[ch] + momentum * (float)unbiased;
+    }
+}
+
+template <typename T, int DEPTH = 4>
 __global__ __launch_bounds__(256) void bn_finalize_kernel(const T* __restrict__ partial, int nblk, int C, double count,
                                                           const float* __restrict__ gamma, const float* __restrict__ beta,
                                                           float* __restrict__ running_mean, float* __restrict__ running_var,
@@ -134,7 +189,10 @@
     const int tid = threadIdx.x, c = tid & 31, row = tid >> 5;
     const int ch = blockIdx.x * 32 + c;
     double s = 0.0, ss = 0.0;
-    if (ch < C) bn_sum_rows<T>(partial, nblk, C, ch, row, s, ss);
+    if (ch < C) {
+        if constexpr (DEPTH == 4) bn_sum_rows<T>(partial, nblk, C, ch, row, s, ss);
+        else bn_sum_rows_ahead<T, DEPTH>(partial, nblk, C, ch, row, s, ss);
+    }
     red[row][c][0] = s;
     red[row][c][1] = ss;
     __syncthreads();
@@ -143,33 +201,101 @@
             s += red[k][c][0];
             ss += red[k][c][1];
         }
-        const double mean = s / count;
-        double var = ss / count - mean * mean;
-        if (var < 0.0 || count <= 1.0) var = 0.0;
-        const float invstd = (float)(1.0 / sqrt(var + (double)eps));
-        const float g = gamma[ch], b = beta[ch];
-        const float sc = g * invstd;
-        mean_out[ch] = (float)mean;
-        invstd_out[ch] = invstd;
-        const float shv = b - (float)mean * sc;
-        scale[ch] = sc;
-        shift[ch] = shv;
-        if (est_out) {
-            const float e = fabsf(sc) * __uint_as_float(*amax_in) + fabsf(shv);
-            const unsigned bits = __float_as_uint(e);
-            if (bits > __hip_atomic_load(est_out, __ATOMIC_RELAXED, __HIP_MEMORY_SCOPE_AGENT)) atomicMax(est_out, bits);
-        }
-        if (running_mean) {
-            const double unbiased = count > 1.0 ? var * (count / (count - 1.0)) : var;
-            running_mean[ch] = (1.f - momentum) * running_mean[ch] + momentum * (float)mean;
-            running_var[ch] = (1.f - momentum) * running_var[ch] + momentum * (float)unbiased;
-        }
+        bn_finalize_tail(ch, s, ss, count, gamma, beta, running_mean, running_var, mean_out, invstd_out, scale, shift, momentum,
+                         eps, amax_in, est_out);
     }
     if (nbt && blockIdx.x == 0 && tid == 0) *nbt += 1;
+}
+
+#define BN_ONE_CH 4
+__device__ inline bool bn_fold_in_block(const float* __restrict__ partial, int nblk, int C, double (*chunk)[BN_ONE_CH][2],
+                                        double (*red)[BN_ONE_CH][2], double& s, double& ss) {
+    const int tid = threadIdx.x, c = tid & (BN_ONE_CH - 1), y = tid / BN_ONE_CH;
+    const int ch = blockIdx.x * BN_ONE_CH + c;
+    const int per = (nblk + BN_STAGE_ROWS - 1) / BN_STAGE_ROWS;
+    const int k0 = y * per;
+    int k1 = k0 + per;
+    if (k1 > nblk) k1 = nblk;
+    double ls[8], lss[8];
+#pragma unroll
+    for (int r = 0; r < 8; ++r) ls[r] = lss[r] = 0.0;
+    if (ch < C) {
+        const size_t pitch = (size_t)C * 2;
+        for (int k = k0; k < k1; k += 8) {
+            float2 v[8];
+#pragma unroll
+            for (int r = 0; r < 8; ++r) {
+                const int kr = k + r < k1 ? k + r : k1 - 1;
+                v[r] = *(const float2*)(partial + (size_t)kr * pitch + (size_t)ch * 2);
+            }
+            __builtin_amdgcn_sched_barrier(0);
+#pragma unroll
+            for (int r = 0; r < 8; ++r)
+                if (k + r < k1) {
+                    ls[r] += (double)v[r].x;
+                    lss[r] += (double)v[r].y;
+                }
+        }
+    }
+    s = ls[0];
+    ss = lss[0];
+#pragma unroll
+    for (int r = 1; r < 8; ++r) {
+        s += ls[r];
+        ss += lss[r];
+    }
+    chunk[y][c][0] = s;
+    chunk[y][c][1] = ss;
+    __syncthreads();
+    const int lane = tid / BN_ONE_CH;
+    if (tid < 8 * BN_ONE_CH) {
+        s = 0.0;
+        ss = 0.0;
+#pragma unroll
+        for (int j = 0; j < BN_STAGE_ROWS / 8; ++j) {
+            s += chunk[lane + 8 * j][c][0];
+            ss += chunk[lane + 8 * j][c][1];
+        }
+        red[lane][c][0] = s;
+        red[lane][c][1] = ss;
+    }
+    __syncthreads();
+    if (tid >= BN_ONE_CH || ch >= C) return false;
+    for (int k = 1; k < 8; ++k) {
+        s += red[k][c][0];
+        ss += red[k][c][1];
+    }
+    return true;
+}
+
+__global__ __launch_bounds__(BN_STAGE_ROWS * BN_ONE_CH) void bn_finalize_one_kernel(
+    const float* __restrict__ partial, int nblk, int C, double count, const float* __restrict__ gamma,
+    const float* __restrict__ beta, float* __restrict__ running_mean, float* __restrict__ running_var, long long* __restrict__ nbt,
+    float* __restrict__ mean_out, float* __restrict__ invstd_out, float* __restrict__ scale, float* __restrict__ shift,
+    float momentum, float eps, const unsigned* __restrict__ amax_in, unsigned* __restrict__ est_out) {
+    __shared__ double chunk[BN_STAGE_ROWS][BN_ONE_CH][2];
+    __shared__ double red[8][BN_ONE_CH][2];
+    double s, ss;
+    if (bn_fold_in_block(partial, nblk, C, chunk, red, s, ss))
+        bn_finalize_tail(blockIdx.x * BN_ONE_CH + threadIdx.x, s, ss, count, gamma, beta, running_mean, running_var, mean_out,
+                         invstd_out, scale, shift, momentum, eps, amax_in, est_out);
+    if (nbt && blockIdx.x == 0 && threadIdx.x == 0) *nbt += 1;
 }
 
 extern "C" size_t spk_bn_finalize_workspace(int nblk, int C) {
     return nblk > BN_STAGE_ROWS ? (size_t)BN_STAGE_ROWS * C * 2 * sizeof(double) : 0;
+}
+
+static int g_bn_finalize_one = 1;
+extern "C" int spk_bn_finalize_one_form(int on) {
+    const int prev = g_bn_finalize_one;
+    g_bn_finalize_one = on < 0 ? 0 : (on > 2 ? 2 : on);
+    return prev;
+}
+static int bn_one_launch_rows(int C) { return C <= 128 ? 4096 : 2048; }
+static bool bn_one_launch(int nblk, int C) {
+    if (!g_bn_finalize_one || nblk <= BN_STAGE_ROWS) return false;
+    return g_bn_finalize_one == 2 || nblk <= bn_one_launch_rows(C);
 }
 
 extern "C" int spk_bn_finalize(const float* partial, int nblk, int C, double count, const float* gamma, const float* beta,
@@ -181,13 +307,18 @@
     SPK_REQUIRE((running_mean == nullptr) == (running_var == nullptr), "spk_bn_finalize: running stats must come in pairs");
     SPK_REQUIRE(!est_out || amax_in, "spk_bn_finalize: est_out needs amax_in");
     hipStream_t st = (hipStream_t)stream;
-    if (spk_bn_finalize_workspace(nblk, C)) {
+    if (bn_one_launch(nblk, C)) {
+        hipLaunchKernelGGL(bn_finalize_one_kernel, dim3(spk_ceil_div(C, BN_ONE_CH)), dim3(BN_STAGE_ROWS * BN_ONE_CH), 0, st, partial,
+                           nblk, C, count, gamma, beta, running_mean, running_var, num_batches_tracked, mean, invstd, scale, shift,
+                           momentum, eps, amax_in, est_out);
+    } else if (spk_bn_finalize_workspace(nblk, C)) {
         SPK_REQUIRE(ws, "spk_bn_finalize: %d partial rows need the fp64 workspace", nblk);
         hipLaunchKernelGGL(bn_fold_partials_kernel, dim3(spk_ceil_div(C, 32), BN_STAGE_ROWS), dim3(256), 0, st, partial, ws, nblk, C);
         SPK_LAUNCH_CHECK("spk_bn_finalize(fold)");
-        hipLaunchKernelGGL(bn_finalize_kernel<double>, dim3(spk_ceil_div(C, 32)), dim3(256), 0, st, ws, BN_STAGE_ROWS, C, count,
-                           gamma, beta, running_mean, running_var, num_batches_tracked, mean, invstd, scale, shift, momentum, eps,
-                           amax_in, est_out);
+        auto fin = g_bn_finalize_one ? bn_finalize_kernel<double, BN_STAGE2_DEPTH> : bn_finalize_kernel<double>;
+        hipLaunchKernelGGL(fin, dim3(spk_ceil_div(C, 32)), dim3(256), 0, st, (const double*)ws, BN_STAGE_ROWS, C, count, gamma, beta,
+                           running_mean, running_var, num_batches_tracked, mean, invstd, scale, shift, momentum, eps, amax_in,
+                           est_out);
     } else {
         hipLaunchKernelGGL(bn_finalize_kernel<float>, dim3(spk_ceil_div(C, 32)), dim3(256), 0, st, partial, nblk, C, count, gamma,
                            beta, running_mean, running_var, num_batches_tracked, mean, invstd, scale, shift, momentum, eps, amax_in,
@@ -354,6 +485,72 @@
     return dy;
 }
 
+template <int NR, int MODE>
+__device__ __forceinline__ void bn_reduce_group(const float* __restrict__ pd, const float* __restrict__ pr,
+                                                const float* __restrict__ pa, const unsigned* __restrict__ pw, size_t step,
+                                                size_t wstep, int wsh, f32x4 mu, f32x4 is, f32x4 sc, f32x4 sh, f32x4& s, f32x4& ss,
+                                                f32x4& mx) {
+    f32x4 rvv[NR], dv[NR], av[NR];
+    unsigned mw[NR];
+#pragma unroll
+    for (int u = 0; u < NR; ++u) {
+        rvv[u] = ld_stream(pr + u * step);
+        dv[u] = ld_stream(pd + u * step);
+        if (MODE == MASK_ACT) av[u] = *(const f32x4*)(pa + u * step);
+        if (MODE == MASK_BITS) mw[u] = pw[u * wstep];
+    }
+    __builtin_amdgcn_sched_barrier(0);
+#pragma unroll
+    for (int u = 0; u < NR; ++u) {
+        const f32x4 rv = rvv[u];
+        f32x4 d = dv[u];
+        if (MODE == MASK_BITS) {
+            const unsigned bits = mw[u] >> wsh;
+#pragma unroll
+            for (int k = 0; k < 4; ++k) d[k] = ((bits >> k) & 1u) ? d[k] : 0.f;
+        } else if (MODE == MASK_ACT) {
+#pragma unroll
+            for (int k = 0; k < 4; ++k) d[k] = av[u][k] > 0.f ? d[k] : 0.f;
+        } else if (MODE == MASK_RAW) {
+#pragma unroll
+            for (int k = 0; k < 4; ++k) d[k] = __builtin_fmaf(rv[k], sc[k], sh[k]) > 0.f ? d[k] : 0.f;
+        }
+        const f32x4 xh = (rv - mu) * is;
+        s += d;
+#pragma unroll
+        for (int k = 0; k < 4; ++k) {
+            ss[k] = __builtin_fmaf(d[k], xh[k], ss[k]);
+            mx[k] = fmaxf(mx[k], spk_finite_abs(d[k]));
+        }
+    }
+}
+
+template <int AHEAD, int MODE>
+__device__ __forceinline__ void bn_reduce_rows_ahead(const float* __restrict__ dy, const float* __restrict__ raw,
+                                                     const float* __restrict__ act, long long r, long long r1, int rstep, int C,
+                                                     int quad, f32x4 mu, f32x4 is, f32x4 sc, f32x4 sh, f32x4& s, f32x4& ss,
+                                                     f32x4& mx) {
+    const size_t off = (size_t)r * C + quad * 4, step = (size_t)rstep * C, wstep = (size_t)rstep * (C >> 5);
+    const float *pd = dy + off, *pr = raw + off, *pa = MODE == MASK_ACT ? act + off : nullptr;
+    const unsigned* pw = MODE == MASK_BITS ? (const unsigned*)act + (size_t)r * (C >> 5) + (quad >> 3) : nullptr;
+    const int wsh = (quad * 4) & 31;
+    for (; r + (long long)(AHEAD - 1) * rstep < r1; r += (long long)AHEAD * rstep) {
+        bn_reduce_group<AHEAD, MODE>(pd, pr, pa, pw, step, wstep, wsh, mu, is, sc, sh, s, ss, mx);
+        pd += AHEAD * step;
+        pr += AHEAD * step;
+        if (MODE == MASK_ACT) pa += AHEAD * step;
+        if (MODE == MASK_BITS) pw += AHEAD * wstep;
+    }
+    for (; r < r1; r += rstep) {
+        bn_reduce_group<1, MODE>(pd, pr, pa, pw, step, wstep, wsh, mu, is, sc, sh, s, ss, mx);
+        pd += step;
+        pr += step;
+        if (MODE == MASK_ACT) pa += step;
+        if (MODE == MASK_BITS) pw += wstep;
+    }
+}
+
+template <int AHEAD>
 __global__ __launch_bounds__(256) void bn_bwd_reduce_kernel(const float* __restrict__ dy, const float* __restrict__ raw,
                                                             const float* __restrict__ act, const float* __restrict__ mean,
                                                             const float* __restrict__ invstd, const float* __restrict__ scale,
@@ -370,6 +567,16 @@
     const f32x4 mu = *(const f32x4*)(mean + quad * 4), is = *(const f32x4*)(invstd + quad * 4);
     const f32x4 sc = *(const f32x4*)(scale + quad * 4), sh = *(const f32x4*)(shift + quad * 4);
     f32x4 s = {0.f, 0.f, 0.f, 0.f}, ss = {0.f, 0.f, 0.f, 0.f}, mx = {0.f, 0.f, 0.f, 0.f};
+    if constexpr (AHEAD > 1) {
+        if (mode == MASK_BITS)
+            bn_reduce_rows_ahead<AHEAD, MASK_BITS>(dy, raw, act, r0 + prow, r1, rstep, C, quad, mu, is, sc, sh, s, ss, mx);
+        else if (mode == MASK_ACT)
+            bn_reduce_rows_ahead<AHEAD, MASK_ACT>(dy, raw, act, r0 + prow, r1, rstep, C, quad, mu, is, sc, sh, s, ss, mx);
+        else if (mode == MASK_RAW)
+            bn_reduce_rows_ahead<AHEAD, MASK_RAW>(dy, raw, act, r0 + prow, r1, rstep, C, quad, mu, is, sc, sh, s, ss, mx);
+        else
+            bn_reduce_rows_ahead<AHEAD, MASK_NONE>(dy, raw, act, r0 + prow, r1, rstep, C, quad, mu, is, sc, sh, s, ss, mx);
+    } else
     for (long long r = r0 + prow; r < r1; r += rstep) {
         const long long off = r * C + quad * 4;
         const f32x4 rv = ld_stream(raw + off);
@@ -417,6 +624,17 @@
             }
         }
     }
+}
+
+#ifndef BN_REDUCE_AHEAD
+#define BN_REDUCE_AHEAD 4
+#endif
+static int g_bn_reduce_form = 1, g_bn_reduce_ahead = BN_REDUCE_AHEAD;
+extern "C" int spk_bn_reduce_ahead_form(int on) {
+    const int prev = g_bn_reduce_form;
+    g_bn_reduce_form = on;
+    g_bn_reduce_ahead = on <= 0 ? 1 : (on == 2 || on == 4 || on == 8) ? on : BN_REDUCE_AHEAD;
+    return prev;
 }
 
 extern "C" int spk_bn_bwd_reduce(const float* dy, const float* raw, const float* act, const float* mean, const float* invstd,
@@ -428,8 +646,11 @@
     SPK_REQUIRE((mask_mode != MASK_ACT && mask_mode != MASK_BITS) || act, "spk_bn_bwd_reduce: MASK_ACT / MASK_BITS need the activated tensor / its sign bits");
     const int nb = spk_bn_stats_blocks(N, C);
     const int rpb = (int)((N + nb - 1) / nb);
-    hipLaunchKernelGGL(bn_bwd_reduce_kernel, dim3(nb), dim3(256), 0, (hipStream_t)stream, dy, raw, act, mean, invstd, scale,
-                       shift, partial, N, C, rpb, mask_mode, chan_amax);
+    auto kern = g_bn_reduce_ahead == 1 ? bn_bwd_reduce_kernel<1>
+              : g_bn_reduce_ahead == 2 ? bn_bwd_reduce_kernel<2>
+              : g_bn_reduce_ahead == 8 ? bn_bwd_reduce_kernel<8> : bn_bwd_reduce_kernel<4>;
+    hipLaunchKernelGGL(kern, dim3(nb), dim3(256), 0, (hipStream_t)stream, dy, raw, act, mean, invstd, scale, shift, partial, N, C,
+                       rpb, mask_mode, chan_amax);
     SPK_LAUNCH_CHECK("spk_bn_bwd_reduce");
     return 0;
 }
@@ -439,7 +660,26 @@
     return fabsf(k1) * (A + fabsf(m1) + xh * fabsf(m2)) * (1.f + 1.52587890625e-05f);
 }
 
-template <typename T>
+__device__ inline void bn_bwd_finalize_tail(int ch, double s, double ss, int C, double count, const float* __restrict__ gamma,
+                                            const float* __restrict__ invstd, float* __restrict__ dgamma, float* __restrict__ dbeta,
+                                            float* __restrict__ coef, int accumulate, const unsigned* __restrict__ amax_in,
+                                            const unsigned* __restrict__ raw_amax, const float* __restrict__ mean,
+                                            unsigned* __restrict__ est_out, const unsigned* __restrict__ chan_amax) {
+    dbeta[ch] = accumulate ? dbeta[ch] + (float)s : (float)s;
+    dgamma[ch] = accumulate ? dgamma[ch] + (float)ss : (float)ss;
+    const float k1 = gamma[ch] * invstd[ch], m1 = (float)(s / count), m2 = (float)(ss / count);
+    coef[ch] = k1;
+    coef[C + ch] = m1;
+    coef[2 * C + ch] = m2;
+    if (est_out) {
+        const float A = chan_amax ? __uint_as_float(chan_amax[ch]) : __uint_as_float(*amax_in);
+        const float e = bnbwd_bound(k1, m1, m2, mean[ch], invstd[ch], A, __uint_as_float(*raw_amax));
+        const unsigned bits = __float_as_uint(e);
+        if (bits > __hip_atomic_load(est_out, __ATOMIC_RELAXED, __HIP_MEMORY_SCOPE_AGENT)) atomicMax(est_out, bits);
+    }
+}
+
+template <typename T, int DEPTH = 4>
 __global__ __launch_bounds__(256) void bn_bwd_finalize_kernel(const T* __restrict__ partial, int nblk, int C, double count,
                                                               const float* __restrict__ gamma, const float* __restrict__ invstd,
                                                               float* __restrict__ dgamma, float* __restrict__ dbeta,
@@ -451,7 +691,10 @@
     const int tid = threadIdx.x, c = tid & 31, row = tid >> 5;
     const int ch = blockIdx.x * 32 + c;
     double s = 0.0, ss = 0.0;
-    if (ch < C) bn_sum_rows<T>(partial, nblk, C, ch, row, s, ss);
+    if (ch < C) {
+        if constexpr (DEPTH == 4) bn_sum_rows<T>(partial, nblk, C, ch, row, s, ss);
+        else bn_sum_rows_ahead<T, DEPTH>(partial, nblk, C, ch, row, s, ss);
+    }
     red[row][c][0] = s;
     red[row][c][1] = ss;
     __syncthreads();
@@ -460,19 +703,22 @@
             s += red[k][c][0];
             ss += red[k][c][1];
         }
-        dbeta[ch] = accumulate ? dbeta[ch] + (float)s : (float)s;
-        dgamma[ch] = accumulate ? dgamma[ch] + (float)ss : (float)ss;
-        const float k1 = gamma[ch] * invstd[ch], m1 = (float)(s / count), m2 = (float)(ss / count);
-        coef[ch] = k1;
-        coef[C + ch] = m1;
-        coef[2 * C + ch] = m2;
-        if (est_out) {
-            const float A = chan_amax ? __uint_as_float(chan_amax[ch]) : __uint_as_float(*amax_in);
-            const float e = bnbwd_bound(k1, m1, m2, mean[ch], invstd[ch], A, __uint_as_float(*raw_amax));
-            const unsigned bits = __float_as_uint(e);
-            if (bits > __hip_atomic_load(est_out, __ATOMIC_RELAXED, __HIP_MEMORY_SCOPE_AGENT)) atomicMax(est_out, bits);
-        }
-    }
+        bn_bwd_finalize_tail(ch, s, ss, C, count, gamma, invstd, dgamma, dbeta, coef, accumulate, amax_in, raw_amax, mean, est_out,
+                             chan_amax);
+    }
+}
+
+__global__ __launch_bounds__(BN_STAGE_ROWS * BN_ONE_CH) void bn_bwd_finalize_one_kernel(
+    const float* __restrict__ partial, int nblk, int C, double count, const float* __restrict__ gamma,
+    const float* __restrict__ invstd, float* __restrict__ dgamma, float* __restrict__ dbeta, float* __restrict__ coef,
+    int accumulate, const unsigned* __restrict__ amax_in, const unsigned* __restrict__ raw_amax, const float* __restrict__ mean,
+    unsigned* __restrict__ est_out, const unsigned* __restrict__ chan_amax) {
+    __shared__ double chunk[BN_STAGE_ROWS][BN_ONE_CH][2];
+    __shared__ double red[8][BN_ONE_CH][2];
+    double s, ss;
+    if (bn_fold_in_block(partial, nblk, C, chunk, red, s, ss))
+        bn_bwd_finalize_tail(blockIdx.x * BN_ONE_CH + threadIdx.x, s, ss, C, count, gamma, invstd, dgamma, dbeta, coef, accumulate,
+                             amax_in, raw_amax, mean, est_out, chan_amax);
 }
 
 extern "C" int spk_bn_bwd_finalize(const float* partial, int nblk, int C, double count, const float* gamma,
@@ -484,12 +730,17 @@
     SPK_REQUIRE(!est_out || ((amax_in || chan_amax) && raw_amax && mean),
                 "spk_bn_bwd_finalize: est_out needs amax_in (or chan_amax), raw_amax and mean");
     hipStream_t st = (hipStream_t)stream;
-    if (spk_bn_finalize_workspace(nblk, C)) {
+    if (bn_one_launch(nblk, C)) {
+        hipLaunchKernelGGL(bn_bwd_finalize_one_kernel, dim3(spk_ceil_div(C, BN_ONE_CH)), dim3(BN_STAGE_ROWS * BN_ONE_CH), 0, st,
+                           partial, nblk, C, count, gamma, invstd, dgamma, dbeta, coef, accumulate, amax_in, raw_amax, mean, est_out,
+                           chan_amax);
+    } else if (spk_bn_finalize_workspace(nblk, C)) {
         SPK_REQUIRE(ws, "spk_bn_bwd_finalize: %d partial rows need the fp64 workspace", nblk);
         hipLaunchKernelGGL(bn_fold_partials_kernel, dim3(spk_ceil_div(C, 32), BN_STAGE_ROWS), dim3(256), 0, st, partial, ws, nblk, C);
         SPK_LAUNCH_CHECK("spk_bn_bwd_finalize(fold)");
-        hipLaunchKernelGGL(bn_bwd_finalize_kernel<double>, dim3(spk_ceil_div(C, 32)), dim3(256), 0, st, ws, BN_STAGE_ROWS, C, count,
-                           gamma, invstd, dgamma, dbeta, coef, accumulate, amax_in, raw_amax, mean, est_out, chan_amax);
+        auto fin = g_bn_finalize_one ? bn_bwd_finalize_kernel<double, BN_STAGE2_DEPTH> : bn_bwd_finalize_kernel<double>;
+        hipLaunchKernelGGL(fin, dim3(spk_ceil_div(C, 32)), dim3(256), 0, st, (const double*)ws, BN_STAGE_ROWS, C, count, gamma, invstd,
+                           dgamma, dbeta, coef, accumulate, amax_in, raw_amax, mean, est_out, chan_amax);
     } else {
         hipLaunchKernelGGL(bn_bwd_finalize_kernel<float>, dim3(spk_ceil_div(C, 32)), dim3(256), 0, st, partial, nblk, C, count, gamma,
                            invstd, dgamma, dbeta, coef, accumulate, amax_in, raw_amax, mean, est_out, chan_amax);
@@ -594,6 +845,75 @@
     return 0;
 }
 
+__global__ __launch_bounds__(256) void bn_bwd_apply2_kernel(float* dy , const unsigned* __restrict__ words,
+                                                            const float* __restrict__ raw2, const float* __restrict__ rawd,
+                                                            const float* __restrict__ mean2, const float* __restrict__ invstd2,
+                                                            const float* __restrict__ coef2, const float* __restrict__ meand,
+                                                            const float* __restrict__ invstdd, const float* __restrict__ coefd,
+                                                            float* __restrict__ draw2, unsigned nquads, int C,
+                                                            unsigned* __restrict__ amax2, const unsigned* __restrict__ pair_scale,
+                                                            unsigned* __restrict__ amaxd) {
+    const int cmask = C - 1;
+    float mx2 = 0.f, mxd = 0.f;
+    const float sig = spk_sigma_from_amax_bits(*pair_scale);
+    const unsigned stride = gridDim.x * 256u;
+    const int lgq = 29 - __builtin_clz((unsigned)C);
+    const unsigned cw = (unsigned)C >> 5;
+    const int c0 = (threadIdx.x * 4) & cmask;
+    const f32x4 pmu = *(const f32x4*)(mean2 + c0), pis = *(const f32x4*)(invstd2 + c0), pk1 = *(const f32x4*)(coef2 + c0);
+    const f32x4 pm1 = *(const f32x4*)(coef2 + C + c0), pm2 = *(const f32x4*)(coef2 + 2 * C + c0);
+    const f32x4 qmu = *(const f32x4*)(meand + c0), qis = *(const f32x4*)(invstdd + c0), qk1 = *(const f32x4*)(coefd + c0);
+    const f32x4 qm1 = *(const f32x4*)(coefd + C + c0), qm2 = *(const f32x4*)(coefd + 2 * C + c0);
+    for (unsigned i = blockIdx.x * 256u + threadIdx.x; i < nquads; i += stride) {
+        const size_t off = (size_t)i * 4;
+        const f32x4 rv = ld_stream(raw2 + off), rd = ld_stream(rawd + off);
+        f32x4 d = ld_stream(dy + off);
+        const unsigned bits = words[(size_t)(i >> lgq) * cw + ((unsigned)c0 >> 5)] >> (c0 & 31);
+#pragma unroll
+        for (int k = 0; k < 4; ++k) d[k] = ((bits >> k) & 1u) ? d[k] : 0.f;
+        const f32x4 xh = (rv - pmu) * pis, xd = (rd - qmu) * qis;
+        const f32x4 t = d - pm1, td = d - qm1;
+        f32x4 o, od;
+#pragma unroll
+        for (int k = 0; k < 4; ++k) {
+            o[k] = pk1[k] * __builtin_fmaf(-xh[k], pm2[k], t[k]);
+            od[k] = qk1[k] * __builtin_fmaf(-xd[k], qm2[k], td[k]);
+        }
+        uint2 t0, t1;
+        split2h(o, sig, t0, t1);
+        st_stream(draw2 + off, spk_pair_pack(t0, t1));
+        st_stream(dy + off, od);
+        mx2 = fmaxf(fmaxf(mx2, fmaxf(fabsf(o[0]), fabsf(o[1]))), fmaxf(fabsf(o[2]), fabsf(o[3])));
+        mxd = fmaxf(fmaxf(mxd, fmaxf(fabsf(od[0]), fabsf(od[1]))), fmaxf(fabsf(od[2]), fabsf(od[3])));
+    }
+    if (amax2) spk_wave_amax_commit(mx2, amax2);
+    if (amaxd) spk_wave_amax_commit(mxd, amaxd);
+}
+
+extern "C" int spk_bn_bwd_apply2(float* dy_drawd, const unsigned* bits, const float* raw2, const float* rawd, const float* mean2,
+                                 const float* invstd2, const float* coef2, const float* meand, const float* invstdd,
+                                 const float* coefd, float* draw2, long long N, int C, unsigned* draw2_amax,
+                                 const unsigned* pair_scale, unsigned* drawd_amax, void* stream) {
+    SPK_REQUIRE(dy_drawd && bits && raw2 && rawd && mean2 && invstd2 && coef2 && meand && invstdd && coefd && draw2 && pair_scale,
+                "spk_bn_bwd_apply2: null pointer");
+    SPK_REQUIRE(N > 0 && bn_c_ok(C) && C % 32 == 0, "spk_bn_bwd_apply2: N=%lld C=%d (C: a power of two in [32,1024])", N, C);
+    SPK_REQUIRE(draw2 != dy_drawd, "spk_bn_bwd_apply2: draw2 must not alias dy");
+    const long long nquads = N * C / 4;
+    SPK_REQUIRE(nquads < 2147483647LL / 8, "spk_bn_bwd_apply2: %lld values exceed the 32-bit group index of the kernel", N * C);
+    hipLaunchKernelGGL(bn_bwd_apply2_kernel, dim3(stream_grid(nquads, 1, BN_BWD_APPLY_CAP)), dim3(256), 0, (hipStream_t)stream,
+                       dy_drawd, bits, raw2, rawd, mean2, invstd2, coef2, meand, invstdd, coefd, draw2, (unsigned)nquads, C,
+                       draw2_amax, pair_scale, drawd_amax);
+    SPK_LAUNCH_CHECK("spk_bn_bwd_apply2");
+    return 0;
+}
+
+static int g_ds_fused_bnbwd = 1;
+extern "C" int spk_ds_fused_bnbwd_form(int on) {
+    const int prev = g_ds_fused_bnbwd;
+    if (on >= 0) g_ds_fused_bnbwd = on ? 1 : 0;
+    return prev;
+}
+
 __global__ __launch_bounds__(256) void absmax_kernel(const float* __restrict__ x, long long n, unsigned* __restrict__ slot) {
     float mx = 0.f;
     const long long nq = n >> 2;
diff --git a/pytorch-kaldi-resnet_amd/engine.py b/pytorch-kaldi-resnet_amd/engine.py
--- a/pytorch-kaldi-resnet_amd/engine.py
+++ b/pytorch-kaldi-resnet_amd/engine.py
@@ -488,7 +488,7 @@
     def _block_bwd(self, b, rec, dout, acc, dout_partial=None, prev=None, dout_amax=None, amx=None, chan=False):
         x, raws, out = rec["x"], rec["raws"], rec["out"]
         n = len(b.convs)
-        g, g_part, g_amax, dz = dout, dout_partial, dout_amax, None
+        g, g_part, g_amax, dz, ds_done = dout, dout_partial, dout_amax, None, None
         take = (lambda: amx.take()) if amx is not None else (lambda: None)
         for i in range(n - 1, -1, -1):
             c, bn, raw = b.convs[i], b.bns[i], raws[i]
@@ -563,11 +563,25 @@
                     bits = rec.get("mask")
                     lazy_dz = b.ds is None and bits is not None and n > 1
                     ca = amx.take_n(c.cout) if (chan and pairs and g_part is None) else None
-                    draw = ops.bn_backward(g, raw, bits if bits is not None else out, bn.t4, bn.h.weight.data, bn.h.weight.grad,
-                                           bn.h.bias.grad, MASK_BITS if bits is not None else MASK_ACT,
-                                           dz_out=None if lazy_dz else g, accumulate=acc, partial=g_part, amax_out=draw_amax,
-                                           pair=pair, chan_amax=ca)
-                    dz = None if lazy_dz else g
+                    if b.ds is not None and bits is not None and pairs and ops.ds_fused_bnbwd():
+                        nrow = raw.numel() // raw.shape[-1]
+                        if g_part is None:
+                            g_part = ops.bn_bwd_partial(g, raw, bits, bn.t4, MASK_BITS, chan_amax=ca)
+                        coef = ops.bn_bwd_coef(g_part, nrow, bn.h.weight.data, bn.t4, bn.h.weight.grad, bn.h.bias.grad, acc,
+                                               amax_in=g_amax, raw_amax=raw_amax, est_out=est, chan_amax=ca)
+                        bnd = b.ds[1]
+                        partd = ops.bn_bwd_partial(g, rec["rawd"], bits, bnd.t4, MASK_BITS)
+                        coefd = ops.bn_bwd_coef(partd, nrow, bnd.h.weight.data, bnd.t4, bnd.h.weight.grad, bnd.h.bias.grad, acc)
+                        drawd_amax = take() if (amx is not None and ops.split_for(1, True) == 3) else None
+                        draw, drawd = ops.bn_bwd_apply2(g, bits, raw, bn.t4, coef, rec["rawd"], bnd.t4, coefd, est,
+                                                        draw2_amax=draw_amax, drawd_amax=drawd_amax)
+                        ds_done = (drawd, drawd_amax)
+                    else:
+                        draw = ops.bn_backward(g, raw, bits if bits is not None else out, bn.t4, bn.h.weight.data,
+                                               bn.h.weight.grad, bn.h.bias.grad, MASK_BITS if bits is not None else MASK_ACT,
+                                               dz_out=None if lazy_dz else g, accumulate=acc, partial=g_part, amax_out=draw_amax,
+                                               pair=pair, chan_amax=ca)
+                        dz = None if lazy_dz else g
                 else:
                     draw = ops.bn_backward(g, raw, None, bn.t4, bn.h.weight.data, bn.h.weight.grad, bn.h.bias.grad, MASK_RAW,
                                            draw_out=g, accumulate=acc, partial=g_part, amax_out=draw_amax, pair=pair)
@@ -589,9 +603,12 @@
         if b.ds is not None:
             cd, bnd = b.ds
             f16d = amx is not None and ops.split_for(1, True) == 3
-            drawd_amax = take() if f16d else None
-            drawd = ops.bn_backward(dz, rec["rawd"], None, bnd.t4, bnd.h.weight.data, bnd.h.weight.grad, bnd.h.bias.grad,
-                                    MASK_NONE, draw_out=dz, accumulate=acc, amax_out=drawd_amax)
+            if ds_done is not None:
+                drawd, drawd_amax = ds_done
+            else:
+                drawd_amax = take() if f16d else None
+                drawd = ops.bn_backward(dz, rec["rawd"], None, bnd.t4, bnd.h.weight.data, bnd.h.weight.grad, bnd.h.bias.grad,
+                                        MASK_NONE, draw_out=dz, accumulate=acc, amax_out=drawd_amax)
             self._count(drawd, drawd_amax)
             self._wgrad(x, drawd, cd.h.weight.grad, 1, cd.stride, accumulate=acc, dy_amax=drawd_amax,
                         x_amax=rec["in_amax"][0] if f16d else None)
diff --git a/pytorch-kaldi-resnet_amd/hip.py b/pytorch-kaldi-resnet_amd/hip.py
--- a/pytorch-kaldi-resnet_amd/hip.py
+++ b/pytorch-kaldi-resnet_amd/hip.py
@@ -57,6 +57,10 @@
     "spk_bn_bwd_reduce": [_P] * 8 + [_L, _I, _I, _P, _P],
     "spk_bn_bwd_finalize": [_P, _I, _I, _D] + [_P] * 5 + [_I, _P, _P, _P, _P, _P, _P, _P],
     "spk_bn_bwd_apply": [_P] * 10 + [_L, _I, _I, _P, _P, _P],
+    "spk_bn_bwd_apply2": [_P] * 11 + [_L, _I, _P, _P, _P, _P],
+    "spk_bn_finalize_one_form": [_I],
+    "spk_bn_reduce_ahead_form": [_I],
+    "spk_ds_fused_bnbwd_form": [_I],
     "spk_absmax": [_P, _P, _L, _P],
     "spk_bnbwd_estimate": [_P, _P, _P, _I, _P, _P, _P, _P],
     "spk_f16_window_count": [_P, _P, _P, _L, _I, _P, _I, _P, _P],
@@ -160,6 +164,12 @@
             fn.restype = ctypes.c_int
         if os.environ.get("SPK_POOL_ROWS", "1") == "0":
             l.spk_stats_pool_row_form(0)
+        if os.environ.get("SPK_BN_FINALIZE_ONE", "1") != "1":
+            l.spk_bn_finalize_one_form(int(os.environ["SPK_BN_FINALIZE_ONE"]))
+        if os.environ.get("SPK_BN_REDUCE_AHEAD", "1") != "1":
+            l.spk_bn_reduce_ahead_form(int(os.environ["SPK_BN_REDUCE_AHEAD"]))
+        if os.environ.get("SPK_DS_FUSED_BNBWD", "1") == "0":
+            l.spk_ds_fused_bnbwd_form(0)
         _lib = l
     return _lib
 
diff --git a/pytorch-kaldi-resnet_amd/ops.py b/pytorch-kaldi-resnet_amd/ops.py
--- a/pytorch-kaldi-resnet_amd/ops.py
+++ b/pytorch-kaldi-resnet_amd/ops.py
@@ -686,6 +686,21 @@
     return part
 
 
+def ds_fused_bnbwd():
+    return hip.lib().spk_ds_fused_bnbwd_form(-1) != 0
+
+
+def bn_bwd_apply2(dy, bits, raw2, bn4, coef2, rawd, bnd4, coefd, pair_scale, draw2_amax=None, drawd_amax=None):
+    C = raw2.shape[-1]
+    N = raw2.numel() // C
+    assert rawd.shape == raw2.shape == dy.shape
+    draw2 = torch.empty_like(raw2)
+    call("spk_bn_bwd_apply2", ptr(dy), ptr(bits), ptr(raw2), ptr(rawd), ptr(bn4[0]), ptr(bn4[1]), ptr(coef2), ptr(bnd4[0]),
+         ptr(bnd4[1]), ptr(coefd), ptr(draw2), N, C, ptr(draw2_amax), ptr(pair_scale), ptr(drawd_amax), stream(),
+         nbytes=4.0 * raw2.numel() * 5 + raw2.numel() / 8.0)
+    return draw2, dy
+
+
 def se_squeeze(x, wlen=None):
     B, H, W, C = x.shape
     if wlen is not None:
```

Result: no change. 5705 utt/s, median of 6 (+0.8%).
